# ajparra/iRotAvg

Measured on AMD Instinct MI355X. Metric: IRLS edge-updates/sec (+ iters-to-converge), higher is better.
Workload: dtype f64

## Files before the change

### irotavg_amd/capi.py

```python
import ctypes as C
import os

import numpy as np

_HERE = os.path.dirname(os.path.abspath(__file__))
LIB_PATH = os.path.join(_HERE, "libirotavg_hip.so")

OK = 0
ERR_BAD_ARG, ERR_NOT_SPANNING, ERR_SOLVER, ERR_UNKNOWN_COST = -1, -2, -3, -4
ERR_NOMEM, ERR_HIP, ERR_NO_DEVICE, ERR_NOT_CONVERGED = -5, -6, -7, -8
ERR_UNSUPPORTED = -9

SYMBOLS = [
    "irotavg_default_options", "irotavg_init_mst", "irotavg_make_A", "irotavg_l1ra", "irotavg_irls",
    "irotavg_quat_normalised", "irotavg_graph_create", "irotavg_graph_destroy",
    "irotavg_graph_set_rotations", "irotavg_graph_get_rotations",
    "irotavg_graph_snapshot_rotations", "irotavg_graph_restore_rotations", "irotavg_graph_get_weights",
    "irotavg_graph_set_weights", "irotavg_graph_irls", "irotavg_graph_l1ra",
    "irotavg_graph_quat_normalised", "irotavg_graph_get_stats", "irotavg_graph_reset_stats",
    "irotavg_graph_synchronize", "irotavg_graph_edge_residual", "irotavg_graph_get_residuals",
    "irotavg_graph_ls_solve", "irotavg_graph_update_weights", "irotavg_graph_apply_step",
    "irotavg_graph_l1decode_pd", "irotavg_graph_time_kernel", "irotavg_graph_fingerprint", "irotavg_version",
    "irotavg_device_count", "irotavg_error_string",
    "irotavg_viewgraph_create", "irotavg_viewgraph_destroy", "irotavg_viewgraph_add_view",
# ... 243 lines not shown
    return I


def default_options(**kw):
    o = Options()
    lib().irotavg_default_options(C.byref(o))
    for k, v in kw.items():
        if not hasattr(o, k):
            raise AttributeError(k)
        setattr(o, k, v)
    return o


def check(rc, where):
    if rc != OK:
        raise IrotavgError(rc, where)


class Graph:

    def __init__(self, I, QQ, n_total, f, **opts):
        I = edges(I)
        QQ = fmat(QQ)
        self.m, self.n_total, self.f = len(I), int(n_total), int(f)
        self.nu = self.n_total - self.f
        self._h = C.c_void_p()
        o = default_options(**opts)
        rc = lib().irotavg_graph_create(C.byref(self._h), self.m, self.n_total, self.f, _i(I),
                                        _d(QQ), QQ.shape[0], C.byref(o))
        if rc != OK:
            self._h = C.c_void_p()
            raise IrotavgError(rc, "irotavg_graph_create")

    def close(self):
        if getattr(self, "_h", None) and self._h.value:
            lib().irotavg_graph_destroy(self._h)
            self._h = C.c_void_p()

    def __del__(self):
        try:
            self.close()
        except Exception:
            pass

    def __enter__(self):
        return self

    def __exit__(self, *a):
        self.close()

    def set_rotations(self, Q):
        Q = fmat(Q)
        assert Q.shape == (self.n_total, 4)
        check(lib().irotavg_graph_set_rotations(self._h, _d(Q), Q.shape[0]), "set_rotations")

    def get_rotations(self):
        Q = np.zeros((self.n_total, 4), order="F")
        check(lib().irotavg_graph_get_rotations(self._h, _d(Q), Q.shape[0]), "get_rotations")
        return Q

    def snapshot_rotations(self):
        check(lib().irotavg_graph_snapshot_rotations(self._h), "snapshot_rotations")

    def restore_rotations(self):
        check(lib().irotavg_graph_restore_rotations(self._h), "restore_rotations")

    def get_weights(self):
        w = np.zeros(self.m)
        check(lib().irotavg_graph_get_weights(self._h, _d(w)), "get_weights")
        return w

    def set_weights(self, w):
        w = np.ascontiguousarray(w, dtype=np.float64)
        assert w.shape == (self.m,)
        check(lib().irotavg_graph_set_weights(self._h, _d(w)), "set_weights")

    def irls(self, cost=4, sigma=5 * np.pi / 180, max_iters=50, change_th=1e-3, allow_rc=()):
        iters = C.c_int(0)
        rt = C.c_double(0)
        trace = np.full(max(max_iters, 1), np.nan)
        rc = lib().irotavg_graph_irls(self._h, cost, sigma, max_iters, change_th, C.byref(iters),
                                      C.byref(rt), _d(trace))
        if rc != OK and rc not in allow_rc:
            raise IrotavgError(rc, "irotavg_graph_irls")
        return dict(rc=rc, iters=iters.value, runtime=rt.value, scores=trace[:iters.value].copy())

    def l1ra(self, max_iters=5, change_th=1e-3, allow_rc=()):
        iters = C.c_int(0)
        rt = C.c_double(0)
        trace = np.full(max(max_iters, 1), np.nan)
        rc = lib().irotavg_graph_l1ra(self._h, max_iters, change_th, C.byref(iters), C.byref(rt),
                                      _d(trace))
        if rc != OK and rc not in allow_rc:
            raise IrotavgError(rc, "irotavg_graph_l1ra")
        return dict(rc=rc, iters=iters.value, runtime=rt.value, scores=trace[:iters.value].copy())

    def quat_normalised(self):
        check(lib().irotavg_graph_quat_normalised(self._h), "quat_normalised")

    def stats(self):
        s = Stats()
        check(lib().irotavg_graph_get_stats(self._h, C.byref(s)), "get_stats")
        d = {k: getattr(s, k) for k, _ in Stats._fields_
             if k not in ("level_rows", "level_nnz", "last_relres")}
        d["level_rows"] = list(s.level_rows)[:s.levels]
        d["level_nnz"] = list(s.level_nnz)[:s.levels]
        d["last_relres"] = list(s.last_relres)
        return d

    def reset_stats(self):
        lib().irotavg_graph_reset_stats(self._h)

    def synchronize(self):
        check(lib().irotavg_graph_synchronize(self._h), "synchronize")

    def edge_residual(self):
        check(lib().irotavg_graph_edge_residual(self._h), "edge_residual")

    def get_residuals(self):
        r = np.zeros((self.m, 3), order="F")
        check(lib().irotavg_graph_get_residuals(self._h, _d(r), self.m), "get_residuals")
        return r

    def ls_solve(self, allow_rc=(), return_rc=False):
        X = np.zeros((self.nu, 3), order="F")
        rc = lib().irotavg_graph_ls_solve(self._h, _d(X), self.nu)
        if rc != OK and rc not in allow_rc:
            raise IrotavgError(rc, "irotavg_graph_ls_solve")
        return (rc, X) if return_rc else X

    def update_weights(self, cost, sigma):
        check(lib().irotavg_graph_update_weights(self._h, cost, sigma), "update_weights")

    def apply_step(self):
        s = C.c_double(0)
        check(lib().irotavg_graph_apply_step(self._h, C.byref(s)), "apply_step")
        return s.value

    def l1decode_pd(self, y, pdmaxiter=2):
        y = np.ascontiguousarray(y, dtype=np.float64)
        assert y.shape == (self.m,)
        x = np.zeros(self.nu)
        stuck = C.c_int(0)
        check(lib().irotavg_graph_l1decode_pd(self._h, _d(y), pdmaxiter, _d(x), C.byref(stuck)),
              "l1decode_pd")
        return x, stuck.value

    def direct_info(self):
        out = (C.c_int64 * 64)()
        k = lib().irotavg_graph_direct_info(self._h, out, 64)
        if k < 0:
            raise IrotavgError(k, "direct_info")
        if out[0] == 0:
            return dict(block=0, levels=[], closures=0, fused_assembly=0)
        nl = int(out[1])
        return dict(block=int(out[0]), levels=[dict(blocks=int(out[2 + 3 * l]), chunks=int(out[3 + 3 * l]),
                                                    reduced=int(out[4 + 3 * l])) for l in range(nl)],
                    closures=int(out[2 + 3 * nl]), fused_assembly=int(out[3 + 3 * nl]) if k > 3 + 3 * nl else 0)

    def direct_residual(self):
        out = np.zeros(3)
        check(lib().irotavg_graph_direct_residual(self._h, _d(out)), "direct_residual")
        return out

    def rotation_variance(self, pairs=None, marginals=True, allow_rc=()):
        return _variance_call(lambda *a: lib().irotavg_graph_rotation_variance(self._h, *a), self.n_total, pairs,
                              marginals, allow_rc, "irotavg_graph_rotation_variance")

    def edge_diagnostics(self, edge_var=True, leverage=True, chi2=True, allow_rc=()):
        return _edge_call(lambda *a: lib().irotavg_graph_edge_diagnostics(self._h, *a), self.m, edge_var, leverage,
                          chi2, allow_rc, "irotavg_graph_edge_diagnostics")

    def pose_weights(self, cost, sigma):
        check(lib().irotavg_graph_pose_weights(self._h, int(cost), float(sigma)), "irotavg_graph_pose_weights")

    def fingerprint(self):
        out = (C.c_uint64 * 512)()
        n = lib().irotavg_graph_fingerprint(self._h, out, 512)
        if n < 0:
            raise IrotavgError(n, "fingerprint")
        return [int(out[i]) for i in range(n)]

    FINGERPRINT_TAIL = ("l0_far_entries", "asm_windowed", "asm_l1_fused", "l1_fused", "cg2", "ndense", "ndense_pad",
                        "dense_bw", "mg_dense_max", "mg_kc_x1000", "additive_top")

    def fingerprint_scalars(self):
        fp = self.fingerprint()
        k = len(self.FINGERPRINT_TAIL)
        if not k <= len(fp) < 512:
            raise ValueError("fingerprint truncated: %d words" % len(fp))
        return dict(zip(self.FINGERPRINT_TAIL, fp[-k:]))

    def time_kernel(self, which, reps=20):
        ms = C.c_double(0)
        check(lib().irotavg_graph_time_kernel(self._h, which, reps, C.byref(ms)), "time_kernel")
        return ms.value


def _variance_call(call, n_total, pairs, marginals, allow_rc, where):
    P = np.zeros((0, 2), dtype=np.int32) if pairs is None else np.ascontiguousarray(pairs, dtype=np.int32).reshape(-1, 2)
    var = np.full(n_total, np.nan) if marginals else None
    pv = np.full(max(len(P), 1), np.nan)
    scale = C.c_double(np.nan)
    rc = call(_d(var) if marginals else None, len(P), _i(P) if len(P) else None, _d(pv), C.byref(scale))
    if rc != OK and rc not in allow_rc:
        raise IrotavgError(rc, where)
    return dict(rc=rc, var=var, pair_var=pv[:len(P)], scale=scale.value)


def rotation_variance(I, QQ, Q, weights, f, pairs=None, marginals=True, allow_rc=()):
    I = edges(I)
    Q = fmat(Q)
    QQ = fmat(QQ)
    w = np.ascontiguousarray(weights, dtype=np.float64)
    n_total = Q.shape[0]
    return _variance_call(lambda *a: lib().irotavg_rotation_variance(len(I), n_total, int(f), _i(I), _d(QQ),
                                                                     QQ.shape[0], _d(Q), Q.shape[0], _d(w), *a),
                          n_total, pairs, marginals, allow_rc, "irotavg_rotation_variance")


def _edge_call(call, m, edge_var, leverage, chi2, allow_rc, where):
    out = [np.full(m, np.nan) if want else None for want in (edge_var, leverage, chi2)]
    scale = C.c_double(np.nan)
    rc = call(*[_d(a) if a is not None else None for a in out], C.byref(scale))
    if rc != OK and rc not in allow_rc:
        raise IrotavgError(rc, where)
    return dict(rc=rc, edge_var=out[0], leverage=out[1], chi2=out[2], scale=scale.value)


def edge_diagnostics(I, QQ, Q, weights, f, edge_var=True, leverage=True, chi2=True, allow_rc=()):
    I = edges(I)
    Q = fmat(Q)
    QQ = fmat(QQ)
    w = np.ascontiguousarray(weights, dtype=np.float64)
    n_total = Q.shape[0]
    return _edge_call(lambda *a: lib().irotavg_edge_diagnostics(len(I), n_total, int(f), _i(I), _d(QQ), QQ.shape[0],
                                                                _d(Q), Q.shape[0], _d(w), *a),
                      len(I), edge_var, leverage, chi2, allow_rc, "irotavg_edge_diagnostics")


def oneshot_cache(enable):
    lib().irotavg_oneshot_cache(1 if enable else 0)


def oneshot_cache_clear():
    lib().irotavg_oneshot_cache_clear()


def oneshot_cache_stats():
    h, m = C.c_int64(0), C.c_int64(0)
    lib().irotavg_oneshot_cache_stats(C.byref(h), C.byref(m))
    return int(h.value), int(m.value)


def trim_memory():
    return int(lib().irotavg_trim_memory())


def window_solve(I, QQ, Q, f, cost=4, sigma=5 * np.pi / 180, l1_iters=100, irls_iters=100,
                 change_th=1e-3, kernel=0):
    I = edges(I)
    QQ = fmat(QQ)
    Q = fmat(Q)
    w = np.zeros(len(I))
    a, b = C.c_int(0), C.c_int(0)
    rc = lib().irotavg_window_solve_kernel(len(I), Q.shape[0], f, _i(I), _d(QQ), QQ.shape[0], _d(Q),
                                           Q.shape[0], cost, sigma, l1_iters, irls_iters, change_th,
                                           _d(w), C.byref(a), C.byref(b), kernel)
    check(rc, "irotavg_window_solve")
    return dict(Q=Q, weights=w, l1_iters=a.value, irls_iters=b.value)


def window_uncertainty(I, QQ, Q, f, weights=None, sigma=5 * np.pi / 180, pairs=None, marginals=True, edge_var=True,
                       leverage=True, chi2=True, allow_rc=()):
    I = edges(I)
    QQ = fmat(QQ)
    Q = fmat(Q)
    w = None if weights is None else np.ascontiguousarray(weights, dtype=np.float64)
    if w is not None and w.shape != (len(I),):
        raise ValueError("weights must have %d entries" % len(I))
    P = np.zeros((0, 2), dtype=np.int32) if pairs is None else np.ascontiguousarray(pairs, dtype=np.int32).reshape(-1, 2)
    n_total = Q.shape[0]
    var = np.full(n_total, np.nan) if marginals else None
    pv = np.full(max(len(P), 1), np.nan)
    out = [np.full(len(I), np.nan) if want else None for want in (edge_var, leverage, chi2)]
    scale = C.c_double(np.nan)
    rc = lib().irotavg_window_uncertainty(len(I), n_total, int(f), _i(I), _d(QQ), QQ.shape[0], _d(Q), n_total,
                                          None if w is None else _d(w), float(sigma), None if var is None else _d(var),
                                          len(P), _i(P) if len(P) else None, _d(pv) if len(P) else None,
                                          *[None if a is None else _d(a) for a in out], C.byref(scale))
    if rc != OK and rc not in allow_rc:
        raise IrotavgError(rc, "irotavg_window_uncertainty")
    return dict(rc=rc, var=var, pair_var=pv[:len(P)], edge_var=out[0], leverage=out[1], chi2=out[2], scale=scale.value)


def window_gate(I, QQ, Q, f, cand_I, cand_QQ, weights=None, sigma=5 * np.pi / 180, angle=True, pair_var=True, chi2=True,
                allow_rc=()):
    I = edges(I)
    QQ = fmat(QQ)
    Q = fmat(Q)
    w = None if weights is None else np.ascontiguousarray(weights, dtype=np.float64)
    if w is not None and w.shape != (len(I),):
        raise ValueError("weights must have %d entries" % len(I))
    cI = np.ascontiguousarray(cand_I, dtype=np.int32).reshape(-1, 2)
    cQ = fmat(np.asarray(cand_QQ, dtype=np.float64).reshape(-1, 4))
    if len(cQ) != len(cI):
        raise ValueError("cand_QQ must have %d rows" % len(cI))
    nc, n_total = len(cI), Q.shape[0]
    out = [np.full(nc, np.nan) if want else None for want in (angle, pair_var, chi2)]
    scale = C.c_double(np.nan)
    rc = lib().irotavg_window_gate(len(I), n_total, int(f), _i(I), _d(QQ), QQ.shape[0], _d(Q), n_total,
# ... 231 lines not shown
```

### irotavg_amd/csrc/bcr.hip

```cpp
#include <atomic>

#include "graph.hpp"
#include "kernels.hpp"
#include "asm0w.hpp"

namespace irh {
constexpr double kBcrGateTolMin = 1e-12;

typedef double v4d __attribute__((ext_vector_type(4)));
typedef double v2d __attribute__((ext_vector_type(2)));
typedef int v2i __attribute__((ext_vector_type(2)));

constexpr int kTopMax = 16, kTopRounds = 6;
struct BcrTopSched {
    int n = 0, nr = 0, last = 0;
    signed char ne[kTopRounds];
    signed char i[kTopRounds][4], a[kTopRounds][4], c[kTopRounds][4];
};

#if defined(__HIP_DEVICE_COMPILE__)
#define IRH_GPTR(T) T __attribute__((address_space(1))) *
#else
#define IRH_GPTR(T) T *
#endif
typedef IRH_GPTR(const double) gp_cd;
typedef IRH_GPTR(double) gp_d;
typedef IRH_GPTR(const int) gp_ci;
typedef IRH_GPTR(int) gp_i;
typedef IRH_GPTR(unsigned) gp_u;
typedef IRH_GPTR(const double4) gp_cd4;
constexpr int kUpLevels = 8;
struct BcrUpLevel {
    int nb, nred, nch;
    gp_cd inD, inR, inXD, inXR, inXG;
    gp_d W, sepD, sepR, extD, extR, extG;
};
struct BcrUpArgs {
    int nl;
    BcrUpLevel lev[kUpLevels];
    int n;
    gp_ci sl_off, col;
    gp_cd val, diag;
    gp_cd4 rhs;
    gp_d xtop;
    gp_u cnt;
    int top16;
    BcrTopSched top;
    gp_d xtop_all;
    gp_i fail;
};

struct BcrLevel {
    int nb = 0;
    int nred = 0;
    int nch = 0;
    DevBuf<double> W;
    DevBuf<double> sepD, sepR, extD, extR, extG;
    DevBuf<double> x;
};
struct BcrState {
    int B = 0;
    int NR = 3;
    int nfar = 0;
    std::vector<BcrLevel> lev;
    DevBuf<double> xtop;
    DevBuf<int> far_i, far_j, far_e;
    std::vector<DevBuf<double>> Dinv;
    DevBuf<double> topDinv;
    DevBuf<int> cl_off;
    DevBuf<int4> cl_step;
    DevBuf<int4> cl_init;
    DevBuf<int> cl_owner;
    DevBuf<double> cl_R, cl_W;
    DevBuf<double> cl_S, cl_T, lam;
    DevBuf<int> cl_alive;
    DevBuf<int> dead;
    DevBuf<int> co_off, co_rec;
    DevBuf<int2> co_elim;
    int cl_nslots = 0, cl_nsteps = 0, cl_nelim = 0, cl_npad = 0, cl_maxsteps = 1, cl_ndense = 0;
    DevBuf<int> cl_dense;
    int ext0 = 0;
    int dbg_word = -1;
    DevBuf<long long> stamps;
    DevBuf<unsigned> up_cnt;
    unsigned up_gen = 0;
    DevBuf<BcrUpArgs> up_args;
    bool up_used = false;
    bool top16 = false;
    BcrTopSched tsched;
    DevBuf<BcrTopSched> tsched_dev;
    DevBuf<int> ghost_extcol;
    DevBuf<double> remD, remR;
    DevBuf<double> res_part;
    DevBuf<int> res_zero;
    DevBuf<int> gate_skip;
    bool dead_clean = false;
    DevBuf<int2> cl_fin;
    DevBuf<int> cl_gid;
    DevBuf<uint8_t> cl_own;
    DevBuf<int> fix_row, fix_off, fix_e;
    DevBuf<double> fix_saved;
    int nfix = 0;
};

void BcrDeleter::operator()(BcrState *p) const { delete p; }

template <int CTRL>
__device__ __forceinline__ double bcr_dpp(double v) {
    int lo = __double2loint(v), hi = __double2hiint(v);
    lo = __builtin_amdgcn_mov_dpp(lo, CTRL, 0xf, 0xf, true);
    hi = __builtin_amdgcn_mov_dpp(hi, CTRL, 0xf, 0xf, true);
    return __hiloint2double(hi, lo);
}
__device__ __forceinline__ double bcr_row16_sum(double v) {
    v += bcr_dpp<0xB1>(v);
    v += bcr_dpp<0x4E>(v);
    v += bcr_dpp<0x141>(v);
    v += bcr_dpp<0x140>(v);
    return v;
}

template <int B>
__device__ __forceinline__ void bcr_invert(double *Dm, int lane, int *dead = nullptr, bool reg = false) {
    static_assert(B % 2 == 0 && B <= 32, "block size");
    constexpr int HB = B / 2;
    const int c = lane & 31, h = lane >> 5;
    const bool act = c < B;
    const int cl = act ? c : B - 1;
    const v2d *Dh = reinterpret_cast<const v2d *>(Dm + h * HB);
    double t[HB];
#pragma unroll
    for (int i = 0; i < HB; i++) t[i] = Dm[(h * HB + i) * B + cl];
    const double dg = Dm[cl * B + cl];
    const double dgt = kDeadTol * dg;
    int ndead = 0;
    auto pivot_inverse = [&](double tk, int k, int kh) {
        const double p0 = readlane_d(tk, k + 32 * kh);
        const bool alive = p0 > readlane_d(dgt, k);
        ndead += alive ? 0 : 1;
        double p = p0;
        if (reg && !alive) {
            const double ref = readlane_d(dg, k);
            p = ref > 0.0 ? ref : 1.0;
        }
        double x = __builtin_amdgcn_rcp(p);
        x = fma(fma(-p, x, 1.0), x, x);
        x = fma(fma(-p, x, 1.0), x, x);
        return (alive || reg) ? x : 0.0;
    };
    if (h == 0 && act) Dm[c] = c == 0 ? -1.0 : t[0];
    asm volatile("" ::: "memory");
    double pinv = pivot_inverse(t[0], 0, 0);
    double rowk = Dm[cl], colk[HB];
#pragma unroll
    for (int i = 0; i < HB; i += 2) {
        const v2d v = Dh[i / 2];
        colk[i] = v.x;
        colk[i + 1] = v.y;
    }
#pragma unroll
    for (int k = 0; k < B; k++) {
        const int kh = k / HB, ki = k - kh * HB;
        const int k1 = k + 1, kh1 = k1 / HB, ki1 = k1 - kh1 * HB;
        const bool isk = c == k;
        const double f = rowk * pinv;
        const double g = f;
        const double keep = isk ? 0.0 : 1.0;
        auto upd = [&](int i) {
            const double a = t[i] * keep;
            double u = fma(-colk[i], g, a);
            if (i == ki) u = (h == kh) ? g : u;
            t[i] = u;
        };
        double pinv1 = 0.0, rowk1 = 0.0, colk1[HB];
        if (k1 < B) {
            upd(ki1);
            if (h == kh1 && act) Dm[c] = c == k1 ? -1.0 : t[ki1];
            asm volatile("" ::: "memory");
            pinv1 = pivot_inverse(t[ki1], k1, kh1);
            rowk1 = Dm[cl];
#pragma unroll
            for (int i = 0; i < HB; i += 2) {
                const v2d v = Dh[i / 2];
                colk1[i] = v.x;
                colk1[i + 1] = v.y;
            }
        }
#pragma unroll
        for (int i = 0; i < HB; i++)
            if (!(k1 < B && i == ki1)) upd(i);
#pragma unroll
        for (int i = 0; i < HB; i++) asm volatile("" : "+v"(t[i]));
        if (k1 < B) {
            pinv = pinv1;
            rowk = rowk1;
#pragma unroll
            for (int i = 0; i < HB; i++) colk[i] = colk1[i];
        }
    }
    asm volatile("" ::: "memory");
#pragma unroll
    for (int i = 0; i < HB; i++)
        if (act) Dm[(h * HB + i) * B + c] = -t[i];
    if (dead && ndead && lane == 0) atomicAdd(dead, ndead);
}

__device__ __forceinline__ void bcr_stamp(long long *st, int slot) {
    if (st && threadIdx.x == 0) st[(size_t)blockIdx.x * 16 + slot] = (long long)__builtin_readcyclecounter();
}

template <int B, int NR = 3>
struct BcrDim {
    static constexpr int NC = 2 * B + NR;
// ... 142 lines not shown
        constexpr int NS = (Dm::NT + WPE - 1) / WPE;
        const int lj = lane & 15, lk = lane >> 4;
#pragma unroll
        for (int sl = 0; sl < NS; sl++) {
            const int nt = part + sl * WPE;
            if (nt >= Dm::NT) continue;
            const int j = 16 * nt + lj;
#pragma unroll
            for (int mt = 0; mt < Dm::MT; mt++)
#pragma unroll
                for (int r = 0; r < 4; r++) {
                    const int row = 16 * mt + 4 * r + lk;
                    if (row < B) {
                        const double v = w[mt][sl][r];
                        if (j < B)
                            Di[row * B + j] = v;
                        else if (j < 2 * B) {
                            if (hasQ) Q[row * B + j - B] = v;
                        } else if (j < Dm::NC)
                            Ri[row * NR + j - 2 * B] = v;
                    }
                }
        }
    }

    template <int WPE>
    __device__ __forceinline__ void phase2_mul(int part, const double *P, v4d (&out)[Dm::MT][NTPW], int lane) {
        constexpr int NS = (Dm::NT + WPE - 1) / WPE;
        double aop[Dm::MT][Dm::KS];
        bcr_load_a<B, false>(P, lane, aop);
#pragma unroll
        for (int sl = 0; sl < NS; sl++)
#pragma unroll
            for (int mt = 0; mt < Dm::MT; mt++) out[mt][sl] = v4d{0.0, 0.0, 0.0, 0.0};
#pragma unroll
        for (int s = 0; s < Dm::KS; s++)
#pragma unroll
            for (int sl = 0; sl < NS; sl++) {
                if (part + sl * WPE >= Dm::NT) continue;
#pragma unroll
                for (int mt = 0; mt < Dm::MT; mt++)
                    out[mt][sl] = __builtin_amdgcn_mfma_f64_16x16x4f64(aop[mt][s], w[s >> 2][sl][s & 3], out[mt][sl], 0, 0, 0);
            }
    }
    template <int WPE>
    __device__ __forceinline__ void phase2_put(int part, const v4d (&out)[Dm::MT][NTPW], double *P, double *Da,
                                               bool assign, double *Ra, int lane) {
        constexpr int NS = (Dm::NT + WPE - 1) / WPE;
        const int lj = lane & 15, lk = lane >> 4;
#pragma unroll
        for (int sl = 0; sl < NS; sl++) {
            const int nt = part + sl * WPE;
            if (nt >= Dm::NT) continue;
            const int c = 16 * nt + lj;
#pragma unroll
            for (int mt = 0; mt < Dm::MT; mt++)
#pragma unroll
                for (int r = 0; r < 4; r++) {
                    const int row = 16 * mt + 4 * r + lk;
                    if (row < B) {
                        const double v = out[mt][sl][r];
                        if (c < B)
                            Da[row * B + c] = assign ? -v : Da[row * B + c] - v;
                        else if (c < 2 * B)
                            P[row * B + c - B] = -v;
                        else if (c < Dm::NC)
                            Ra[row * NR + c - 2 * B] -= v;
                    }
                }
        }
    }
};

template <int B, int NR, int NBT = 12>
__device__ __forceinline__ void bcr_gather_row(int row, int lb, int r, const int *__restrict__ sl_off,
                                               const int *__restrict__ col, const double *__restrict__ val,
                                               const double *__restrict__ diag, const double4 *__restrict__ rhs,
                                               double *blocks, int oD, int oGnext, int oGprevT, double *Rblk, int nfar,
                                               const int *__restrict__ far_i, const int *__restrict__ far_j) {
    double *Dblk = blocks + oD;
    const int sl = row >> 6, ln = row & 63;
    const int o0 = sl_off[sl], w = sl_off[sl + 1] - o0;
    const v2i *__restrict__ cp = reinterpret_cast<const v2i *>(col) + (size_t)(o0 / 2) * 64 + ln;
    const v2d *__restrict__ vp = reinterpret_cast<const v2d *>(val) + (size_t)(o0 / 2) * 64 + ln;
    const int c0 = lb * B;
    const double dgv = diag[row];
    const double4 bb = rhs[row];
    for (int q0 = 0; q0 < w / 2; q0 += NBT) {
        v2i cc[NBT];
        v2d vv[NBT];
#pragma unroll
        for (int u = 0; u < NBT; u++) {
            const int q = q0 + u < w / 2 ? q0 + u : w / 2 - 1;
            cc[u] = __builtin_nontemporal_load(&cp[(size_t)q * 64]);
            vv[u] = __builtin_nontemporal_load(&vp[(size_t)q * 64]);
        }
#pragma unroll
        for (int u = 0; u < NBT; u++) {
#pragma unroll
            for (int h = 0; h < 2; h++) {
                const int c = h ? cc[u].y : cc[u].x;
                const double v = h ? vv[u].y : vv[u].x;
                const int gc = c - c0;
                const bool inD = gc >= 0 && gc < B, inN = gc >= B && gc < 2 * B, inP = gc < 0 && gc >= -B;
                int idx = oD + r * B + r;
                idx = inD ? oD + r * B + gc : idx;
                idx = inN ? oGnext + r * B + gc - B : idx;
                idx = inP ? oGprevT + (gc + B) * B + r : idx;
                const bool keep = q0 + u < w / 2 && v != 0.0 && !(inN && oGnext < 0) && !(inP && oGprevT < 0);
                double *dst = blocks + idx;
                if (keep) atomicAdd(dst, v);
            }
        }
    }
    Dblk[r * B + r] += dgv;
    Rblk[r * NR + 0] = bb.x;
    Rblk[r * NR + 1] = bb.y;
    Rblk[r * NR + 2] = bb.z;
    if (NR > 3)
        for (int q = 0; q < nfar; q++) {
            const int fi = far_i[q], fj = far_j[q];
            if (fi == row || fj == row) Rblk[r * NR + 3 + q] = (fi == row ? 1.0 : 0.0) - (fj == row ? 1.0 : 0.0);
        }
}

__constant__ signed char kBcrPlace[9][8] = {{-1, -1, -1, -1, -1, -1, -1, -1}, {7, -1, -1, -1, -1, -1, -1, -1},
                                             {3, 7, -1, -1, -1, -1, -1, -1},   {3, 5, 7, -1, -1, -1, -1, -1},
                                             {1, 3, 5, 7, -1, -1, -1, -1},     {1, 3, 5, 6, 7, -1, -1, -1},
                                             {1, 3, 4, 5, 6, 7, -1, -1},       {1, 2, 3, 4, 5, 6, 7, -1},
                                             {0, 1, 2, 3, 4, 5, 6, 7}};
__device__ __forceinline__ int bcr_pos(bool placed, int k, int t) { return placed ? (int)kBcrPlace[k][t] : t; }
__device__ __forceinline__ int bcr_ridx(bool placed, int k, int i) {
    if (!placed) return i < k ? i : -1;
    for (int t = 0; t < k; t++)
        if (kBcrPlace[k][t] == i) return t;
    return -1;
}

template <bool COH>
__device__ __forceinline__ double bcr_ld(const double *p) {
    if (!COH) return *p;
    const unsigned long long v = __hip_atomic_load(reinterpret_cast<const unsigned long long *>(p), __ATOMIC_RELAXED, __HIP_MEMORY_SCOPE_AGENT);
    return __longlong_as_double((long long)v);
}
template <bool COH>
__device__ __forceinline__ void bcr_st(double *p, double v) {
    if (!COH)
        *p = v;
    else
        __hip_atomic_store(reinterpret_cast<unsigned long long *>(p), (unsigned long long)__double_as_longlong(v), __ATOMIC_RELAXED,
                           __HIP_MEMORY_SCOPE_AGENT);
}

template <int B, int NR, bool L0, bool TOP, int NW, bool COH>
__device__ __forceinline__ void bcr_reduce_body(
    const int chunk, double (*sDG)[B * B], double (*sR)[B * NR], double *sZ,

    int nb, int nred, int n, const int *__restrict__ sl_off, const int *__restrict__ col, const double *__restrict__ val,
    const double *__restrict__ diag, const double4 *__restrict__ rhs, const double *__restrict__ inD,
    const double *__restrict__ inR, const double *__restrict__ inXD, const double *__restrict__ inXR,
    const double *__restrict__ inXG, double *__restrict__ W, double *__restrict__ sepD, double *__restrict__ sepR,
    double *__restrict__ extD, double *__restrict__ extR, double *__restrict__ extG, double *__restrict__ xtop, int dbg,
    int nfar, const int *__restrict__ far_i, const int *__restrict__ far_j, int ext0, const int *__restrict__ bptr,
    const int *__restrict__ bghost, const double *__restrict__ bval, const int *__restrict__ ghost_extcol, int place,
    long long *__restrict__ stamps, double *__restrict__ Dinvg, double *__restrict__ topDinv, int *__restrict__ deadctr,
    int reg) {
    typedef BcrDim<B, NR> Dm;
    constexpr int BB = B * B;
    double(*sD)[BB] = sDG;
    double(*sG)[BB] = sDG + 8;
    const int tid = threadIdx.x, lane = tid & 63;
    const int wave = __builtin_amdgcn_readfirstlane(tid >> 6);
    const bool hasExt = chunk > 0 || ext0;
    constexpr int NT_ = NW * 64;
    const int kreal = nb - chunk * 8 < 8 ? nb - chunk * 8 : 8;
    const bool placed = place && kreal < 8;

    const bool fastload = !L0 && !placed && !(chunk * 8 + 8 > nred && nred < nb);
    if (!fastload) {
        for (int e = tid; e < 8 * BB; e += NT_) {
            (&sD[0][0])[e] = 0.0;
            (&sG[0][0])[e] = 0.0;
        }
        for (int e = tid; e < 9 * B * NR; e += NT_) (&sR[0][0])[e] = 0.0;
        if (tid < 2) sZ[tid] = 0.0;
    }
    bcr_stamp(stamps, 0);
    if (!fastload) __syncthreads();
    bcr_stamp(stamps, 1);
    if (!L0 && fastload) {
        constexpr int NIT = (8 * BB + NT_ - 1) / NT_, U = NIT <= 12 ? NIT : 8;
        constexpr int NIR = (8 * B * NR + NT_ - 1) / NT_;
        const size_t cb = (size_t)chunk * 8 * BB, cr = (size_t)chunk * 8 * B * NR;
        double vr[NIR], vy[NIR];
#pragma unroll
        for (int u = 0; u < NIR; u++) {
            const int e = tid + NT_ * u, i = e / (B * NR);
            const bool ok = e < 8 * B * NR && i < kreal;
            vr[u] = ok ? bcr_ld<COH>(inR + cr + e) : 0.0;
            vy[u] = ok && chunk * 8 + i + 1 < nred ? bcr_ld<COH>(inXR + cr + B * NR + e) : 0.0;
        }
        for (int u0 = 0; u0 < NIT; u0 += U) {
            double vd[U], vx[U], vg[U];
#pragma unroll
            for (int u = 0; u < U; u++) {
                const int e = tid + NT_ * (u0 + u), i = e / BB;
                const bool ok = e < 8 * BB && i < kreal;
                vd[u] = ok ? bcr_ld<COH>(inD + cb + e) : 0.0;
                vx[u] = ok && chunk * 8 + i + 1 < nred ? bcr_ld<COH>(inXD + cb + BB + e) : 0.0;
                vg[u] = ok && (chunk * 8 + i > 0 || ext0) ? bcr_ld<COH>(inXG + cb + e) : 0.0;
            }
#pragma unroll
            for (int u = 0; u < U; u++) {
                const int e = tid + NT_ * (u0 + u), i = e / BB, el = e - i * BB;
                if (e >= 8 * BB) continue;
                (&sD[0][0])[e] = i < kreal ? vd[u] + vx[u] : (el % (B + 1) == 0 ? 1.0 : 0.0);
                (&sG[0][0])[e] = vg[u];
            }
        }
#pragma unroll
        for (int u = 0; u < NIR; u++) {
            const int e = tid + NT_ * u;
            if (e < 8 * B * NR) (&sR[1][0])[e] = vr[u] + vy[u];
        }
        for (int e = tid; e < B * NR; e += NT_) sR[0][e] = 0.0;
        if (tid < 2) sZ[tid] = 0.0;
    } else if (L0) {
        const int row0 = chunk * 8 * B;
        for (int t = tid; t < kreal * B; t += NT_) {
            const int row = row0 + t, blk = t / B, r = t - blk * B;
            const int ps = bcr_pos(placed, kreal, blk);
            if (row < n)
                bcr_gather_row<B, NR>(row, chunk * 8 + blk, r, sl_off, col, val, diag, rhs, &sDG[0][0], ps * BB,
                                      ps < 7 ? (8 + ps + 1) * BB : -1, blk == 0 ? 8 * BB : -1, sR[ps + 1], nfar, far_i,
                                      far_j);
            else
                sD[ps][r * B + r] = 1.0;
        }
        for (int i = placed ? 1 : 0; i < 8; i++)
            if (bcr_ridx(placed, kreal, i) < 0)
                for (int e = tid; e < B; e += NT_) sD[i][e * B + e] = 1.0;
        if (ext0 && chunk == 0) {
            for (int r = tid; r < B && r < n; r += NT_)
                for (int sl = bptr[r]; sl < bptr[r + 1]; sl++) {
                    const int gi = bghost[sl];
                    const int ec = gi >= 0 ? ghost_extcol[gi] : -1;
                    if (ec >= 0) sG[0][ec * B + r] -= bval[sl];
                }
        }
    } else {
        auto where = [&](int i, int &gb, int &slot) {
            const int t = bcr_ridx(placed, kreal, i);
            gb = t >= 0 ? chunk * 8 + t : -1;
            slot = t > 0 ? bcr_pos(placed, kreal, t - 1) + 1 : 0;
            return t;
        };
        constexpr int NIT = (8 * BB + NT_ - 1) / NT_, U = NIT <= 12 ? NIT : 8;
        const bool allraw = !placed && chunk * 8 >= nred;
        if (allraw)
            for (int e = tid; e < (8 - kreal) * B; e += NT_) sD[kreal + e / B][(e % B) * (B + 1)] = 1.0;
        for (int u0 = 0; u0 < NIT && !allraw; u0 += U) {
            double vd[U], vx[U], vg[U];
#pragma unroll
            for (int u = 0; u < U; u++) {
                const int e = tid + NT_ * (u0 + u), i = e / BB, el = e - i * BB;
                int gb, slot;
                const int t = e < 8 * BB ? where(i, gb, slot) : -1;
                const bool ok = t >= 0 && gb < nred;
                vd[u] = ok ? bcr_ld<COH>(inD + (size_t)gb * BB + el) : 0.0;
                vx[u] = ok && gb + 1 < nred ? bcr_ld<COH>(inXD + (size_t)(gb + 1) * BB + el) : 0.0;
                vg[u] = ok && (gb > 0 || ext0) ? bcr_ld<COH>(inXG + (size_t)gb * BB + el) : 0.0;
            }
#pragma unroll
            for (int u = 0; u < U; u++) {
                const int e = tid + NT_ * (u0 + u), i = e / BB, el = e - i * BB;
                if (e >= 8 * BB) continue;
                int gb, slot;
                const int t = where(i, gb, slot);
                if (t >= 0 && gb < nred) {
                    sD[i][el] = vd[u] + vx[u];
                    if (gb > 0 || ext0) sG[slot][el] = vg[u];
                } else if (t < 0 && !(placed && i == 0) && el / B == el % B) {
                    sD[i][el] = 1.0;
                }
            }
        }
        if (!allraw) {
            constexpr int NIR = (8 * B * NR + NT_ - 1) / NT_;
            double vr[NIR], vy[NIR];
#pragma unroll
            for (int u = 0; u < NIR; u++) {
                const int e = tid + NT_ * u, i = e / (B * NR), el = e - i * (B * NR);
                int gb, slot;
                const int t = e < 8 * B * NR ? where(i, gb, slot) : -1;
                const bool ok = t >= 0 && gb < nred;
                vr[u] = ok ? bcr_ld<COH>(inR + (size_t)gb * B * NR + el) : 0.0;
                vy[u] = ok && gb + 1 < nred ? bcr_ld<COH>(inXR + (size_t)(gb + 1) * B * NR + el) : 0.0;
                if (ok) sR[i + 1][el] = vr[u] + vy[u];
            }
        }
        if (chunk * 8 + 8 > nred && nred < nb) {
            for (int t = tid; t < 8 * B; t += NT_) {
                const int i = t / B, r = t - i * B, gb = chunk * 8 + i;
                if (gb >= nred && gb < nb) {
                    const int lb = 8 * nred + (gb - nred), row = lb * B + r;
                    if (row < n)
                        bcr_gather_row<B, NR, (NW == 8 && B <= 24 ? 24 : 12)>(row, lb, r, sl_off, col, val, diag, rhs, &sDG[0][0],
                                                                            i * BB, -1, gb > 0 ? (8 + i) * BB : -1, sR[i + 1],
                                                                            nfar, far_i, far_j);
                    else
                        sD[i][r * B + r] = 1.0;
                }
            }
        }
    }
    __syncthreads();
    bcr_stamp(stamps, 2);

    constexpr int WPE0 = NW / 4 < Dm::NT ? NW / 4 : Dm::NT;
    constexpr int NTPW = (Dm::NT + WPE0 - 1) / WPE0;
    BcrElim<B, NR, NTPW> E;
    v4d out[Dm::MT][NTPW];
#define IRH_BCR_ROUND(RND)                                                                                          \
    {                                                                                                               \
        constexpr int NE = 4 >> RND;                                                                                \
        constexpr int WPE = NW / NE < Dm::NT ? NW / NE : Dm::NT;                                                    \
         \
         \
         \
        const int e = wave / WPE, part0 = wave - e * WPE;                                                           \
        const int part = (WPE == 2 && NE == 4) ? (part0 ^ ((e >> 1) & 1)) : part0;                                  \
        int i = -1, a = -1, c = 7;                                                                                  \
        if (e < NE) {                                                                                               \
            if (RND == 0) {                                                                                         \
                i = 2 * e;                                                                                          \
                a = i - 1;                                                                                          \
                c = i + 1;                                                                                          \
            } else if (RND == 1) {                                                                                  \
                i = 1 + 4 * e;                                                                                      \
                a = e == 0 ? -1 : 3;                                                                                \
                c = e == 0 ? 3 : 7;                                                                                 \
            } else {                                                                                                \
                i = 3;                                                                                              \
            }                                                                                                       \
        }                                                                                                           \
        const bool active = i >= 0 && bcr_ridx(placed, kreal, i) >= 0;                                              \
        const bool hasP = a >= 0 || hasExt;                                                                         \
           \
          \
        const int isw = wave < NE ? (RND == 0 ? 2 * wave : RND == 1 ? 1 + 4 * wave : 3) : -1;                       \
        if (isw >= 0 && bcr_ridx(placed, kreal, isw) >= 0 && !(dbg & 1))                                            \
            bcr_invert<B>(sD[isw], lane, deadctr, reg != 0);                                                        \
        __syncthreads();                                                                                            \
                                        \
        if (Dinvg && active && part == 0)                                                                           \
            for (int o = lane; o < BB; o += 64) Dinvg[((size_t)chunk * 7 + i) * BB + o] = sD[i][o];                 \
        bcr_stamp(stamps, 3 + 4 * RND);                                                                             \
        if (active && !(dbg & 2))                                                                                   \
            E.template phase1<WPE>(part, sD[i], sG[a + 1], hasP, sG[i + 1], sR[i + 1], sD[c], sR[c + 1],            \
                                   W + ((size_t)chunk * 7 + i) * B * Dm::NC, sZ, lane);                             \
        __syncthreads();                                                                                            \
        bcr_stamp(stamps, 4 + 4 * RND);                                                                             \
        if (active && hasP && !(dbg & 4)) E.template phase2_mul<WPE>(part, sG[a + 1], out, lane);                   \
        if (WPE > 1) __syncthreads();                                                                               \
        bcr_stamp(stamps, 5 + 4 * RND);                                                                             \
        if (active && hasP && !(dbg & 4))                                                                           \
            E.template phase2_put<WPE>(part, out, sG[a + 1], a >= 0 ? sD[a] : sD[0], a < 0 && RND == 0, sR[a + 1],  \
                                       lane);                                                                       \
        __syncthreads();                                                                                            \
        bcr_stamp(stamps, 6 + 4 * RND);                                                                             \
    }
    IRH_BCR_ROUND(0)
    IRH_BCR_ROUND(1)
    IRH_BCR_ROUND(2)
#undef IRH_BCR_ROUND

    if (TOP) {
        if (wave == 0) {
            if (bcr_ridx(placed, kreal, 7) >= 0) {
                bcr_invert<B>(sD[7], lane, deadctr, reg != 0);
                if (topDinv)
                    for (int o = lane; o < BB; o += 64) topDinv[o] = sD[7][o];
                for (int o = lane; o < B * NR; o += 64) {
                    const int k = o / NR, q = o - NR * k;
                    double s = 0.0;
                    for (int cidx = 0; cidx < B; cidx++) s += sD[7][k * B + cidx] * sR[8][cidx * NR + q];
                    xtop[o] = s;
                }
            } else {
                for (int o = lane; o < B * NR; o += 64) xtop[o] = 0.0;
            }
        }
    } else {
        for (int e = tid; e < BB; e += NT_) {
            bcr_st<COH>(sepD + (size_t)chunk * BB + e, sD[7][e]);
            if (hasExt) {
                bcr_st<COH>(extD + (size_t)chunk * BB + e, sD[0][e]);
                bcr_st<COH>(extG + (size_t)chunk * BB + e, sG[0][e]);
            }
        }
        for (int e = tid; e < B * NR; e += NT_) {
            bcr_st<COH>(sepR + (size_t)chunk * B * NR + e, sR[8][e]);
            if (hasExt) bcr_st<COH>(extR + (size_t)chunk * B * NR + e, sR[0][e]);
        }
    }
    bcr_stamp(stamps, 15);
}

struct BcrAsmArgs {
    int nch, nsl;
    long long m, mpad;
    const uint32_t *slot_eid;
    const int *tile_e0;
    const uint32_t *beid;
    const uint8_t *bflag;
    const double *wsrc, *er;
    double *excess, *idg, *bval;
};
template <bool ASM>
struct BcrL0Ptr {
    typedef const double *__restrict__ d;
    typedef const double4 *__restrict__ d4;
};
template <>
struct BcrL0Ptr<true> {
    typedef double *d;
    typedef double4 *d4;
};

template <int B, int NR, bool L0, bool TOP, int NW, bool ASM = false>
__global__ __launch_bounds__(NW * 64, (NW == 4 && B <= 24 && NR == 3 ? 2 : 1)) void k_bcr_reduce(

    int nb, int nred, int n, const int *__restrict__ sl_off, const int *__restrict__ col, typename BcrL0Ptr<ASM>::d val,
    typename BcrL0Ptr<ASM>::d diag, typename BcrL0Ptr<ASM>::d4 rhs, const double *__restrict__ inD,
    const double *__restrict__ inR, const double *__restrict__ inXD, const double *__restrict__ inXR,
    const double *__restrict__ inXG, double *__restrict__ W, double *__restrict__ sepD, double *__restrict__ sepR,
    double *__restrict__ extD, double *__restrict__ extR, double *__restrict__ extG, double *__restrict__ xtop, int dbg,
    int nfar, const int *__restrict__ far_i, const int *__restrict__ far_j, int ext0, const int *__restrict__ bptr,
    const int *__restrict__ bghost, const double *__restrict__ bval, const int *__restrict__ ghost_extcol, int place,
    long long *__restrict__ stamps, double *__restrict__ Dinvg, double *__restrict__ topDinv, int *__restrict__ deadctr,
    int reg, BcrAsmArgs A) {
    constexpr int kRed = 16 * B * B + 9 * B * NR + 2, kAsm = ASM ? Asm0wLds<0, false>::doubles : 0;
    __shared__ double lds[kRed > kAsm ? kRed : kAsm];
    double(*sDG)[B * B] = reinterpret_cast<double(*)[B * B]>(lds);
    double(*sR)[B * NR] = reinterpret_cast<double(*)[B * NR]>(lds + 16 * B * B);
    double *sZ = lds + 16 * B * B + 9 * B * NR;
    if constexpr (ASM) {
        static_assert(L0 && NR == 3 && (8 * B) % 64 == 0, "a chunk's rows are whole slices");
        constexpr int SPC = 8 * B / 64;
#define IRH_BCR_ASM_SLICE(sl_)                                                                                           \
    asm0w_slice<0, false, NW * 64>(sl_, lds, n, A.m, A.mpad, sl_off, A.slot_eid, (const uint8_t *)nullptr, A.tile_e0, bptr, \
                                   A.beid, A.bflag, A.wsrc, A.er, val, A.excess, diag, A.idg, rhs, A.bval, 0,            \
                                   (const int *)nullptr, (double *)nullptr, (double *)nullptr, (double *)nullptr,        \
                                   (double *)nullptr)
        if ((int)blockIdx.x >= A.nch) {
            const int sl = A.nch * SPC + ((int)blockIdx.x - A.nch);
            if (sl < A.nsl) IRH_BCR_ASM_SLICE(sl);
            return;
        }
        for (int k = 0; k < SPC; k++) {
            const int sl = (int)blockIdx.x * SPC + k;
            if (sl >= A.nsl) break;
            IRH_BCR_ASM_SLICE(sl);
            __syncthreads();
        }
#undef IRH_BCR_ASM_SLICE
        __builtin_amdgcn_fence(__ATOMIC_RELEASE, "workgroup");
        __syncthreads();
        __builtin_amdgcn_fence(__ATOMIC_ACQUIRE, "workgroup");
    }
    bcr_reduce_body<B, NR, L0, TOP, NW, false>(blockIdx.x, sDG, sR, sZ, nb, nred, n, sl_off, col, val, diag, rhs, inD, inR, inXD, inXR,
                                               inXG, W, sepD, sepR, extD, extR, extG, xtop, dbg, nfar, far_i, far_j, ext0, bptr,
                                               bghost, bval, ghost_extcol, place, stamps, Dinvg, topDinv, deadctr, reg);
}

static BcrTopSched bcr_top_schedule(int n) {
    BcrTopSched T;
    memset(&T, 0, sizeof(T));
    T.n = n;
    std::vector<int> alive(n);
    for (int k = 0; k < n; k++) alive[k] = k;
    while (alive.size() > 1 && T.nr < kTopRounds) {
        const int r = T.nr++;
        std::vector<int> next;
        int ne = 0;
        for (size_t p = 0; p < alive.size(); p++) {
            if (p % 2 == 0 && ne < 4) {
                T.i[r][ne] = (signed char)alive[p];
                T.a[r][ne] = (signed char)(p > 0 ? alive[p - 1] : -1);
                T.c[r][ne] = (signed char)(p + 1 < alive.size() ? alive[p + 1] : -1);
                ne++;
            } else {
                next.push_back(alive[p]);
            }
        }
        T.ne[r] = (signed char)ne;
        alive.swap(next);
    }
    T.last = alive[0];
    return T;
}
static size_t bcr_top_lds(int B, int n) {
    return ((size_t)(2 * n - 1) * B * B + (size_t)2 * n * B * 3 + 2) * sizeof(double) + sizeof(BcrTopSched);
}

template <int B, int NW, bool COH>
__device__ __forceinline__ void bcr_top_body(double *smem, const BcrTopSched *__restrict__ Tg, const double *__restrict__ inD,
                                             const double *__restrict__ inR, const double *__restrict__ inXD,
                                             const double *__restrict__ inXR, const double *__restrict__ inXG,
                                             double *__restrict__ xout, int dbg, long long *__restrict__ stamps) {
    constexpr int NR = 3;
    typedef BcrDim<B, NR> Dm;
    constexpr int BB = B * B, XB = B * NR, NT_ = NW * 64;
    static_assert(NW == 8, "eight waves");
    const int n = Tg->n;
    double(*sD)[BB] = reinterpret_cast<double(*)[BB]>(smem);
    double(*sG)[BB] = sD + n;
    double(*sR)[XB] = reinterpret_cast<double(*)[XB]>(smem + (size_t)(2 * n - 1) * BB);
    double(*sX)[XB] = sR + n;
    double *sZ = &sX[n][0];
    BcrTopSched &T = *reinterpret_cast<BcrTopSched *>(sZ + 2);
    const int tid = threadIdx.x, lane = tid & 63;
    const int wave = __builtin_amdgcn_readfirstlane(tid >> 6);
    static_assert(sizeof(BcrTopSched) % 4 == 0, "copied by words");
    if (tid < (int)(sizeof(BcrTopSched) / 4)) reinterpret_cast<int *>(&T)[tid] = reinterpret_cast<const int *>(Tg)[tid];
    bcr_stamp(stamps, 0);
    {
        constexpr int U = 6;
        const int nD = n * BB, nG = (n - 1) * BB, nR = n * XB;
        for (int e0 = 0; e0 < nD; e0 += U * NT_) {
            double vd[U], vx[U], vg[U];
#pragma unroll
            for (int u = 0; u < U; u++) {
                const int e = e0 + tid + NT_ * u;
                vd[u] = e < nD ? bcr_ld<COH>(inD + e) : 0.0;
                vx[u] = e < nG ? bcr_ld<COH>(inXD + BB + e) : 0.0;
                vg[u] = e < nG ? bcr_ld<COH>(inXG + BB + e) : 0.0;
            }
#pragma unroll
            for (int u = 0; u < U; u++) {
                const int e = e0 + tid + NT_ * u;
                if (e < nD) (&sD[0][0])[e] = vd[u] + vx[u];
                if (e < nG) (&sG[0][0])[e] = vg[u];
            }
        }
        for (int e = tid; e < nR; e += NT_) {
            const double vr = bcr_ld<COH>(inR + e);
            const double vy = e < nR - XB ? bcr_ld<COH>(inXR + XB + e) : 0.0;
            (&sR[0][0])[e] = vr + vy;
        }
        if (tid < 2) sZ[tid] = 0.0;
    }
    __syncthreads();
    bcr_stamp(stamps, 1);
    for (int r = 0; r < T.nr; r++) {
        const int ne = T.ne[r];
        if (wave < ne && !(dbg & 1)) bcr_invert<B>(sD[T.i[r][wave]], lane);
        __syncthreads();
        bcr_stamp(stamps, 2 + 2 * r);
        auto products = [&](auto wpe_tag) {
            constexpr int WPE = decltype(wpe_tag)::value;
            const int e = wave / WPE, part0 = wave - e * WPE;
            const int part = WPE == 2 ? (part0 ^ ((e >> 1) & 1)) : part0;
            const bool active = e < ne;
            const int i = active ? T.i[r][e] : 0, a = active ? T.a[r][e] : -1, c = active ? T.c[r][e] : -1;
            const bool hasP = a >= 0, hasQ = c >= 0;
            BcrElim<B, NR, 2> E;
            v4d out[Dm::MT][2];
            if (active && !(dbg & 2))
                E.template phase1<WPE>(part, sD[i], hasP ? sG[a] : sZ, hasP, hasQ ? sG[i] : sZ, sR[i], hasQ ? sD[c] : sD[i],
                                       hasQ ? sR[c] : sR[i], (double *)nullptr, sZ, lane, hasQ);
            __syncthreads();
            if (active && hasP && !(dbg & 4)) E.template phase2_mul<WPE>(part, sG[a], out, lane);
            if (active && !(dbg & 2)) E.template keep_w<WPE>(part, sD[i], hasQ ? sG[i] : sZ, hasQ, sR[i], lane);
            __syncthreads();
            if (active && hasP && !(dbg & 4)) E.template phase2_put<WPE>(part, out, sG[a], sD[a], false, sR[a], lane);
            __syncthreads();
        };
        if (ne > 2) products(std::integral_constant<int, 2>());
        else products(std::integral_constant<int, 4>());
        bcr_stamp(stamps, 3 + 2 * r);
    }
    const int last = T.last;
    if (wave == 0) {
        bcr_invert<B>(sD[last], lane);
        for (int o = lane; o < XB; o += 64) {
            const int k = o / NR, q = o - NR * k;
            double acc = 0.0;
            for (int cidx = 0; cidx < B; cidx++) acc += sD[last][k * B + cidx] * sR[last][cidx * NR + q];
            sX[last][o] = acc;
        }
    }
    __syncthreads();
    bcr_stamp(stamps, 14);
    {
        constexpr int UPB = B / 4, NCT = (2 * B + 15) / 16;
        const int lk = lane >> 4, lp = lane & 15;
        for (int r = T.nr - 1; r >= 0; r--) {
            const int ne = T.ne[r];
            for (int u = wave; u < ne * UPB; u += NW) {
                const int e = u / UPB, it = u - e * UPB;
                const int i = T.i[r][e], a = T.a[r][e], c = T.c[r][e];
                const double *xa = sX[a >= 0 ? a : 0], *xc = sX[c >= 0 ? c : 0];
                const int k = 4 * it + lk;
                double s0 = 0.0, s1 = 0.0, s2 = 0.0;
#pragma unroll
                for (int t = 0; t < NCT; t++) {
                    const int cidx = lp + 16 * t;
                    if (cidx < B) {
                        if (a >= 0) {
                            const double wv = sD[i][k * B + cidx];
                            s0 += wv * xa[cidx * 3 + 0];
                            s1 += wv * xa[cidx * 3 + 1];
                            s2 += wv * xa[cidx * 3 + 2];
                        }
                    } else if (cidx < 2 * B) {
                        if (c >= 0) {
                            const double wv = sG[i][k * B + cidx - B];
                            s0 += wv * xc[(cidx - B) * 3 + 0];
                            s1 += wv * xc[(cidx - B) * 3 + 1];
                            s2 += wv * xc[(cidx - B) * 3 + 2];
                        }
                    }
                }
                s0 = bcr_row16_sum(s0);
                s1 = bcr_row16_sum(s1);
                s2 = bcr_row16_sum(s2);
                if (lp == 0) {
                    sX[i][k * 3 + 0] = sR[i][k * 3 + 0] - s0;
                    sX[i][k * 3 + 1] = sR[i][k * 3 + 1] - s1;
                    sX[i][k * 3 + 2] = sR[i][k * 3 + 2] - s2;
                }
            }
            __syncthreads();
        }
    }
    for (int e = tid; e < n * XB; e += NT_) xout[e] = (&sX[0][0])[e];
    bcr_stamp(stamps, 15);
}

template <int B>
__global__ __launch_bounds__(512, 1) void k_bcr_top(const BcrTopSched *__restrict__ T, const double *__restrict__ inD, const double *__restrict__ inR,
                                                    const double *__restrict__ inXD, const double *__restrict__ inXR,
                                                    const double *__restrict__ inXG, double *__restrict__ xout, int dbg,
                                                    long long *__restrict__ stamps) {
    extern __shared__ __attribute__((aligned(16))) double top_smem[];
    bcr_top_body<B, 8, false>(top_smem, T, inD, inR, inXD, inXR, inXG, xout, dbg, stamps);
}

extern __shared__ __attribute__((aligned(16))) double up_smem[];
typedef IRH_GPTR(const BcrUpArgs) gp_args;
template <int B, bool TOP>
__device__ __noinline__ void bcr_up_chunk(gp_args A, int i, int dbg, long long *stl) {
    constexpr int NR = 3;
    IRH_GPTR(const BcrUpLevel) L = &A->lev[i];
    double(*sDG)[B * B] = reinterpret_cast<double(*)[B * B]>(up_smem);
    double(*sR)[B * NR] = reinterpret_cast<double(*)[B * NR]>(up_smem + 16 * B * B);
    double *sZ = up_smem + 16 * B * B + 9 * B * NR;
    bcr_reduce_body<B, NR, false, TOP, 8, true>(
        blockIdx.x, sDG, sR, sZ, L->nb, L->nred, A->n, (const int *)A->sl_off, (const int *)A->col, (const double *)A->val,
        (const double *)A->diag, (const double4 *)A->rhs, (const double *)L->inD, (const double *)L->inR, (const double *)L->inXD,
        (const double *)L->inXR, (const double *)L->inXG, (double *)L->W, (double *)L->sepD, (double *)L->sepR, (double *)L->extD,
        (double *)L->extR, (double *)L->extG, (double *)A->xtop, dbg, 0, (const int *)nullptr, (const int *)nullptr, 0, (const int *)nullptr, (const int *)nullptr,
        (const double *)nullptr, (const int *)nullptr, 0, stl ? stl - (size_t)blockIdx.x * 16 : nullptr, (double *)nullptr,
        (double *)nullptr, (int *)nullptr, 0);
}
template <int B>
__device__ __noinline__ void bcr_up_top(gp_args A, int i, int dbg, long long *stl) {
    IRH_GPTR(const BcrUpLevel) L = &A->lev[i];
    bcr_top_body<B, 8, true>(up_smem, (const BcrTopSched *)&A->top, (const double *)L->inD, (const double *)L->inR,
                             (const double *)L->inXD, (const double *)L->inXR, (const double *)L->inXG, (double *)A->xtop_all, dbg,
                             stl ? stl - (size_t)blockIdx.x * 16 : nullptr);
}
template <int B>
__global__ __launch_bounds__(512, 1) void k_bcr_reduce_up(const BcrUpArgs *__restrict__ Ap, unsigned gen, int dbg,
                                                          long long *__restrict__ stamps) {
    constexpr int NR = 3;
    __shared__ int s_ok;
    const gp_args Ag = (gp_args)Ap;
    const BcrUpArgs &A = *Ap;
    const int wg = blockIdx.x;
    const int nl = A.nl;
    bool fine = true;
    for (int i = 0; i < nl; i++) {
        if (wg >= A.lev[i].nch) break;
        long long *stl = stamps && wg == (dbg >> 8) ? stamps + 32 * i : nullptr;
        if (stl && threadIdx.x == 0) stl[16] = (long long)__builtin_readcyclecounter();
        if (stl && (threadIdx.x & 63) == 0) stl[20 + (threadIdx.x >> 6)] = 0x10000 + (long long)__builtin_amdgcn_s_getreg((4 << 0) | (0 << 6) | (31 << 11));
        if (i > 0) {
            if (threadIdx.x == 0) {
                const unsigned target = gen * (unsigned)A.lev[i - 1].nch;
                int good = 0;
                for (int spin = 0; spin < (1 << 21); spin++) {
                    if ((int)(__hip_atomic_load((const unsigned *)A.cnt + (i - 1), __ATOMIC_RELAXED, __HIP_MEMORY_SCOPE_AGENT) - target) >= 0) {
                        good = 1;
                        break;
                    }
                    __builtin_amdgcn_s_sleep(2);
                }
                if (!good) __hip_atomic_store((int *)A.fail, 1, __ATOMIC_RELAXED, __HIP_MEMORY_SCOPE_AGENT);
                s_ok = good;
            }
            __syncthreads();
            fine = fine && s_ok != 0;
        }
        if (stl && threadIdx.x == 0) stl[17] = (long long)__builtin_readcyclecounter();
        if (i == nl - 1) {
            const bool bad = !fine || __hip_atomic_load((const int *)A.fail, __ATOMIC_RELAXED, __HIP_MEMORY_SCOPE_AGENT) != 0;
            if (A.top16) {
                if (!bad) bcr_up_top<B>(Ag, i, dbg, stl);
                else
                    for (int e = threadIdx.x; e < A.top.n * B * NR; e += 512) A.xtop_all[e] = __builtin_nan("");
            } else {
                if (!bad) bcr_up_chunk<B, true>(Ag, i, dbg, stl);
                else
                    for (int e = threadIdx.x; e < B * NR; e += 512) A.xtop[e] = __builtin_nan("");
            }
        } else {
            if (fine) bcr_up_chunk<B, false>(Ag, i, dbg, stl);
            if (stl && threadIdx.x == 0) stl[18] = (long long)__builtin_readcyclecounter();
            __builtin_amdgcn_s_waitcnt(0);
            __syncthreads();
            if (threadIdx.x == 0) __hip_atomic_fetch_add((unsigned *)A.cnt + i, 1u, __ATOMIC_RELAXED, __HIP_MEMORY_SCOPE_AGENT);
            if (stl && threadIdx.x == 0) stl[19] = (long long)__builtin_readcyclecounter();
        }
    }
}

template <int B>
static size_t bcr_up_lds(int ntop) {
    const size_t chunk = ((size_t)16 * B * B + 9 * B * 3 + 2) * sizeof(double);
    return ntop > 0 ? std::max(chunk, bcr_top_lds(B, ntop)) : chunk;
}
namespace {
std::atomic<int> g_up_used[16];
template <int B>
int bcr_up_capacity(int dev) {
    static std::atomic<int> cap[16];
    const int d = dev & 15;
    int c = cap[d].load(std::memory_order_relaxed);
    if (c == 0) {
        int per_cu = 0, cus = 0;
        if (hipOccupancyMaxActiveBlocksPerMultiprocessor(&per_cu, k_bcr_reduce_up<B>, 512, bcr_up_lds<B>(0)) != hipSuccess) per_cu = 0;
        if (hipDeviceGetAttribute(&cus, hipDeviceAttributeMultiprocessorCount, dev) != hipSuccess) cus = 0;
        (void)hipGetLastError();
        c = per_cu > 0 && cus > 0 ? per_cu * cus : -1;
        cap[d].store(c, std::memory_order_relaxed);
    }
    return c;
}
template <int B>
bool bcr_up_reserve(Graph &g, int nwg) {
    const int capwg = bcr_up_capacity<B>(g.device);
    if (capwg <= 0) return false;
    const int total = g.sw.bcr_up_cap;
    const int cost = (int)(((long long)nwg * 1024 + capwg - 1) / capwg);
    const int need = cost - g.bcr_up_held;
    if (need <= 0) return true;
    std::atomic<int> &used = g_up_used[g.device & 15];
    const int before = used.fetch_add(need, std::memory_order_acq_rel);
    if (before + need > total) {
        used.fetch_sub(need, std::memory_order_acq_rel);
        return false;
    }
    g.bcr_up_held += need;
    return true;
}
}
void bcr_up_release(Graph &g) noexcept {
    if (g.bcr_up_held > 0) {
        g_up_used[g.device & 15].fetch_sub(g.bcr_up_held, std::memory_order_acq_rel);
        g.bcr_up_held = 0;
    }
}

__device__ __forceinline__ int bcr_back_mask(int m) {
    if (m & 0x05) m |= 0x02;
    if (m & 0x50) m |= 0x20;
    if (m & 0x36) m |= 0x08;
    return m;
}
template <int B, int NR, int NWB = 4>
__device__ __forceinline__ void bcr_back_rounds(const double *sW, double (*sX)[B * NR], bool placed, int kreal, int wave,
                                                int lane, int mask = 0x7f) {
    typedef BcrDim<B, NR> Dm;
    constexpr int WB = B * Dm::NC;
    const int lk = lane >> 4, lp = lane & 15;
#pragma unroll
    for (int rnd = 2; rnd >= 0; rnd--) {
        if (NR == 3) {
            constexpr int UPB = B / 4;
            const int nbk = 4 >> rnd;
            for (int u = wave; u < nbk * UPB; u += NWB) {
                const int e = u / UPB, it = u - e * UPB;
                int i, a, c;
                if (rnd == 0) {
                    i = 2 * e;
                    a = i - 1;
                    c = i + 1;
                } else if (rnd == 1) {
                    i = 1 + 4 * e;
                    a = e == 0 ? -1 : 3;
                    c = e == 0 ? 3 : 7;
                } else {
                    i = 3;
                    a = -1;
                    c = 7;
                }
                if (!((mask >> i) & 1) || bcr_ridx(placed, kreal, i) < 0) continue;
                const double *Wi = sW + i * WB;
                const double *xa = sX[a + 1], *xcn = sX[c + 1];
                const int k = 4 * it + lk;
                double s0 = 0.0, s1 = 0.0, s2 = 0.0;
#pragma unroll
                for (int t = 0; t < Dm::NT; t++) {
                    const int cidx = lp + 16 * t;
                    if (cidx < Dm::NC) {
                        const double wv = Wi[k * Dm::NC + cidx];
                        if (cidx < B) {
                            s0 -= wv * xa[cidx * 3 + 0];
                            s1 -= wv * xa[cidx * 3 + 1];
                            s2 -= wv * xa[cidx * 3 + 2];
                        } else if (cidx < 2 * B) {
                            s0 -= wv * xcn[(cidx - B) * 3 + 0];
                            s1 -= wv * xcn[(cidx - B) * 3 + 1];
                            s2 -= wv * xcn[(cidx - B) * 3 + 2];
                        } else {
                            const int q = cidx - 2 * B;
                            s0 += q == 0 ? wv : 0.0;
                            s1 += q == 1 ? wv : 0.0;
                            s2 += q == 2 ? wv : 0.0;
                        }
                    }
                }
                s0 = bcr_row16_sum(s0);
                s1 = bcr_row16_sum(s1);
                s2 = bcr_row16_sum(s2);
                if (lp == 0) {
                    sX[i + 1][k * 3 + 0] = s0;
                    sX[i + 1][k * 3 + 1] = s1;
                    sX[i + 1][k * 3 + 2] = s2;
                }
            }
        } else {
            static_assert(NR == 3 || NWB == 4, "the closures' right-hand sides ride on four-wave workgroups");
            int i = -1, a = -1, c = 7;
            if (rnd == 0) {
                i = 2 * wave;
                a = i - 1;
                c = i + 1;
            } else if (rnd == 1) {
                if (wave < 2) {
                    i = 1 + 4 * wave;
                    a = wave == 0 ? -1 : 3;
                    c = wave == 0 ? 3 : 7;
                }
            } else if (wave == 0) {
                i = 3;
            }
            if (i >= 0 && bcr_ridx(placed, kreal, i) >= 0) {
                const double *Wi = sW + i * WB;
                const double *xa = sX[a + 1], *xcn = sX[c + 1];
                for (int o = lane; o < B * NR; o += 64) {
                    const int k = o / NR, q = o - NR * k;
                    const double *wr = Wi + k * Dm::NC;
                    double sacc = wr[2 * B + q];
#pragma unroll 4
                    for (int cidx = 0; cidx < B; cidx++)
                        sacc -= wr[cidx] * xa[cidx * NR + q] + wr[B + cidx] * xcn[cidx * NR + q];
                    sX[i + 1][o] = sacc;
                }
            }
        }
        __syncthreads();
    }
}

__device__ __forceinline__ void bcr_apply_sum(double acc, double *__restrict__ part, int slot) {
    __shared__ double sm[16];
    acc = wave_sum(acc);
    if ((threadIdx.x & 63) == 0) sm[threadIdx.x >> 6] = acc;
    __syncthreads();
    if (threadIdx.x == 0) {
        double t = 0.0;
        for (int w = 0; w < (int)(blockDim.x >> 6); w++) t += sm[w];
        part[slot] = t;
    }
// ... 893 lines not shown
    for (size_t k = 0; k < steps.size(); k++) steps[k].w *= 2;
    if (r >= 8) {
        int d = 0;
        for (auto &kv : by_key)
            if ((long long)kv.second.size() * 4 >= r) {
                dense.resize((size_t)(d + 1) * r, -1);
                for (int k : kv.second) {
                    dense[(size_t)d * r + owner[(size_t)k]] = k;
                    steps[(size_t)k].w |= 1;
                }
                d++;
            }
        S.cl_ndense = d;
    }
    if (dense.empty()) dense.push_back(-1);
    S.cl_dense.upload(dense, g.stream);
    S.cl_nslots = nslots;
    S.cl_nsteps = (int)steps.size();
    S.cl_nelim = (int)elim.size();
    S.cl_npad = r <= kSolveLdsMax ? r : (r + 63) / 64 * 64;
    S.far_i.upload(g.bcr_far_i, g.stream);
    S.far_j.upload(g.bcr_far_j, g.stream);
    S.far_e.upload(g.bcr_far_e, g.stream);
    S.cl_off.upload(off, g.stream);
    S.cl_step.upload(steps, g.stream);
    S.cl_init.upload(init, g.stream);
    if (shard) {
        std::vector<int> gowner(owner.size());
        for (size_t k = 0; k < owner.size(); k++) gowner[k] = g.bcr_far_gid[(size_t)owner[k]];
        if (gowner.empty()) gowner.push_back(0);
        S.cl_owner.upload(gowner, g.stream);
        S.cl_fin.upload(fin, g.stream);
        S.cl_gid.upload(g.bcr_far_gid, g.stream);
        S.cl_own.upload(g.bcr_far_own, g.stream);
    } else {
        S.cl_owner.upload(owner, g.stream);
    }
    S.co_off.upload(eoff, g.stream);
    S.co_rec.upload(erec, g.stream);
    S.co_elim.upload(elim, g.stream);
    S.cl_R.alloc(steps.size() * (size_t)B);
    S.cl_W.alloc(steps.size() * (size_t)B);
    if (!shard) S.cl_S.alloc((size_t)S.cl_npad * S.cl_npad);
    S.cl_T.alloc((size_t)S.cl_npad * 3);
    S.lam.alloc((size_t)S.cl_npad * 3);
    S.cl_alive.alloc((size_t)S.cl_npad);
    S.Dinv.resize((size_t)nl);
    for (int l = 0; l < nl; l++) S.Dinv[(size_t)l].alloc((size_t)S.lev[l].nch * 7 * B * B);
    S.topDinv.alloc((size_t)B * B);
    S.dead.alloc(1);
    IRH_CHECK(hipMemsetAsync(S.topDinv.p, 0, sizeof(double) * (size_t)B * B, g.stream));
    IRH_CHECK(hipStreamSynchronize(g.stream));
}

static void bcr_alloc(Graph &g) {
    if (g.bcr) return;
    g.bcr.reset(new BcrState());
    BcrState &S = *g.bcr;
    S.B = g.bcr_B;
    S.nfar = (int)g.bcr_far_e.size();
    S.NR = 3;
    const int B = S.B, NR = S.NR, NC = 2 * B + NR;
    const int nb0 = (g.levels[0].n + B - 1) / B;
    int nch0 = (nb0 + 7) / 8;
    int nraw = 0;
    {
        int ncu = 256;
        (void)hipDeviceGetAttribute(&ncu, hipDeviceAttributeMultiprocessorCount, g.device);
        if (ncu <= 0) ncu = 256;
        const int cap = ncu * (B <= 24 && NR == 3 ? 2 : 1);
        const int full = nch0 / cap * cap, rem = nch0 - full;
        if (full > 0 && rem > 0 && rem <= cap / 4 && !g.bcr_shard && !g.sw.bcr_no_mixed) {
            nraw = nb0 - 8 * full;
            nch0 = full;
        }
    }
    S.top16 = B <= 24 && S.nfar == 0 && !g.bcr_shard && !g.sw.bcr_no_top16;
    const int topmax = S.top16 ? kTopMax : 8;
    int nb = nb0, nch = nch0;
    for (int l = 0;; l++) {
        S.lev.emplace_back();
        BcrLevel &L = S.lev.back();
        L.nb = nb;
        L.nch = nch;
        L.nred = (l == 1 && nraw > 0) ? nb - nraw : nb;
        const bool last = nb <= topmax && !g.bcr_shard && l > 0;
        if (last && S.top16) {
            L.x.alloc((size_t)L.nch * 8 * B * NR);
            S.tsched = bcr_top_schedule(nb);
            S.tsched_dev.alloc(1);
            IRH_CHECK(hipMemcpyAsync(S.tsched_dev.p, &S.tsched, sizeof(BcrTopSched), hipMemcpyHostToDevice, g.stream));
            IRH_CHECK(hipStreamSynchronize(g.stream));
            break;
        }
        if (l == 0 && nb <= 8) S.top16 = false;
        L.W.alloc((size_t)L.nch * 7 * B * NC);
        if (l > 0) L.x.alloc((size_t)L.nch * 8 * B * NR);
        if (nb <= 8 && !g.bcr_shard) {
            S.top16 = false;
            break;
        }
        L.sepD.alloc((size_t)L.nch * B * B);
        L.extD.alloc((size_t)L.nch * B * B);
        L.extG.alloc((size_t)L.nch * B * B);
        L.sepR.alloc((size_t)L.nch * B * NR);
        L.extR.alloc((size_t)L.nch * B * NR);
        if (nb <= 8) break;
        nb = L.nch + (l == 0 ? nraw : 0);
        nch = (nb + 7) / 8;
    }
    if (g.bcr_shard) {
        S.ext0 = g.bcr_ext0;
        S.ghost_extcol.upload(g.bcr_ghost_extcol, g.stream);
        S.remD.alloc((size_t)B * B);
        S.remR.alloc((size_t)B * NR);
        IRH_CHECK(hipStreamSynchronize(g.stream));
    }
    S.xtop.alloc((size_t)B * NR);
    if (S.nfar > 0) bcr_closure_plan(g);
    if (g.bcr_shard && !g.bcr_fix_row.empty()) {
        S.nfix = (int)g.bcr_fix_row.size();
        S.fix_row.upload(g.bcr_fix_row, g.stream);
        S.fix_off.upload(g.bcr_fix_off, g.stream);
        S.fix_e.upload(g.bcr_fix_e, g.stream);
        S.fix_saved.alloc((size_t)S.nfix);
        IRH_CHECK(hipStreamSynchronize(g.stream));
    }
}

template <int B, int NR>
static void bcr_run(Graph &g, int only, int pass, bool open_top = false, int phase = 0, const double *xc_top = nullptr,
                    const double *xext = nullptr) {
    BcrState &S = *g.bcr;
    Level &L0 = g.levels[0];
    hipStream_t st = g.stream;
    const int nl = (int)S.lev.size();
    const int dbg = S.dbg_word >= 0 ? S.dbg_word : g.sw.bcr_dbg;
    long long *stamps = nullptr;
    if (dbg & 64) {
        if (!S.stamps.p) S.stamps.alloc((size_t)S.lev[0].nch * 16);
        stamps = S.stamps.p;
    }
    const int nfar = 0;
    const int *fi = nullptr, *fj = nullptr;
    (void)pass;
    bool fused_up = false;
    if constexpr (NR == 3 && B <= 24) {
        fused_up = nl >= 3 && nl - 1 <= kUpLevels && only < 0 && phase == 0 && !open_top && !g.bcr_shard && S.nfar == 0 &&
                   S.lev[1].nch <= 256 && !(dbg & 64) && !g.bcr_no_fused_up;
        if ((dbg & 128) && !S.stamps.p) S.stamps.alloc((size_t)std::max(S.lev[0].nch * 16, 32 * kUpLevels));
        if (fused_up) fused_up = bcr_up_reserve<B>(g, S.lev[1].nch);
    }
    if (only < 0 && phase != 2) S.up_used = false;
    for (int l = 0; l < nl && phase != 2; l++) {
        if (only >= 0 && only != l) continue;
        if constexpr (NR == 3 && B <= 24) {
            if (S.top16 && l == nl - 1 && !fused_up) {
                const BcrLevel &F = S.lev[l - 1];
                const size_t lds = bcr_top_lds(B, S.lev[l].nb);
                static std::atomic<size_t> lds_set[16];
                if (lds_set[g.device & 15].load() < lds) {
                    IRH_CHECK(hipFuncSetAttribute(reinterpret_cast<const void *>(&k_bcr_top<B>),
                                                  hipFuncAttributeMaxDynamicSharedMemorySize, (int)lds));
                    lds_set[g.device & 15].store(lds);
                }
                hipLaunchKernelGGL((k_bcr_top<B>), dim3(1), dim3(512), lds, st, S.tsched_dev.p, F.sepD.p, F.sepR.p, F.extD.p,
                                   F.extR.p, F.extG.p, S.lev[l].x.p, dbg, stamps);
                continue;
            }
            if (fused_up && l >= 1) {
                if (l > 1) continue;
                if (S.up_cnt.n < (size_t)kUpLevels + 1) {
                    S.up_cnt.alloc(kUpLevels + 1);
                    S.up_cnt.zero(st);
                    S.up_gen = 0;
                }
                if (!S.up_args.p) {
                    BcrUpArgs A;
                    memset(&A, 0, sizeof(A));
                    A.nl = nl - 1;
                    for (int i = 0; i < A.nl; i++) {
                        BcrLevel &Li = S.lev[1 + i], &Fi = S.lev[i];
                        A.lev[i] = BcrUpLevel{Li.nb,          Li.nred,        Li.nch,         (gp_cd)Fi.sepD.p, (gp_cd)Fi.sepR.p,
                                              (gp_cd)Fi.extD.p, (gp_cd)Fi.extR.p, (gp_cd)Fi.extG.p, (gp_d)Li.W.p,   (gp_d)Li.sepD.p,
                                              (gp_d)Li.sepR.p, (gp_d)Li.extD.p, (gp_d)Li.extR.p, (gp_d)Li.extG.p};
                    }
                    A.n = L0.n;
                    A.sl_off = (gp_ci)L0.sl_off.p;
                    A.col = (gp_ci)L0.col.p;
                    A.val = (gp_cd)L0.val.p;
                    A.diag = (gp_cd)L0.diag.p;
                    A.rhs = (gp_cd4)L0.b.p;
                    A.xtop = (gp_d)S.xtop.p;
                    A.cnt = (gp_u)S.up_cnt.p;
                    A.top16 = S.top16;
                    A.top = S.tsched;
                    A.xtop_all = (gp_d)S.lev[nl - 1].x.p;
                    A.fail = (gp_i) reinterpret_cast<int *>(S.up_cnt.p + kUpLevels);
                    S.up_args.alloc(1);
                    IRH_CHECK(hipMemcpyAsync(S.up_args.p, &A, sizeof(A), hipMemcpyHostToDevice, st));
                    IRH_CHECK(hipStreamSynchronize(st));
                }
                if (g.sw.bcr_fake_up_fail && g.stats.direct_up_fallbacks == 0)
                    IRH_CHECK(hipMemsetAsync(S.up_cnt.p + kUpLevels, 1, sizeof(int), st));
                const size_t lds = bcr_up_lds<B>(S.top16 ? S.lev[nl - 1].nb : 0);
                static std::atomic<size_t> lds_set[16];
                if (lds_set[g.device & 15].load() < lds) {
                    IRH_CHECK(hipFuncSetAttribute(reinterpret_cast<const void *>(&k_bcr_reduce_up<B>),
                                                  hipFuncAttributeMaxDynamicSharedMemorySize, (int)lds));
                    lds_set[g.device & 15].store(lds);
                }
                hipLaunchKernelGGL((k_bcr_reduce_up<B>), dim3(S.lev[1].nch), dim3(512), lds, st, S.up_args.p, ++S.up_gen, dbg,
                                   (dbg & 128) ? S.stamps.p : (long long *)nullptr);
                S.up_used = true;
                continue;
            }
        }
        BcrLevel &L = S.lev[l];
        const BcrLevel *F = l > 0 ? &S.lev[l - 1] : nullptr;
        const bool top = l == nl - 1 && !open_top;
#define IRH_BCR_ARGS                                                                                             \
    L.nb, L.nred, L0.n, L0.sl_off.p, L0.col.p, L0.val.p, L0.diag.p, L0.b.p, F ? F->sepD.p : nullptr,             \
        F ? F->sepR.p : nullptr, F ? F->extD.p : nullptr, F ? F->extR.p : nullptr, F ? F->extG.p : nullptr, L.W.p, \
        L.sepD.p, L.sepR.p, L.extD.p, L.extR.p, L.extG.p, S.xtop.p, dbg, nfar, fi, fj, S.ext0, g.bptr.p, g.bghost.p,  \
        g.bval.p, S.ghost_extcol.p, (int)g.bcr_shard, stamps, S.nfar > 0 ? S.Dinv[(size_t)l].p : (double *)nullptr,         \
        S.nfar > 0 ? S.topDinv.p : (double *)nullptr, S.nfar > 0 ? S.dead.p : (int *)nullptr, (int)g.bcr_guard, asmA
        const bool wide = L.nch <= 256;
        BcrAsmArgs asmA{};
        bool asm0 = false;
        if constexpr (NR == 3 && (8 * B) % 64 == 0) {
            asm0 = l == 0 && g.bcr_asm_fused && only < 0 && phase == 0 && !open_top && S.nfar == 0 && !g.bcr_shard;
            if (asm0) {
                asmA = BcrAsmArgs{L.nch,   L0.nsl,    (long long)g.m, (long long)g.mpad, g.slot_eid.p, g.tile_e0.p, g.beid.p,
                                  g.bflag.p, g.bcr_wsrc, g.er.p,         L0.excess.p,       L0.idg.p,     g.bval.p};
                const int extra = std::max(0, L0.nsl - L.nch * (8 * B / 64));
#define IRH_BCR_LAUNCH_ASM(TOP_)                                                                                          \
    if (B <= 24 && wide)                                                                                                  \
        hipLaunchKernelGGL((k_bcr_reduce<B, NR, true, TOP_, (B <= 24 ? 8 : 4), true>), dim3(L.nch + extra),               \
                           dim3(B <= 24 ? 512 : 256), 0, st, IRH_BCR_ARGS);                                               \
    else                                                                                                                  \
        hipLaunchKernelGGL((k_bcr_reduce<B, NR, true, TOP_, 4, true>), dim3(L.nch + extra), dim3(256), 0, st, IRH_BCR_ARGS);
                if (top) {
                    IRH_BCR_LAUNCH_ASM(true)
                } else {
                    IRH_BCR_LAUNCH_ASM(false)
                }
#undef IRH_BCR_LAUNCH_ASM
            }
        }
        if (asm0) continue;
#define IRH_BCR_LAUNCH(L0_, TOP_)                                                                                   \
    if constexpr (B <= 24) {                                                                                        \
        if (wide)                                                                                                   \
            hipLaunchKernelGGL((k_bcr_reduce<B, NR, L0_, TOP_, 8>), dim3(L.nch), dim3(512), 0, st, IRH_BCR_ARGS);   \
        else                                                                                                        \
            hipLaunchKernelGGL((k_bcr_reduce<B, NR, L0_, TOP_, 4>), dim3(L.nch), dim3(256), 0, st, IRH_BCR_ARGS);   \
    } else {                                                                                                        \
        hipLaunchKernelGGL((k_bcr_reduce<B, NR, L0_, TOP_, 4>), dim3(L.nch), dim3(256), 0, st, IRH_BCR_ARGS);       \
    }
        if (l == 0 && top) {
            IRH_BCR_LAUNCH(true, true)
        } else if (l == 0) {
            IRH_BCR_LAUNCH(true, false)
        } else if (top) {
            IRH_BCR_LAUNCH(false, true)
        } else {
            IRH_BCR_LAUNCH(false, false)
        }
#undef IRH_BCR_LAUNCH
#undef IRH_BCR_ARGS
    }
    double4 *Xout = g.bcr_out ? g.bcr_out : g.X.p + g.ng;
    bool fused_back = false;
    const int ltop = S.top16 ? nl - 2 : nl - 1;
    if constexpr (NR == 3) fused_back = ltop >= 1 && !g.bcr_shard && !open_top;
    const bool apply = NR == 3 && g.bcr_apply && only < 0 && phase == 0 && (fused_back || (S.top16 && nl == 2)) && !g.bcr_out &&
                       g.ng == 0;
    g.bcr_applied = apply;
    for (int l = ltop; l >= 0 && phase != 1; l--) {
        if (only >= 0 && only != 100 + l) continue;
        BcrLevel &L = S.lev[l];
        if constexpr (NR == 3) {
            if (fused_back && l >= 1) {
                if (l > 1) continue;
                BcrBackPlan P;
                for (int k = 0; k < nl; k++) {
                    P.W[k] = S.lev[k].W.p;
                    P.nb[k] = S.lev[k].nb;
                }
                P.top = ltop;
                P.base = 1;
                hipLaunchKernelGGL((k_bcr_back_top<B>), dim3(L.nch), dim3(kBackTopThreads), 0, st, P,
                                   S.top16 ? S.lev[nl - 1].x.p : S.xtop.p, L.x.p, Xout, L0.n, L.nred,
                                   apply ? g.Q.p : (double4 *)nullptr, g.f, g.part_score.p, S.lev[0].nch, (int)S.top16);
                continue;
            }
        }
        const double *xc = l == nl - 1 ? (open_top ? xc_top : S.xtop.p) : S.lev[l + 1].x.p;
        if (l == 0)
            hipLaunchKernelGGL((k_bcr_back<B, NR, true>), dim3(L.nch), dim3(256), 0, st, L.nb, L.nred, L0.n, L.W.p, xc,
                               (double *)nullptr, Xout, (double *)nullptr, 0, 0, nfar, xext, (int)g.bcr_shard,
                               apply ? g.Q.p : (double4 *)nullptr, g.f, g.part_score.p, 0);
        else
            hipLaunchKernelGGL((k_bcr_back<B, NR, false>), dim3(L.nch), dim3(256), 0, st, L.nb, L.nred, L0.n, L.W.p, xc,
                               L.x.p, Xout, (double *)nullptr, 0, 0, nfar, xext, (int)g.bcr_shard);
    }
}

template <int B>
static void bcr_launch_forward(hipStream_t st, const BcrClPlan &P, int r, int nslots, const int *off, const int4 *steps,
                               const int4 *init, double *recR, double *recW, double *T, const double *slot_init,
                               const int2 *fin, const int *gid, double *dep, int world, int rank);

template <int B>
static void bcr_run_all(Graph &g, int only) {
    BcrState &S = *g.bcr;
    if (S.nfar == 0 || only >= 0) {
        bcr_run<B, 3>(g, only, 0);
        return;
    }
    hipStream_t st = g.stream;
    const int r = S.nfar, npad = S.cl_npad, nl = (int)S.lev.size();
    if (!S.dead_clean) IRH_CHECK(hipMemsetAsync(S.dead.p, 0, sizeof(int), st));
    S.dead_clean = false;
    bcr_run<B, 3>(g, -1, 0, false, 1);
    BcrClPlan P;
    for (int l = 0; l < nl; l++) {
        P.W[l] = S.lev[l].W.p;
        P.Wrw[l] = S.lev[l].W.p;
        P.Dinv[l] = S.Dinv[(size_t)l].p;
    }
    P.topDinv = S.topDinv.p;
    P.xtop = S.xtop.p;
    bcr_launch_forward<B>(st, P, r, S.cl_nslots, S.cl_off.p, S.cl_step.p, S.cl_init.p, S.cl_R.p, S.cl_W.p, S.cl_T.p, nullptr,
                          nullptr, nullptr, nullptr, 0, 0);
    const int nt = (npad + 15) / 16;
    const size_t lds_pairs = (size_t)4 * (S.cl_maxsteps + 64) * sizeof(int);
    if (r <= kClosurePairsMax && S.cl_maxsteps < 32768 && lds_pairs <= 60 * 1024 && !g.sw.bcr_s_tiles)
        hipLaunchKernelGGL((k_bcr_closure_S_pairs<B>), dim3((npad + 3) / 4, npad), dim3(256), lds_pairs, st, r, npad,
                           S.cl_maxsteps, S.cl_off.p, S.cl_step.p, S.cl_R.p, S.cl_W.p, S.far_e.p, g.bcr_wsrc, g.bcr_wsquare,
                           S.cl_S.p, S.cl_T.p, S.cl_alive.p);
    else
    hipLaunchKernelGGL((k_bcr_closure_S<B>), dim3(nt, nt), dim3(256), (size_t)32 * S.cl_maxsteps * sizeof(int), st, r, npad,
                       S.cl_maxsteps, S.cl_ndense, S.cl_dense.p, S.cl_off.p, S.cl_step.p, S.cl_R.p,
                       S.cl_W.p, S.far_e.p, g.bcr_wsrc, g.bcr_wsquare, S.cl_S.p, S.cl_T.p, S.cl_alive.p);
    if (r <= kSolveLdsMax) {
        bcr_launch_solve_lds(st, r, npad, S.cl_S.p, S.cl_T.p, S.lam.p);
    } else {
        dense_invert_spd(g, S.cl_S.p, npad);
        hipLaunchKernelGGL(k_bcr_closure_lambda, dim3((r + 3) / 4), dim3(256), 0, st, r, npad, S.cl_S.p, S.cl_T.p,
                           S.lam.p);
    }
    hipLaunchKernelGGL((k_bcr_closure_correct<B>), dim3(S.cl_nelim), dim3(1024), 0, st, P, S.co_off.p, S.co_rec.p,
                       S.co_elim.p, S.cl_owner.p, S.cl_W.p, S.lam.p);
    bcr_run<B, 3>(g, -1, 0, false, 2);
}

struct BcrPtrs {
    const double *d[kMaxLevels], *r[kMaxLevels];
    int n;
};
template <int B>
__global__ __launch_bounds__(256) void k_bcr_pack_top(BcrPtrs P, int ext0, const double *__restrict__ sepD,
                                                      const double *__restrict__ sepR, const double *__restrict__ extG,
                                                      double *__restrict__ buf, int world, int rank) {
    constexpr int BB = B * B, BR = B * 3;
    double *oD = buf + (size_t)rank * BB, *oXD = buf + (size_t)world * BB + (size_t)rank * BB,
           *oXG = buf + (size_t)2 * world * BB + (size_t)rank * BB,
           *oR = buf + (size_t)3 * world * BB + (size_t)rank * BR,
           *oXR = buf + (size_t)3 * world * BB + (size_t)world * BR + (size_t)rank * BR;
    for (int e = threadIdx.x; e < BB; e += 256) {
        oD[e] = sepD[e];
        double sacc = 0.0;
        if (ext0)
            for (int l = 0; l < P.n; l++) sacc += P.d[l][e];
        oXD[e] = sacc;
        oXG[e] = ext0 ? extG[e] : 0.0;
    }
    for (int e = threadIdx.x; e < BR; e += 256) {
        oR[e] = sepR[e];
        double sacc = 0.0;
        if (ext0)
            for (int l = 0; l < P.n; l++) sacc += P.r[l][e];
        oXR[e] = sacc;
    }
}

__global__ __launch_bounds__(256) void k_bcr_top_records(int B, int world, int mine, double *__restrict__ buf, double *__restrict__ rec) {
    const int BB = B * B, BR = B * 3, RS = 3 * BB + 2 * BR;
    const int r0 = mine >= 0 ? mine : 0, r1 = mine >= 0 ? mine + 1 : world;
    for (int idx = blockIdx.x * 256 + threadIdx.x; idx < (r1 - r0) * RS; idx += gridDim.x * 256) {
        const int rank = r0 + idx / RS, e = idx % RS;
        size_t b;
        if (e < 3 * BB) b = (size_t)(e / BB) * world * BB + (size_t)rank * BB + e % BB;
        else {
            const int q = e - 3 * BB;
            b = (size_t)3 * world * BB + (size_t)(q / BR) * world * BR + (size_t)rank * BR + q % BR;
        }
        if (mine >= 0) rec[(size_t)rank * RS + e] = buf[b];
        else buf[b] = rec[(size_t)rank * RS + e];
    }
}
void bcr_top_to_record(BcrTop &T, int rank, hipStream_t st) {
    hipLaunchKernelGGL(k_bcr_top_records, dim3(8), dim3(256), 0, st, T.B, T.world, rank, T.buf.p, T.rec.p);
}
void bcr_top_from_records(BcrTop &T, hipStream_t st) {
    hipLaunchKernelGGL(k_bcr_top_records, dim3(8 * T.world), dim3(256), 0, st, T.B, T.world, -1, T.buf.p, T.rec.p);
}

void bcr_top_alloc(BcrTop &T, int B, int world) {
    T.B = B;
    T.world = world;
    T.buf.alloc(T.n_doubles());
    T.rec.alloc(T.n_doubles());
    T.W.alloc((size_t)7 * B * (2 * B + 3));
    T.x.alloc((size_t)8 * B * 3);
    T.xtop.alloc((size_t)B * 3);
}


__global__ __launch_bounds__(256) void k_bcr_fix_diag(int nfix, const int *__restrict__ row, const int *__restrict__ off,
                                                       const int *__restrict__ e, const double *__restrict__ wsrc, int wsquare,
                                                       double *__restrict__ diag, double *__restrict__ saved, int restore) {
    const int k = blockIdx.x * 256 + threadIdx.x;
    if (k >= nfix) return;
    const int rw = row[k];
    if (restore) {
        diag[rw] = saved[k];
        return;
    }
    const double d = diag[rw];
    saved[k] = d;
    double s = 0.0;
    for (int t = off[k]; t < off[k + 1]; t++) {
        const double w = wsrc[e[t]];
        s += wsquare ? w * w : w;
    }
    diag[rw] = d - s;
}

__global__ void k_bcr_add_dead(const int *__restrict__ dead, double *__restrict__ sum) {
    if (threadIdx.x == 0 && blockIdx.x == 0) *sum += (double)*dead;
}

template <int B>
__global__ __launch_bounds__(256) void k_bcr_top_closure_S(int r, int npad, int nst, const double *__restrict__ recR,
                                                            const double *__restrict__ recW, const double *__restrict__ Ttop,
                                                            double *__restrict__ S, double *__restrict__ T,
                                                            const double *__restrict__ deadx) {
    __shared__ double sx[16][65], sy[16][65];
    if (blockIdx.x < blockIdx.y) return;
    const int tp = threadIdx.x >> 4, tq = threadIdx.x & 15;
    const int p = blockIdx.y * 16 + tp, q = blockIdx.x * 16 + tq;
// ... 215 lines not shown
    std::vector<int4> steps((size_t)r * nst);
    for (int q = 0; q <= r; q++) off[(size_t)q] = q * nst;
    for (int q = 0; q < r; q++)
        for (int d = 0; d < nst; d++) {
            steps[(size_t)q * nst + d] = prog[(size_t)d];
            owner[(size_t)q * nst + d] = q;
        }
    for (int d = 0; d <= nst; d++) eoff[(size_t)d] = d * r;
    for (int d = 0; d < nst; d++)
        for (int q = 0; q < r; q++) erec[(size_t)d * r + q] = q * nst + d;
    hipStream_t st = g0.stream;
    T.cl_off.upload(off, st);
    T.cl_step.upload(steps, st);
    T.cl_owner.upload(owner, st);
    T.co_off.upload(eoff, st);
    T.co_rec.upload(erec, st);
    T.co_elim.upload(elim, st);
    T.xbuf.alloc(T.x_doubles());
    T.Dinv.alloc((size_t)7 * B * B);
    T.topDinv.alloc((size_t)B * B);
    T.recR.alloc((size_t)r * nst * B);
    T.recW.alloc((size_t)r * nst * B);
    T.Ttop.alloc((size_t)r * 3);
    T.lam.alloc((size_t)T.npad * 3);
    T.dead.alloc(1);
    IRH_CHECK(hipMemsetAsync(T.topDinv.p, 0, sizeof(double) * (size_t)B * B, st));
    IRH_CHECK(hipMemsetAsync(T.xbuf.p, 0, sizeof(double) * T.x_doubles(), st));
    IRH_CHECK(hipStreamSynchronize(st));
}
#define IRH_BCR_DISPATCH(fn, ...)              \
    switch (g.bcr_B) {                         \
    case 8: fn<8>(__VA_ARGS__); break;         \
    case 16: fn<16>(__VA_ARGS__); break;       \
    case 24: fn<24>(__VA_ARGS__); break;       \
    default: fn<32>(__VA_ARGS__); break;       \
    }
void bcr_shard_reduce(Graph &g, BcrTop &T, int rank) {
    bcr_alloc(g);
    IRH_BCR_DISPATCH(bcr_shard_reduce_t, g, T, rank)
}
void bcr_top_solve(Graph &g, BcrTop &T) { IRH_BCR_DISPATCH(bcr_top_solve_t, g, T) }
void bcr_shard_back(Graph &g, BcrTop &T, int rank) {
    IRH_BCR_DISPATCH(bcr_shard_back_t, g, T, rank)
    g.stats.direct_solves += 1;
}
void bcr_shard_closures_forward(Graph &g, BcrTop &T, int rank) { IRH_BCR_DISPATCH(bcr_shard_closures_forward_t, g, T, rank) }
void bcr_top_solve_closures(Graph &g, BcrTop &T) { IRH_BCR_DISPATCH(bcr_top_solve_closures_t, g, T) }
void bcr_shard_closures_correct(Graph &g, BcrTop &T) { IRH_BCR_DISPATCH(bcr_shard_closures_correct_t, g, T) }

int bcr_solve(Graph &g, int only) {
    if (!g.bcr_B) return IROTAVG_ERR_BAD_ARG;
    bcr_alloc(g);
    switch (g.bcr_B) {
    case 8: bcr_run_all<8>(g, only); break;
    case 12: bcr_run_all<12>(g, only); break;
    case 16: bcr_run_all<16>(g, only); break;
    case 20: bcr_run_all<20>(g, only); break;
    case 24: bcr_run_all<24>(g, only); break;
    case 28: bcr_run_all<28>(g, only); break;
    case 32: bcr_run_all<32>(g, only); break;
    default: return IROTAVG_ERR_BAD_ARG;
    }
    if (only < 0) g.stats.direct_solves += 1;
    return IROTAVG_OK;
}

__global__ __launch_bounds__(256) void k_bcr_residual(int n, const int *__restrict__ sl_off, const int *__restrict__ col,
                                                       const double *__restrict__ val, const double *__restrict__ diag,
                                                       const double4 *__restrict__ rhs, const double4 *__restrict__ X,
                                                       double *__restrict__ part) {
    const int row = blockIdx.x * 256 + threadIdx.x;
    double r0 = 0.0, r1 = 0.0, r2 = 0.0, b0 = 0.0, b1 = 0.0, b2 = 0.0;
    if (row < n) {
        const int sl = row >> 6, ln = row & 63;
        const int o0 = sl_off[sl], w = sl_off[sl + 1] - o0;
        const v2i *__restrict__ cp = reinterpret_cast<const v2i *>(col) + (size_t)(o0 / 2) * 64 + ln;
        const v2d *__restrict__ vp = reinterpret_cast<const v2d *>(val) + (size_t)(o0 / 2) * 64 + ln;
        const double4 x = X[row], bb = rhs[row];
        const double d = diag[row];
        double s0 = d * x.x, s1 = d * x.y, s2 = d * x.z;
        for (int q = 0; q < w / 2; q++) {
            const v2i cc = cp[(size_t)q * 64];
            const v2d vv = vp[(size_t)q * 64];
#pragma unroll
            for (int h = 0; h < 2; h++) {
                const double v = h ? vv.y : vv.x;
                const int c = h ? cc.y : cc.x;
                if (v != 0.0) {
                    const double4 xc = X[c];
                    s0 += v * xc.x;
                    s1 += v * xc.y;
                    s2 += v * xc.z;
                }
            }
        }
        r0 = (bb.x - s0) * (bb.x - s0);
        r1 = (bb.y - s1) * (bb.y - s1);
        r2 = (bb.z - s2) * (bb.z - s2);
        b0 = bb.x * bb.x;
        b1 = bb.y * bb.y;
        b2 = bb.z * bb.z;
    }
    block_sum3_store(r0, r1, r2, part + 8 * blockIdx.x);
    __syncthreads();
    block_sum3_store(b0, b1, b2, part + 8 * blockIdx.x + 4);
}

int bcr_residual(Graph &g, double *relres) {
    if (!g.bcr_B || g.stats.direct_solves == 0 || g.levels.empty()) return IROTAVG_ERR_BAD_ARG;
    if (g.ng > 0 || g.bcr_shard) return IROTAVG_ERR_BAD_ARG;
    if (g.bcr_last_guarded) {
        for (int c = 0; c < 3; c++) relres[c] = g.stats.last_relres[c];
        return IROTAVG_OK;
    }
    Level &L0 = g.levels[0];
    const int grid = (L0.n + 255) / 256;
    DevBuf<double> part;
    part.alloc((size_t)grid * 8);
    hipLaunchKernelGGL(k_bcr_residual, dim3(grid), dim3(256), 0, g.stream, L0.n, L0.sl_off.p, L0.col.p, L0.val.p, L0.diag.p,
                       L0.b.p, g.X.p, part.p);
    IRH_CHECK(hipGetLastError());
    std::vector<double> h((size_t)grid * 8);
    IRH_CHECK(hipMemcpyAsync(h.data(), part.p, sizeof(double) * h.size(), hipMemcpyDeviceToHost, g.stream));
    IRH_CHECK(hipStreamSynchronize(g.stream));
    double rr[3] = {0, 0, 0}, bb[3] = {0, 0, 0};
    for (int b = 0; b < grid; b++)
        for (int c = 0; c < 3; c++) {
            rr[c] += h[(size_t)b * 8 + c];
            bb[c] += h[(size_t)b * 8 + 4 + c];
        }
    for (int c = 0; c < 3; c++) {
        relres[c] = bb[c] > 0.0 ? std::sqrt(rr[c] / bb[c]) : (rr[c] > 0.0 ? HUGE_VAL : 0.0);
        g.stats.last_relres[c] = relres[c];
    }
    return IROTAVG_OK;
}

int bcr_info(Graph &g, int64_t *out, int cap) {
    int k = 0;
    auto put = [&](int64_t v) {
        if (k < cap) out[k++] = v;
    };
    put(g.bcr_B);
    if (!g.bcr_B) return k;
    bcr_alloc(g);
    put((int64_t)g.bcr->lev.size());
    for (const BcrLevel &L : g.bcr->lev) {
        put(L.nb);
        put(L.nch);
        put(L.nred);
    }
    put(g.bcr->nfar);
    put(g.bcr_asm_fused_last ? 1 : 0);
    return k;
}

int bcr_stamps_up(Graph &g, double *out) {
    if (!g.bcr_B) return IROTAVG_ERR_BAD_ARG;
    bcr_alloc(g);
    BcrState &S = *g.bcr;
    struct DbgScope {
        BcrState &S;
        ~DbgScope() { S.dbg_word = -1; }
    } dbg_scope{S};
    S.dbg_word = 128 + 256 * g.sw.bcr_stamp_chunk;
    const size_t cnt = (size_t)std::max(S.lev[0].nch * 16, 32 * kUpLevels);
    if (!S.stamps.p) S.stamps.alloc(cnt);
    IRH_CHECK(hipMemsetAsync(S.stamps.p, 0, sizeof(long long) * cnt, g.stream));
    const int rc = bcr_solve(g, -1);
    S.dbg_word = -1;
    if (rc != IROTAVG_OK) return rc;
    long long h[32 * kUpLevels];
    IRH_CHECK(hipMemcpyAsync(h, S.stamps.p, sizeof(h), hipMemcpyDeviceToHost, g.stream));
    IRH_CHECK(hipStreamSynchronize(g.stream));
    bcr_up_release(g);
    for (int k = 0; k < 32 * kUpLevels; k++) out[k] = !h[k] ? -1.0 : (k & 31) >= 20 ? (double)h[k] : (double)(h[k] - h[16]);
    return S.up_used ? IROTAVG_OK : IROTAVG_ERR_BAD_ARG;
}

int bcr_stamps(Graph &g, int level, int chunk, double *out) {
    if (!g.bcr_B) return IROTAVG_ERR_BAD_ARG;
    bcr_alloc(g);
    BcrState &S = *g.bcr;
    if (level < 0 || level >= (int)S.lev.size() || chunk < 0 || chunk >= S.lev[level].nch) return IROTAVG_ERR_BAD_ARG;
    struct DbgScope {
        BcrState &S;
        ~DbgScope() { S.dbg_word = -1; }
    } dbg_scope{S};
    S.dbg_word = 64;
    if (!S.stamps.p) S.stamps.alloc((size_t)S.lev[0].nch * 16);
    IRH_CHECK(hipMemsetAsync(S.stamps.p, 0, sizeof(long long) * (size_t)S.lev[0].nch * 16, g.stream));
    const int rc = bcr_solve(g, level);
    S.dbg_word = -1;
    if (rc != IROTAVG_OK) return rc;
    long long h[16];
    IRH_CHECK(hipMemcpyAsync(h, S.stamps.p + (size_t)chunk * 16, sizeof(h), hipMemcpyDeviceToHost, g.stream));
    IRH_CHECK(hipStreamSynchronize(g.stream));
    for (int k = 0; k < 16; k++) out[k] = h[k] ? (double)(h[k] - h[0]) : -1.0;
    return IROTAVG_OK;
}

__global__ __launch_bounds__(256) void k_bcr_resid_norms(int n, const double4 *__restrict__ b, const double4 *__restrict__ Ax,
                                                          double *__restrict__ part) {
    const int row = blockIdx.x * 256 + threadIdx.x;
    double r0 = 0.0, r1 = 0.0, r2 = 0.0, b0 = 0.0, b1 = 0.0, b2 = 0.0;
    if (row < n) {
        const double4 bb = b[row], a = Ax[row];
        r0 = (bb.x - a.x) * (bb.x - a.x);
        r1 = (bb.y - a.y) * (bb.y - a.y);
        r2 = (bb.z - a.z) * (bb.z - a.z);
        b0 = bb.x * bb.x;
        b1 = bb.y * bb.y;
        b2 = bb.z * bb.z;
    }
    block_sum3_store(r0, r1, r2, part + 8 * blockIdx.x);
    __syncthreads();
    block_sum3_store(b0, b1, b2, part + 8 * blockIdx.x + 4);
}

__global__ __launch_bounds__(256) void k_bcr_gate(int *__restrict__ dead, int *__restrict__ flags,
                                                  const double *__restrict__ part, int nparts, double tol2,
                                                  int *__restrict__ skip_out, int *__restrict__ flags_copy) {
    __shared__ double sh[4][6];
    const int t = threadIdx.x;
    double a[6] = {0, 0, 0, 0, 0, 0};
    if (part)
        for (int b = t; b < nparts; b += 256) {
            for (int c = 0; c < 3; c++) {
                a[c] += part[(size_t)b * 8 + c];
                a[3 + c] += part[(size_t)b * 8 + 4 + c];
            }
        }
    for (int c = 0; c < 6; c++) {
        double v = a[c];
        for (int o = 32; o > 0; o >>= 1) v += __shfl_xor(v, o);
        if ((t & 63) == 0) sh[t >> 6][c] = v;
    }
    __syncthreads();
    if (t != 0) return;
    bool ok = true;
    if (part) {
        for (int c = 0; c < 6; c++) a[c] = sh[0][c] + sh[1][c] + sh[2][c] + sh[3][c];
        for (int c = 0; c < 3; c++) ok = ok && (a[c] <= tol2 * a[3 + c]);
    }
    const int d = dead ? dead[0] : 0;
    flags[FL_DONE] = d == 0 && ok ? 1 : 0;
    flags[FL_ITERS] = d == 0 && !ok ? 1 : 0;
    flags[3] = d;
    if (dead) dead[0] = 0;
    if (skip_out) skip_out[0] = d == 0 && ok ? 0 : 1;
    if (flags_copy) {
        flags_copy[FL_DONE] = d == 0 && ok ? 1 : 0;
        flags_copy[FL_ITERS] = d == 0 && !ok ? 1 : 0;
        flags_copy[FL_STALE] = 0;
        flags_copy[3] = d;
    }
}
const int *bcr_gate_skip_word(Graph &g) {
    BcrState *S = g.bcr.get();
    if (!S) return nullptr;
    if (!S->gate_skip.p) {
        S->gate_skip.alloc(1);
        S->gate_skip.zero(g.stream);
    }
    return S->gate_skip.p;
}
void bcr_gate(Graph &g, double *flags_copy) {
    BcrState *S = g.bcr.get();
    int *dead = S && S->nfar > 0 ? S->dead.p : nullptr;
    if (dead) S->dead_clean = true;
    const double *part = nullptr;
    int grid = 0;
    if (S && S->nfar > 0 && g.ng == 0 && !g.bcr_shard) {
        Level &L0 = g.levels[0];
        grid = (L0.n + 255) / 256;
        if (S->res_part.n < (size_t)grid * 8) {
            S->res_part.alloc((size_t)grid * 8);
            S->res_zero.alloc(FL_COUNT);
            S->res_zero.zero(g.stream);
        }
        launch_spmv(g, g.X.p, nullptr, S->res_zero.p);
        hipLaunchKernelGGL(k_bcr_resid_norms, dim3(grid), dim3(256), 0, g.stream, L0.n, L0.b.p, g.AP.p, S->res_part.p);
        part = S->res_part.p;
    }
    const double gate = std::max(g.opt.pcg_rtol, kBcrGateTolMin);
    const double tol = g.sw.bcr_fake_give_up ? -1.0 : gate * gate;
    int *skip_out = (S && flags_copy) ? const_cast<int *>(bcr_gate_skip_word(g)) : nullptr;
    hipLaunchKernelGGL(k_bcr_gate, dim3(1), dim3(256), 0, g.stream, dead, g.flags.p, part, grid, tol, skip_out,
                       reinterpret_cast<int *>(flags_copy));
}

int bcr_closures(Graph &g) { return g.bcr_B ? (int)g.bcr_far_e.size() : 0; }

int bcr_apply_slots(Graph &g) {
    if (!g.bcr_B || !g.bcr_far_e.empty() || g.bcr_shard || g.ng != 0) return 0;
    bcr_alloc(g);
    const BcrState &S = *g.bcr;
    if (S.lev.size() < 2 || S.nfar != 0) return 0;
    const int slots = S.lev[0].nch + (S.top16 && S.lev.size() == 2 ? 0 : S.lev[1].nch);
    return slots <= 4 * kMaxParts ? slots : 0;
}

const int *bcr_fail_word(Graph &g) {
    if (!g.bcr || !g.bcr->up_used || g.bcr->up_cnt.n < (size_t)kUpLevels + 1) return nullptr;
    return reinterpret_cast<const int *>(g.bcr->up_cnt.p + kUpLevels);
}
bool bcr_up_failed(Graph &g) {
    const int *w = bcr_fail_word(g);
    if (!w) return false;
    int h = 0;
    if (hipMemcpyAsync(&h, w, sizeof(int), hipMemcpyDeviceToHost, g.stream) != hipSuccess) return false;
    if (hipStreamSynchronize(g.stream) != hipSuccess) return false;
    if (!h) return false;
    (void)hipMemsetAsync(const_cast<int *>(w), 0, sizeof(int), g.stream);
    g.bcr_no_fused_up = true;
    g.stats.direct_up_fallbacks += 1;
    bcr_up_release(g);
    return true;
}

int bcr_levels(Graph &g) {
    if (!g.bcr_B) return 0;
    bcr_alloc(g);
    return (int)g.bcr->lev.size();
}

constexpr int kBcrMaxFar = 2048;

bool bcr_band_part_anchored(int64_t m, int f, int64_t nu, int B, const int32_t *I) {
    std::vector<int> parent((size_t)nu);
    for (int64_t r = 0; r < nu; r++) parent[(size_t)r] = (int)r;
    std::vector<uint8_t> anch((size_t)nu, 0);
    auto find = [&](int x) {
        while (parent[(size_t)x] != x) {
            parent[(size_t)x] = parent[(size_t)parent[(size_t)x]];
            x = parent[(size_t)x];
        }
        return x;
    };
    for (int64_t k = 0; k < m; k++) {
        const int i = I[2 * k], j = I[2 * k + 1];
        if (i >= f && j >= f) {
            if (i == j) continue;
            if (std::abs(i - j) > 32 && std::abs((i - f) / B - (j - f) / B) >= 2) continue;
            const int a = find(i - f), b = find(j - f);
            if (a != b) parent[(size_t)std::max(a, b)] = std::min(a, b);
        } else if (i < f && j >= f) {
            anch[(size_t)(j - f)] = 1;
        }
    }
    for (int64_t r = 0; r < nu; r++)
        if (anch[(size_t)r]) anch[(size_t)find((int)r)] = 1;
    for (int64_t r = 0; r < nu; r++)
        if (!anch[(size_t)find((int)r)]) return false;
    return true;
}

static bool bcr_plan_begin(Graph &g, int *mode) {
    g.bcr_B = 0;
    g.band0 = -1;
    g.bcr_far_i.clear();
    g.bcr_far_j.clear();
    g.bcr_far_e.clear();
    *mode = g.sw.has_band_direct ? g.sw.band_direct : g.opt.band_direct;
    return *mode >= 0 && g.ng == 0 && g.no >= 1;
}
static int bcr_plan_block(Graph &g, int mode, int band, int bandall, long long nfar) {
    g.band0 = bandall;
    if (nfar > (g.no < 8192 ? kBcrMaxFar / 2 : kBcrMaxFar)) return 0;
    if (mode == 0 && g.no <= 2048) return 0;
    return band <= 8 ? 8 : (band + 3) / 4 * 4;
}

void bcr_plan(Graph &g, const int32_t *I) {
    int mode = 0;
    if (!bcr_plan_begin(g, &mode)) return;
    const int f = g.f;
    std::atomic<int> band(0), bandall(0);
    std::atomic<long long> nfar(0);
    std::atomic<bool> bad(false);
    const int64_t nt = g.n_total;
    parallel_for(g.m, 65536, [&](int64_t k0, int64_t k1, int) {
        int bmax = 0, ball = 0;
        long long far = 0;
        for (int64_t k = k0; k < k1; k++) {
            const int i = I[2 * k], j = I[2 * k + 1];
            if (i < 0 || j < 0 || i >= nt || j >= nt) {
                bad = true;
                return;
            }
            if (i >= f && j >= f) {
                const int d = std::abs(i - j);
                ball = std::max(ball, d);
                if (d <= 32) bmax = std::max(bmax, d);
                else far++;
            }
        }
        int cur = band.load();
        while (bmax > cur && !band.compare_exchange_weak(cur, bmax)) {
        }
        cur = bandall.load();
        while (ball > cur && !bandall.compare_exchange_weak(cur, ball)) {
        }
        nfar += far;
    });
    if (bad.load()) return;
    const int B = bcr_plan_block(g, mode, band.load(), bandall.load(), nfar.load());
    if (!B) return;
    if (nfar.load() > 0) {
        for (int64_t k = 0; k < g.m; k++) {
            const int i = I[2 * k], j = I[2 * k + 1];
            if (i >= f && j >= f && std::abs(i - j) > 32 && std::abs((i - f) / B - (j - f) / B) >= 2) {
                g.bcr_far_i.push_back(i - f);
                g.bcr_far_j.push_back(j - f);
                g.bcr_far_e.push_back((int)k);
            }
        }
        bool refuse = !g.bcr_far_e.empty() && g.sw.bcr_no_closures;
        if (!g.bcr_far_e.empty() && !refuse) {
            std::vector<uint8_t> ok((size_t)g.no, 0);
            parallel_for(g.m, 65536, [&](int64_t k0, int64_t k1, int) {
                for (int64_t k = k0; k < k1; k++) {
                    const int i = I[2 * k], j = I[2 * k + 1];
                    if (i >= f && j >= f) {
                        if (i != j && std::abs(i - j) <= 32) ok[(size_t)(std::max(i, j) - f)] = 1;
                    } else if (i < f && j >= f) {
                        ok[(size_t)(j - f)] = 1;
                    }
                }
            });
            for (int r = 0; r < g.no && !refuse; r++) refuse = !ok[(size_t)r];
            if (refuse) refuse = !bcr_band_part_anchored(g.m, f, g.no, B, I);
        }
        if (refuse) {
            g.bcr_far_i.clear();
            g.bcr_far_j.clear();
            g.bcr_far_e.clear();
            return;
        }
    }
    g.bcr_B = B;
}

namespace {
__global__ __launch_bounds__(256) void k_plan_stats(long long m, int f, int nt, const int2 *__restrict__ I,
                                                    const int *__restrict__ relabel, int *__restrict__ out,
                                                    unsigned long long *__restrict__ nfar) {
    __shared__ int sb[3][4];
    __shared__ unsigned long long sf[4];
    int band = 0, ball = 0, bad = 0;
    unsigned long long far = 0;
    for (long long k = (long long)blockIdx.x * 256 + threadIdx.x; k < m; k += (long long)gridDim.x * 256) {
        const int2 e = I[k];
        int i = e.x, j = e.y;
        if (i < 0 || j < 0 || i >= nt || j >= nt) {
            bad = 1;
            continue;
        }
        if (relabel) {
            i = relabel[i];
            j = relabel[j];
        }
        if (i >= f && j >= f) {
            const int d = abs(i - j);
            ball = max(ball, d);
            if (d <= 32) band = max(band, d);
            else far++;
        }
    }
    for (int o = 32; o >= 1; o >>= 1) {
        band = max(band, __shfl_xor(band, o));
        ball = max(ball, __shfl_xor(ball, o));
// ... 104 lines not shown
```

### irotavg_amd/csrc/capi.cpp

```cpp
#include <atomic>
#include <cmath>
#include <mutex>
#include <new>
#include <vector>

#include "graph.hpp"
#include "marginals.hpp"
#include "winbatch.hpp"

using namespace irh;

struct irotavg_graph {
    Graph g;
};

#define API_TRY try {
#define API_CATCH                          \
    }                                      \
    catch (const HipError &) {             \
        return IROTAVG_ERR_HIP;            \
    }                                      \
    catch (const std::bad_alloc &) {       \
        return IROTAVG_ERR_NOMEM;          \
    }                                      \
// ... 64 lines not shown
        bool grew = false;
        for (int64_t k = 0; k < m; k++) {
            const int64_t a = I[2 * k], b = I[2 * k + 1];
            if (a < 0 || b < 0 || a >= n || b >= n) return IROTAVG_ERR_BAD_ARG;
            if (seen[a] && !seen[b]) {
                if (b >= f) {
                    const double qq[4] = {QQ[k], QQ[ldqq + k], QQ[2 * ldqq + k], QQ[3 * ldqq + k]};
                    const double qa[4] = {Q[a], Q[ldq + a], Q[2 * ldq + a], Q[3 * ldq + a]};
                    double r[4];
                    h_qmul(qq, qa, r);
                    for (int c = 0; c < 4; c++) Q[c * ldq + b] = r[c];
                }
                seen[b] = 1;
                count++;
                grew = true;
            } else if (!seen[a] && seen[b]) {
                if (a >= f) {
                    const double qq[4] = {QQ[k], QQ[ldqq + k], QQ[2 * ldqq + k], -QQ[3 * ldqq + k]};
                    const double qb[4] = {Q[b], Q[ldq + b], Q[2 * ldq + b], Q[3 * ldq + b]};
                    double r[4];
                    h_qmul(qq, qb, r);
                    for (int c = 0; c < 4; c++) Q[c * ldq + a] = r[c];
                }
                seen[a] = 1;
                count++;
                grew = true;
            }
        }
        if (!grew && count < n) return IROTAVG_ERR_NOT_SPANNING;
    }
    return IROTAVG_OK;
}

int64_t irotavg_make_A(int n, int f, int64_t m, const int32_t *I, int64_t *colptr,
                       int64_t *rowidx, double *vals) {
    if (n < 0 || f < 0 || n - f <= 1 || !I || !colptr || !rowidx || !vals)
        return IROTAVG_ERR_BAD_ARG;
    const int64_t nu = (int64_t)n - f;
    std::vector<int64_t> cnt((size_t)nu + 1, 0);
    auto row = [&](int64_t k, int64_t c[2], double v[2]) -> int {
        const int64_t j = (int64_t)I[2 * k + 1] - f, i = (int64_t)I[2 * k] - f;
        if (j < 0) return 0;
        if (i < 0) {
            c[0] = j;
            v[0] = 1.0;
            return 1;
        }
        if (i == j) {
            c[0] = i;
            v[0] = -1.0;
            return 1;
        }
        c[0] = j;
        v[0] = 1.0;
        c[1] = i;
        v[1] = -1.0;
        return 2;
    };
    int64_t c[2];
    double v[2];
    for (int64_t k = 0; k < m; k++) {
        const int ne = row(k, c, v);
        for (int e = 0; e < ne; e++) {
            if (c[e] >= nu) return IROTAVG_ERR_BAD_ARG;
            cnt[c[e]]++;
        }
    }
    colptr[0] = 0;
    for (int64_t q = 0; q < nu; q++) colptr[q + 1] = colptr[q] + cnt[q];
    for (int64_t q = 0; q < nu; q++) cnt[q] = colptr[q];
    for (int64_t k = 0; k < m; k++) {
        const int ne = row(k, c, v);
        for (int e = 0; e < ne; e++) {
            const int64_t p = cnt[c[e]]++;
            rowidx[p] = k;
            vals[p] = v[e];
        }
    }
    return colptr[nu];
}

}

int irh::graph_create(irotavg_graph **out, int64_t m, int64_t n_total, int f, const int32_t *I, const double *QQ,
                      int64_t ldqq, const irotavg_options *opt, const DevEdgeSrc *src, const Switches &sw) {
    if (!out || (src ? !src->I || !src->qq : !I || !QQ || ldqq < m) || m <= 0 || n_total <= 0 || f < 0 || n_total - f < 1 ||
        n_total > 0x7fffffffLL)
        return IROTAVG_ERR_BAD_ARG;
    *out = nullptr;
    if (irotavg_device_count() <= 0) return IROTAVG_ERR_NO_DEVICE;
    irotavg_graph *h = nullptr;
    API_TRY
    h = new irotavg_graph();
    Graph &g = h->g;
    g.sw = sw;
    if (opt)
        g.opt = *opt;
    else
        irotavg_default_options(&g.opt);
    if (g.opt.pcg_rtol <= 0) g.opt.pcg_rtol = 1e-10;
    if (g.opt.mg_omega <= 0) g.opt.mg_omega = 0.7;
    if (g.opt.mg_levels_max <= 0) g.opt.mg_levels_max = 16;
    if (g.opt.pcg_max_iters <= 0) g.opt.pcg_max_iters = 2000;
    if (g.opt.pcg_check_every <= 0) g.opt.pcg_check_every = 8;
    if (g.opt.device >= 0) IRH_CHECK(hipSetDevice(g.opt.device));
    IRH_CHECK(hipGetDevice(&g.device));
    g.stream = StreamPool::get().take();
    g.m = m;
    g.n_total = n_total;
    g.f = f;
    g.nu = (int)(n_total - f);
    g.ng = 0;
    g.no = g.nu;
    if (src && src->ordered) order_streams(g, src->caller, g.stream, true);
    if (src)
        bcr_plan_dev(g, *src);
    else
        bcr_plan(g, I);
    if (g.bcr_B) g.opt.mg_levels_max = 1;
    const int rc = src ? build_graph_device(g, nullptr, nullptr, 0, src) : build_graph(g, I, QQ, ldqq);
    if (rc != IROTAVG_OK) {
        irotavg_graph_destroy(h);
        return rc;
    }
    *out = h;
    return IROTAVG_OK;
    }
    catch (const HipError &) {
        if (h) irotavg_graph_destroy(h);
        return IROTAVG_ERR_HIP;
    }
    catch (const std::bad_alloc &) {
        if (h) irotavg_graph_destroy(h);
        return IROTAVG_ERR_NOMEM;
    }
    catch (...) {
        if (h) irotavg_graph_destroy(h);
        return IROTAVG_ERR_HIP;
    }
}

Graph &irh::graph_of(irotavg_graph *h) { return h->g; }

extern "C" {

int irotavg_graph_create(irotavg_graph **out, int64_t m, int64_t n_total, int f, const int32_t *I,
                         const double *QQ, int64_t ldqq, const irotavg_options *opt) {
    return graph_create(out, m, n_total, f, I, QQ, ldqq, opt, nullptr, read_switches());
}

int64_t irotavg_trim_memory(void) {
    try {
        StreamPool::get().trim();
        return (int64_t)DevPool::get().trim();
    } catch (...) {
        return 0;
    }
}

void irotavg_graph_destroy(irotavg_graph *h) {
    if (!h) return;
    const bool timing = h->g.sw.build_timing;
    double t0 = now_seconds();
    auto lap = [&](const char *what) {
        if (!timing) return;
        const double t = now_seconds();
        std::fprintf(stderr, "[irotavg_hip destroy] %-24s %8.3f ms\n", what, 1e3 * (t - t0));
        t0 = t;
    };
    hipStream_t s = h->g.stream;
    const int dev = h->g.device;
    if (s) (void)hipStreamSynchronize(s);
    lap("sync");
    release_l1_clones(h->g);
    lap("clones");
    h->g.stream = nullptr;
    delete h;
    lap("delete");
    if (s) StreamPool::get().give(s, dev);
    lap("stream destroy");
}

int irotavg_graph_set_rotations(irotavg_graph *h, const double *Q, int64_t ldq) {
    if (!h || !Q || ldq < h->g.n_total) return IROTAVG_ERR_BAD_ARG;
    API_TRY
    Graph &g = h->g;
    std::vector<double4> aos((size_t)g.n_total);
    parallel_for(g.n_total, 8192, [&](int64_t a, int64_t b, int) {
        for (int64_t i = a; i < b; i++) aos[i] = make_double4(Q[i], Q[ldq + i], Q[2 * ldq + i], Q[3 * ldq + i]);
    });
    g.Q.upload(aos.data(), aos.size(), g.stream);
    IRH_CHECK(hipStreamSynchronize(g.stream));
    return IROTAVG_OK;
    API_CATCH
}

int irotavg_graph_get_rotations(irotavg_graph *h, double *Q, int64_t ldq) {
    if (!h || !Q || ldq < h->g.n_total) return IROTAVG_ERR_BAD_ARG;
    API_TRY
    Graph &g = h->g;
    std::vector<double4> aos((size_t)g.n_total);
    IRH_CHECK(hipMemcpyAsync(aos.data(), g.Q.p, sizeof(double4) * aos.size(), hipMemcpyDeviceToHost,
                             g.stream));
    IRH_CHECK(hipStreamSynchronize(g.stream));
    parallel_for(g.n_total, 8192, [&](int64_t a, int64_t b, int) {
        for (int64_t i = a; i < b; i++) {
            Q[i] = aos[i].x;
            Q[ldq + i] = aos[i].y;
            Q[2 * ldq + i] = aos[i].z;
            Q[3 * ldq + i] = aos[i].w;
        }
    });
    return IROTAVG_OK;
    API_CATCH
}

int irotavg_graph_snapshot_rotations(irotavg_graph *h) {
    if (!h) return IROTAVG_ERR_BAD_ARG;
    API_TRY
    Graph &g = h->g;
    if (g.Qsnap.n < (size_t)g.n_total) g.Qsnap.alloc((size_t)g.n_total);
    IRH_CHECK(hipMemcpyAsync(g.Qsnap.p, g.Q.p, sizeof(double4) * (size_t)g.n_total,
                             hipMemcpyDeviceToDevice, g.stream));
    IRH_CHECK(hipStreamSynchronize(g.stream));
    return IROTAVG_OK;
    API_CATCH
}

int irotavg_graph_restore_rotations(irotavg_graph *h) {
    if (!h || h->g.Qsnap.n < (size_t)h->g.n_total) return IROTAVG_ERR_BAD_ARG;
    API_TRY
    Graph &g = h->g;
    IRH_CHECK(hipMemcpyAsync(g.Q.p, g.Qsnap.p, sizeof(double4) * (size_t)g.n_total,
                             hipMemcpyDeviceToDevice, g.stream));
    return IROTAVG_OK;
    API_CATCH
}

int irotavg_graph_get_weights(irotavg_graph *h, double *w) {
    if (!h || !w) return IROTAVG_ERR_BAD_ARG;
    API_TRY
    Graph &g = h->g;
    IRH_CHECK(hipMemcpyAsync(w, g.dw.p, sizeof(double) * (size_t)g.m, hipMemcpyDeviceToHost, g.stream));
    IRH_CHECK(hipStreamSynchronize(g.stream));
    return IROTAVG_OK;
    API_CATCH
}

int irotavg_graph_set_weights(irotavg_graph *h, const double *w) {
    if (!h || !w) return IROTAVG_ERR_BAD_ARG;
    API_TRY
    Graph &g = h->g;
    IRH_CHECK(hipMemcpyAsync(g.dw.p, w, sizeof(double) * (size_t)g.m, hipMemcpyHostToDevice, g.stream));
    IRH_CHECK(hipStreamSynchronize(g.stream));
    return IROTAVG_OK;
    API_CATCH
}

int irotavg_graph_irls(irotavg_graph *h, int cost, double sigma, int max_iters, double change_th,
                       int *iters, double *runtime, double *trace) {
    if (!h || !iters || !runtime) return IROTAVG_ERR_BAD_ARG;
    API_TRY
    return run_irls(h->g, cost, sigma, max_iters, change_th, iters, runtime, trace);
    API_CATCH
}

int irotavg_graph_l1ra(irotavg_graph *h, int max_iters, double change_th, int *iter, double *runtime,
                       double *trace) {
    if (!h || !iter || !runtime) return IROTAVG_ERR_BAD_ARG;
    API_TRY
    return run_l1ra(h->g, max_iters, change_th, iter, runtime, trace);
    API_CATCH
}

int irotavg_graph_quat_normalised(irotavg_graph *h) {
    if (!h) return IROTAVG_ERR_BAD_ARG;
    API_TRY
    normalise_rotations(h->g);
    IRH_CHECK(hipStreamSynchronize(h->g.stream));
    return IROTAVG_OK;
    API_CATCH
}

int irotavg_graph_get_stats(irotavg_graph *h, irotavg_stats *out) {
    if (!h || !out) return IROTAVG_ERR_BAD_ARG;
    *out = h->g.stats;
    out->band = h->g.band0;
    out->band_block = h->g.bcr_B;
    return IROTAVG_OK;
}

int irotavg_graph_direct_info(irotavg_graph *h, int64_t *info, int cap) {
    if (!h || !info || cap < 1) return IROTAVG_ERR_BAD_ARG;
    API_TRY
    return bcr_info(h->g, info, cap);
    API_CATCH
}

static bool variance_args_ok(int64_t n_total, int64_t npairs, const int32_t *pairs, const double *pair_var) {
    if (npairs < 0 || (npairs > 0 && (!pairs || !pair_var))) return false;
    for (int64_t t = 0; t < 2 * npairs; t++)
        if (pairs[t] < 0 || pairs[t] >= n_total) return false;
    return true;
}

int irotavg_graph_rotation_variance(irotavg_graph *h, double *var, int64_t npairs, const int32_t *pairs,
// ... 586 lines not shown
```

### irotavg_amd/csrc/graph.hpp

```cpp
#pragma once
#include <functional>
#include <memory>

#include "common.hpp"
#include "hostwait.hpp"

namespace irh {

struct Graph;
void bcr_up_release(Graph &g) noexcept;
struct BcrState;
struct BcrDeleter {
    void operator()(BcrState *p) const;
};

struct Graph {
    int64_t m = 0, n_total = 0, mpad = 0;
    int f = 0, nu = 0, ng = 0, no = 0;
    irotavg_options opt{};
    Switches sw;
    hipStream_t stream = nullptr;
    int device = 0;

    DevBuf<int> ei, ej;
    DevBuf<uint8_t> eflag;
    DevBuf<double> qq;
    DevBuf<double> er;
    DevBuf<double> dw;
    DevBuf<double4> T;
    DevBuf<double4> Q;
    DevBuf<double4> Qsnap;

    DevBuf<uint8_t> slot_cs;
    DevBuf<int> tile_e0;
    int asm_windowed = 1;
    int asm_l1_fused = 0;
    DevBuf<uint32_t> slot_eid;
    DevBuf<int> bptr;
    DevBuf<uint32_t> beid;
    DevBuf<uint8_t> bflag;
    DevBuf<int> bghost;
    DevBuf<double> bval;
    DevBuf<double4> PG;

    std::vector<Level> levels;
    DevBuf<double> dense_inv;
    DevBuf<double> dense_wr, dense_wc;
    DevBuf<double> dense_chol;
    DevBuf<double> dense_wb;
    int dense_repairs_in_a_row = 0;
    DevBuf<double> dense_la;
    int ndense = 0, ndense_pad = 0;
    int dense_bw = 0;
    bool dense_valid = false, dense_fresh = false;
    int64_t its_fresh = 0;
    bool asm_check_stale = false, asm_check_done = false;
    DevBuf<unsigned long long> dense_mm;
    int stale_streak = 0;
    unsigned stale_skips = 0;
    bool dense_stale_pending = false;
    double dense_scale = 1.0, stale_spread = 1.1;
    DevBuf<double> dense_ref_diag, dense_ref_val;
    struct DenseSlot {
        DevBuf<double> inv, ref_diag, ref_val;
        double scale = 1.0;
        bool valid = false;
    };
    std::vector<DenseSlot> dense_parked;
    int dense_slot = 0;
    DevBuf<double> dense_maxdiag;
    int additive_top = 1;

    DevBuf<double4> X, P, AP;
    bool kc_auto = false;
    int l1_fused = 0;
    int cg2 = 0;
    long long l0_far_entries = 0;
    DevBuf<double> b2p;
    DevBuf<double4> R2;
    DevBuf<double4> P2;
    DevBuf<double> part_pq, part_rr, part_rz, part_rz2, part_score;
    DevBuf<double> scal;
    DevBuf<int> flags;

    DevBuf<double> pd;
    DevBuf<double> pdn;
    DevBuf<double> pd_part;
    bool pd_ready = false;
    const double *pd_rhs_src = nullptr;
    bool pd_rhs_done = false;
    std::vector<std::unique_ptr<Graph>> l1_clones;
    bool is_clone = false;

    double *hpin = nullptr;
    double *h_part() { return hpin; }
    double *h_scal() { return hpin + 4 * kMaxParts; }
    int *h_flags() { return reinterpret_cast<int *>(hpin + 4 * kMaxParts + SC_COUNT); }
    int *h_seq() { return reinterpret_cast<int *>(hpin + 8192); }
    int pub_seq = 0;
    hipEvent_t ev_in = nullptr, ev_out = nullptr;
    ~Graph() {
        bcr_up_release(*this);
        if (ev_in) (void)hipEventDestroy(ev_in);
        if (ev_out) (void)hipEventDestroy(ev_out);
        if (hpin) PinPool::get().give(hpin);
    }
    Graph() = default;
    Graph(const Graph &) = delete;
    Graph &operator=(const Graph &) = delete;

    int bcr_B = 0, band0 = -1;
    bool bcr_apply = false, bcr_applied = false;
    int bcr_up_held = 0;
    bool pool_headroom = false;
    bool bcr_no_fused_up = false;
    bool bcr_asm_fused = false, bcr_asm_fused_last = false;
    std::unique_ptr<BcrState, BcrDeleter> bcr;
    std::vector<int> bcr_far_i, bcr_far_j, bcr_far_e;
    const double *bcr_wsrc = nullptr;
    int bcr_wsquare = 0;
    bool bcr_guard = false;
    bool bcr_last_guarded = false;
    double4 *bcr_out = nullptr;
    bool bcr_shard = false;
    int bcr_ext0 = 0;
    std::vector<int> bcr_ghost_extcol;
    std::vector<int> bcr_far_gid;
    std::vector<uint8_t> bcr_far_own;
    std::vector<int> bcr_fix_row, bcr_fix_off, bcr_fix_e;

    double last_score_sum = 0.0;
    double irls_settle = -1.0;
    int force_np = 0;
    irotavg_stats stats{};
};

struct PrecInfo {
    int np_rz = 0, np_rz2 = 0;
};

struct BuildTail {
    int nlev = 1;
    int agg[kMaxLevels] = {0};
    int dense_bw = 0;
    bool l1_window_ok = false;
    bool l1_band8 = false;
};
struct HierPlan {
    std::vector<int> n, agg;
};
HierPlan plan_hierarchy(Graph &g, int n0, int64_t nnz0, bool far0);
struct DevEdgeSrc {
    const int2 *I = nullptr;
    const double *qq = nullptr;
    long long qq_rs = 4, qq_cs = 1;
    const int *relabel = nullptr;
    bool ordered = false;
    hipStream_t caller = nullptr;
};
int build_graph(Graph &g, const int32_t *I, const double *QQ, int64_t ldqq);
int build_graph_host(Graph &g, const int32_t *I, const double *QQ, int64_t ldqq);
int build_graph_device(Graph &g, const int32_t *I, const double *QQ, int64_t ldqq, const DevEdgeSrc *src = nullptr);
int finish_build(Graph &g, const BuildTail &T);
void ingest_qq(Graph &g, const double *src, long long rs, long long cs);
void order_streams(Graph &g, hipStream_t from, hipStream_t to, bool in);

void launch_edge_residual(Graph &g, bool weights_to_one = false);
int ls_solve(Graph &g, const std::function<void()> *tail = nullptr, bool *tail_ran = nullptr);
void launch_update_weights(Graph &g, int cost, double sigma, bool gated = false);
void launch_apply_step(Graph &g, bool gated);
double finish_apply_step(Graph &g);
double apply_step(Graph &g, bool gated = false, const std::function<void()> *behind = nullptr);
struct PubPart {
    const double *src;
    double *dst;
    int n;
};
void publish_parts(Graph &g, const PubPart *parts, int nparts);
void wait_published(Graph &g);
int run_irls(Graph &g, int cost, double sigma, int max_iters, double change_th, int *iters,
             double *runtime, double *trace);
int run_l1ra(Graph &g, int max_iters, double change_th, int *iters, double *runtime,
             double *trace);
int l1decode_pd_dev(Graph &g, int coord_plane_from_er, const double *y_host, int pdmaxiter,
                    double *x_host, int *stuck, int out_component);
int time_kernel(Graph &g, int which, int reps, double *ms);
void release_l1_clones(Graph &g);
std::unique_ptr<Graph> make_solver_clone(Graph &g, hipStream_t stream);
void normalise_rotations(Graph &g);
void fill(Graph &g, double *p, long long n, double v);
void read_back_state(Graph &g);
void alloc_state(Graph &g);
void assemble(Graph &g, int mode, const double *wsrc, bool refresh_dense = true);
void assemble_values(Graph &g, int mode, const double *wsrc);
int pcg_solve(Graph &g, const std::function<void()> *tail = nullptr, bool *tail_ran = nullptr);
int pcg_solve_classic(Graph &g, const std::function<void()> *tail = nullptr, bool *tail_ran = nullptr);
void launch_spmv(Graph &g, const double4 *p = nullptr, const double4 *pg = nullptr, const int *flags = nullptr);
void launch_update(Graph &g, bool init, int par, int np_pq, const double4 *p = nullptr,
                   const double4 *rin = nullptr, double4 *rout = nullptr);
void launch_pupdate(Graph &g, int par, int first, const PrecInfo &pi, bool check = false, int np_rr = 1,
                    double rtol2 = 0.0);
PrecInfo precondition(Graph &g, int first, double rtol2, bool check = true);
void launch_form_u(Graph &g, double *part_g);
void launch_cgd_update(Graph &g, bool init, int par, int first, double rtol2, const double *part_g,
                       const double *part_d, const double *rr_in, double *rr_out);
int round_grid(long long gsz);
int grid_for_rows(const Level &L);
int grid_for_elems(long long n);
int normalise_host_rows(int64_t n, double *Q, int64_t ldq, int f);
struct PdMember {
    Graph *g;
    const uint8_t *eown;
    const double *y;
};
struct PdGroup {
    std::vector<PdMember> mem;
    long long m_global = 0;
    std::function<void(double *, int, int)> combine;
    std::function<void()> halo_x;
    std::function<int()> solve;
};
int l1decode_group(PdGroup &G, int pdmaxiter, int xplane, int *stuck);
void pd_prepare_graph(Graph &g);
void pd_pack_solution(Graph &g);
constexpr int kPdXPlane0 = 3;
constexpr int IROTAVG_RETRY_STALE = 100;
int pcg_solve_cg2(Graph &g, const std::function<void()> *tail = nullptr, bool *tail_ran = nullptr,
                  bool device_scale = false);
void cg2_time_once(Graph &g, int which);
int cg2_phase_stamps(Graph &g, double *out, int n);
void cycle_levels(Graph &g, int from);
struct WindowSolver;
WindowSolver *window_solver_new(const Switches &sw);
void window_solver_delete(WindowSolver *w);
bool window_fits(int nv, int f, int ne);
int window_solve(WindowSolver &ws, int nv, int f, int ne, const int32_t *I, const double *QQ_aos,
                 double *Q_aos, double *weights, int l1_max, int irls_max, int cost, double sigma,
                 double change_th, int *l1_iters, int *irls_iters, int kernel = 0);
bool window_fits_wave(int nv, int f, int ne);
struct WinBatchItem {
    int nv, f, ne;
    const int32_t *I;
    const double *QQ_aos;
    double *Q_aos;
    int l1_iters, irls_iters, status;
};
int window_solve_batch(WindowSolver &ws, int nb, WinBatchItem *items, int l1_max, int irls_max, int cost, double sigma,
                       double change_th);
struct WinBatchPlan;
struct WinBatchArrays {
    const int32_t *I;
    const double *QQ;
    long long qq_rs, qq_cs;
    double *Q;
    long long q_rs, q_cs;
    double *weights;
};
int window_solve_batch_dev(const WinBatchPlan &plan, int device, const WinBatchArrays &A, int cost, double sigma,
                           int l1_max, int irls_max, double change_th, int32_t *results, hipStream_t stream);
int window_init_mst_batch_dev(const WinBatchPlan &plan, int device, const WinBatchArrays &A, int32_t *results ,
                              hipStream_t stream);
struct CycleArrays {
    const int32_t *I;
    const double *QQ;
    long long qq_rs, qq_cs;
    int32_t *tri_count, *tri_ok;
    double *tri_min;
};
int cycle_check_dev(int64_t m, int64_t n_total, const CycleArrays &A, double threshold, int64_t *summary ,
                    hipStream_t stream);
int cycle_check_host(int64_t m, int64_t n_total, const CycleArrays &A, double threshold, int64_t *summary);
int cycle_check_group(int lanes);
struct WinCov;
WinCov *wincov_new();
void wincov_delete(WinCov *w);
struct WinCovQuery {
    int nv, f, ne;
    const int32_t *I;
    const double *qq_aos, *Q_aos;
    double sigma;
    const double *weights;
    double *var;
    double *edge_var, *leverage, *chi2;
    int np;
    const int32_t *prow;
    double *pair_var;
    int nc;
    const int32_t *crow;
    const double *cq;
    double *angle, *cand_var, *cand_chi2;
    double s2;
};
int wincov_query(WinCov &wc, WinCovQuery &q);
struct WinCovPlan;
struct WinCovArrays {
    const int32_t *I;
    const double *QQ;
    long long qq_rs, qq_cs;
    const double *Q;
    long long q_rs, q_cs;
    const double *weights;
    double *var;
    const int32_t *pairs;
    double *pair_var;
    double *edge_var, *leverage, *chi2;
    bool gate = false;
    const int32_t *cand = nullptr;
    const double *cand_QQ = nullptr;
    long long cq_rs = 0, cq_cs = 0;
    double *angle = nullptr, *cand_var = nullptr, *cand_chi2 = nullptr;
};
int wincov_batch_dev(const WinCovPlan &plan, int device, const WinCovArrays &A, double sigma, double *scale ,
                     int32_t *results , hipStream_t stream);
void launch_pose_weights(Graph &g, int cost, double sigma);
void candidate_angles(Graph &g, int64_t n, const double *q12, double *angle);
void bcr_plan(Graph &g, const int32_t *I);
void bcr_plan_dev(Graph &g, const DevEdgeSrc &src);
int bcr_solve(Graph &g, int only = -1);
int bcr_levels(Graph &g);
int bcr_info(Graph &g, int64_t *out, int cap);
int bcr_residual(Graph &g, double *relres);
int bcr_closures(Graph &g);
constexpr double kClosureRepairAccept = 1e-8;
bool bcr_band_part_anchored(int64_t m, int f, int64_t nu, int B, const int32_t *I);
int bcr_apply_slots(Graph &g);
void bcr_gate(Graph &g, double *flags_copy = nullptr);
const int *bcr_gate_skip_word(Graph &g);
void dense_invert_spd(Graph &g, double *A, int npad);
int bcr_stamps(Graph &g, int level, int chunk, double *out);
int bcr_stamps_up(Graph &g, double *out);
bool bcr_up_failed(Graph &g);
const int *bcr_fail_word(Graph &g);
struct BcrTop {
    int B = 0, world = 0;
    DevBuf<double> buf;
    DevBuf<double> rec;
    size_t record_doubles() const { return 3 * (size_t)B * B + 2 * (size_t)B * 3; }
    DevBuf<double> W, x, xtop;
    size_t n_doubles() const { return (size_t)world * (3 * (size_t)B * B + 2 * (size_t)B * 3); }
    int r = 0, npad = 0, nst = 0;
    DevBuf<double> xbuf, Dinv, topDinv, recR, recW, Ttop, lam;
    DevBuf<int> dead, cl_off, cl_owner, co_off, co_rec;
    DevBuf<int4> cl_step;
    DevBuf<int2> co_elim;
    size_t x_dep() const { return 0; }
    size_t x_S() const { return (size_t)r * world * B; }
    size_t x_T() const { return x_S() + (size_t)npad * npad; }
    size_t x_dead() const { return x_T() + (size_t)npad * 3; }
    size_t x_pivots() const { return x_dead() + (size_t)npad; }
    size_t x_doubles() const { return x_pivots() + 1; }
};
void bcr_top_alloc(BcrTop &T, int B, int world);
void bcr_top_to_record(BcrTop &T, int rank, hipStream_t st);
void bcr_top_from_records(BcrTop &T, hipStream_t st);
void bcr_shard_reduce(Graph &g, BcrTop &T, int rank);
void bcr_top_solve(Graph &g, BcrTop &T);
void bcr_shard_back(Graph &g, BcrTop &T, int rank);
void bcr_top_closures_alloc(Graph &g0, BcrTop &T, int r);
void bcr_shard_closures_forward(Graph &g, BcrTop &T, int rank);
void bcr_top_solve_closures(Graph &g, BcrTop &T);
void bcr_shard_closures_correct(Graph &g, BcrTop &T);
int rotation_variance(Graph &g, double *var, int64_t npairs, const int32_t *pairs, double *pair_var, double *scale,
                      double *var_dev = nullptr);
void dense_refresh(Graph &g);
void dense_select_slot(Graph &g, int slot);
bool dense_is_stale(Graph &g, bool allow_repair = false);
bool dense_rescale_only(Graph &g);
bool dense_direct_solve(Graph &g);
void dense_check_async(Graph &g);
int dense_apply_grid(const Graph &g);
void dense_apply(Graph &g, const double4 *b, double4 *y, bool check, bool dot, double *part_dot,
                 int np_rr, int first, double rtol2);

}
struct irotavg_graph;
namespace irh {
int graph_create(irotavg_graph **out, int64_t m, int64_t n_total, int f, const int32_t *I, const double *QQ, int64_t ldqq,
                 const irotavg_options *opt, const DevEdgeSrc *src, const Switches &sw);
Graph &graph_of(irotavg_graph *h);

struct Resident;
struct ResidentStage {
    double *R;
    uint8_t *fixed;
    int32_t *I;
    double *qq;
    double *Q;
};
Resident *resident_new();
void resident_delete(Resident *r);
void resident_invalidate(Resident &r);
long resident_views(const Resident &r);
long resident_edges(const Resident &r);
ResidentStage resident_stage(Resident &r, long n_views, long view_lo, long n_edges, long edge_lo);
int resident_rot_avg(Resident &r, long n_views, long view_lo, long n_edges, long edge_lo, int f,
                     const irotavg_options &opt, const Switches &sw, irotavg_rotavg_info &loc, bool timing, bool dry = false,
                     int dry_a = -1, int dry_b = -1);

int resident_build_handle(Resident &r, long n_views, long view_lo, long n_edges, long edge_lo, int f,
                          const irotavg_options &opt, const Switches &sw, irotavg_graph **out);

}
```

### irotavg_amd/csrc/solver.hip

```cpp
#include <cstring>

#include "graph.hpp"
#include "kernels.hpp"
#include "asm0w.hpp"

namespace irh {


__global__ __launch_bounds__(256) void k_edge_residual(long long mpad, const int *__restrict__ ei,
                                                       const int *__restrict__ ej,
                                                       const double *__restrict__ qq,
                                                       const double4 *__restrict__ Q,
                                                       double *__restrict__ er, double *__restrict__ ones) {
    const long long k = 2ll * ((long long)blockIdx.x * blockDim.x + threadIdx.x);
    if (k >= mpad) return;
    if (ones) *reinterpret_cast<double2 *>(ones + k) = make_double2(1.0, 1.0);
    const int2 ii = *reinterpret_cast<const int2 *>(ei + k);
    const int2 jj = *reinterpret_cast<const int2 *>(ej + k);
    const double2 qx = *reinterpret_cast<const double2 *>(qq + k);
    const double2 qy = *reinterpret_cast<const double2 *>(qq + mpad + k);
    const double2 qz = *reinterpret_cast<const double2 *>(qq + 2 * mpad + k);
    const double2 qw = *reinterpret_cast<const double2 *>(qq + 3 * mpad + k);
    const double4 qi0 = Q[ii.x], qj0 = Q[jj.x], qi1 = Q[ii.y], qj1 = Q[jj.y];
    double2 rx, ry, rz;
// ... 1789 lines not shown
        }
        if (cur < 0.5 * best) {
            best = cur;
            best_it = it;
        } else if (it - best_it >= kStallIters && cur <= accept) {
            stagnated = true;
            break;
        }
        if (it >= maxit) break;
        iteration_tail(pi);
    }
    g.stats.pcg_solves += 1;
    g.stats.pcg_iters += (stagnated || attained) ? it : h_flags[FL_ITERS];
    g.stats.pcg_iters_last = (stagnated || attained) ? it : h_flags[FL_ITERS];
    for (int c = 0; c < 3; c++) g.stats.last_relres[c] = h_scal[SC_RELRES + c];
    if (h_flags[FL_DONE] == 2) return IROTAVG_ERR_SOLVER;
    if (attained) return IROTAVG_OK;
    if (stagnated) {
        g.stats.pcg_stagnated += 1;
        return IROTAVG_OK;
    }
    if (h_flags[FL_DONE] == 0) return IROTAVG_ERR_NOT_CONVERGED;
    return IROTAVG_OK;
}

int ls_solve(Graph &g, const std::function<void()> *tail, bool *tail_ran) {
    if (tail_ran) *tail_ran = false;
    const bool fused_asm = g.bcr_B && (8 * g.bcr_B) % 64 == 0 && g.asm_windowed && g.bcr_far_e.empty() && !g.bcr_shard &&
                           g.ng == 0 && !g.bcr_no_fused_up && !g.sw.bcr_no_fused_asm;
    if (fused_asm) {
        g.bcr_wsrc = g.dw.p;
        g.bcr_wsquare = 1;
    } else {
        assemble(g, 0, g.dw.p, g.opt.dense_always_refresh == 1);
    }
    if (g.bcr_B) {
        g.bcr_last_guarded = false;
        g.bcr_asm_fused = fused_asm;
        struct Done {
            Graph &g;
            ~Done() {
                g.bcr_asm_fused_last = g.bcr_asm_fused;
                g.bcr_asm_fused = false;
            }
        } done{g};
        return bcr_solve(g);
    }
    int rc = pcg_solve(g, tail, tail_ran);
    auto failed = [&]() { return rc == IROTAVG_ERR_NOT_CONVERGED || rc == IROTAVG_ERR_SOLVER; };
    if (failed() && g.ndense > 0 && !g.dense_fresh) {
        assemble(g, 0, g.dw.p, true);
        rc = pcg_solve(g);
    }
    if (failed()) {
        assemble_values(g, 0, g.dw.p);
        if (dense_direct_solve(g)) {
            g.stats.pcg_stagnated += 1;
            rc = IROTAVG_OK;
        }
    }
    return rc;
}

__global__ __launch_bounds__(256) void k_publish(const double *__restrict__ s0, double *__restrict__ d0, int n0,
                                                 const double *__restrict__ s1, double *__restrict__ d1, int n1,
                                                 const double *__restrict__ s2, double *__restrict__ d2, int n2,
                                                 int *__restrict__ seqp, int seq) {
    for (int i = threadIdx.x; i < n0; i += 256) d0[i] = s0[i];
    for (int i = threadIdx.x; i < n1; i += 256) d1[i] = s1[i];
    for (int i = threadIdx.x; i < n2; i += 256) d2[i] = s2[i];
    __threadfence_system();
    __syncthreads();
    if (threadIdx.x == 0) __hip_atomic_store(seqp, seq, __ATOMIC_RELEASE, __HIP_MEMORY_SCOPE_SYSTEM);
}

void publish_begin(Graph &g) {
    next_seq(g.pub_seq);
    __atomic_store_n(g.h_seq(), 0, __ATOMIC_RELEASE);
}
void publish_parts(Graph &g, const PubPart *parts, int nparts) {
    PubPart p[3] = {{nullptr, nullptr, 0}, {nullptr, nullptr, 0}, {nullptr, nullptr, 0}};
    for (int i = 0; i < nparts && i < 3; i++) p[i] = parts[i];
    publish_begin(g);
    hipLaunchKernelGGL(k_publish, dim3(1), dim3(256), 0, g.stream, p[0].src, p[0].dst, p[0].n, p[1].src, p[1].dst,
                       p[1].n, p[2].src, p[2].dst, p[2].n, g.h_seq(), g.pub_seq);
    IRH_CHECK(hipGetLastError());
}

void wait_published(Graph &g) {
    static const bool no_poll = env_no_poll();
    if (no_poll || !wait_seq(g.h_seq(), 0, 1, g.pub_seq, 2e-3, 100e-6)) IRH_CHECK(hipStreamSynchronize(g.stream));
}

void launch_apply_step(Graph &g, bool gated) {
    const int n = g.nu;
    const int grid = grid_for_elems(n);
    hipLaunchKernelGGL(k_apply_step, dim3(grid), dim3(kRowBlock), 0, g.stream, n, g.f, g.ng, g.X.p,
                       g.Q.p, g.part_score.p, 1, gated ? (const int *)g.flags.p : (const int *)nullptr);
    IRH_CHECK(hipMemcpyAsync(g.h_part(), g.part_score.p, sizeof(double) * 4 * (size_t)grid,
                             hipMemcpyDeviceToHost, g.stream));
}
double finish_apply_step(Graph &g) {
    const int grid = grid_for_elems(g.nu);
    double s = 0.0;
    for (int b = 0; b < grid; b++) s += g.h_part()[4 * (size_t)b];
    g.last_score_sum = s;
    return s / (double)g.no;
}
double apply_step(Graph &g, bool gated, const std::function<void()> *behind) {
    const int n = g.nu;
    const int grid = grid_for_elems(n);
    hipLaunchKernelGGL(k_apply_step, dim3(grid), dim3(kRowBlock), 0, g.stream, n, g.f, g.ng, g.X.p, g.Q.p,
                       g.part_score.p, 1, gated ? (const int *)g.flags.p : (const int *)nullptr);
    PubPart part[2] = {{g.part_score.p, g.h_part(), 4 * grid},
                       {reinterpret_cast<const double *>(g.flags.p), reinterpret_cast<double *>(g.h_flags()), FL_COUNT / 2}};
    publish_parts(g, part, gated ? 2 : 1);
    if (behind) (*behind)();
    wait_published(g);
    return finish_apply_step(g);
}

int run_irls(Graph &g, int cost, double sigma, int max_iters, double change_th, int *iters,
             double *runtime, double *trace) {
    if (cost < IROTAVG_L2 || cost > IROTAVG_WELSCH) return IROTAVG_ERR_UNKNOWN_COST;
    const double tic = now_seconds();
    double score = HUGE_VAL;
    int it = 0, rc = IROTAVG_OK;
    if (!(score > change_th && 0 < max_iters)) fill(g, g.dw.p, (long long)g.mpad, 1.0);
    const bool fuse_wr = g.bcr_B && g.ng == 0 && !g.bcr_shard;
    bool er_fresh = false;
    bool with_res = true;
    const std::function<void()> wr_tail = [&]() { launch_weights_then_residual(g, cost, sigma, nullptr, with_res); };
    const int ap_slots = fuse_wr ? bcr_apply_slots(g) : 0;
    while (score > change_th && it < max_iters) {
        if (!er_fresh) launch_edge_residual(g, it == 0);
        er_fresh = false;
        const double rtol_keep = g.opt.pcg_rtol;
        if (!g.bcr_B && (it == 0 || score > 50.0 * change_th) && it + 1 < max_iters) {
            const bool on = g.sw.inexact >= 0 ? g.sw.inexact != 0 : g.opt.inexact_outer == 1;
            if (on) {
                const double last = it == 0 ? 1.0 : score;
                g.opt.pcg_rtol = std::max(rtol_keep, std::min(1e-4, 0.01 * change_th / last));
            }
        }
        struct Restore {
            double &r, v;
            ~Restore() { r = v; }
        } restore_rtol{g.opt.pcg_rtol, rtol_keep};
        if (g.bcr_B) {
            const double score_before = score;
            g.bcr_apply = ap_slots > 0;
            g.bcr_applied = false;
            with_res = !(it + 1 >= max_iters || (it > 0 && score <= 50.0 * change_th));
            rc = ls_solve(g);
            g.bcr_apply = false;
            if (rc != IROTAVG_OK) break;
            if (bcr_closures(g) > 0) {
                const int sgrid = grid_for_elems(g.nu);
                const bool fuse_cl = fuse_wr && 4 * sgrid + 2 <= 4 * kMaxParts && !g.sw.no_fused_cl;
                if (fuse_cl) {
                    bcr_gate(g, g.part_score.p + 4 * (size_t)sgrid);
                    hipLaunchKernelGGL(k_apply_step, dim3(sgrid), dim3(kRowBlock), 0, g.stream, g.nu, g.f, g.ng, g.X.p, g.Q.p,
                                       g.part_score.p, 1, (const int *)g.flags.p);
                    const PubPart part = {g.part_score.p, g.h_part(), 4 * sgrid + 2};
                    publish_begin(g);
                    launch_weights_then_residual(g, cost, sigma, &part, with_res, bcr_gate_skip_word(g));
                    wait_published(g);
                    std::memcpy(g.h_flags(), g.h_part() + 4 * (size_t)sgrid, sizeof(int) * FL_COUNT);
                    score = finish_apply_step(g);
                    er_fresh = with_res && g.h_flags()[FL_DONE] == 1;
                } else {
                    bcr_gate(g);
                    launch_update_weights(g, cost, sigma, true);
                    score = apply_step(g, true);
                }
                if (g.h_flags()[FL_DONE] != 1) {
                    const bool inexact_only = g.h_flags()[FL_ITERS] == 1 && g.h_flags()[3] == 0;
                    g.stats.direct_guarded += 1;
                    g.stats.direct_dead_pivots = g.h_flags()[3];
                    {
                        struct GuardScope {
                            Graph &g;
                            const int64_t ds_keep;
                            const int maxit_keep;
                            ~GuardScope() {
                                g.opt.pcg_max_iters = maxit_keep;
                                g.bcr_guard = false;
                                g.stats.direct_solves = ds_keep;
                            }
                        } guard_scope{g, g.stats.direct_solves, g.opt.pcg_max_iters};
                        g.bcr_guard = true;
                        if (inexact_only) g.opt.pcg_max_iters = 12;
                        rc = pcg_solve_classic(g);
                    }
                    g.bcr_last_guarded = true;
                    if (inexact_only && rc == IROTAVG_ERR_NOT_CONVERGED) {
                        g.stats.pcg_stagnated += 1;
                        rc = IROTAVG_OK;
                    }
                    if (rc == IROTAVG_OK && inexact_only) {
                        const double worst = std::max(g.stats.last_relres[0], std::max(g.stats.last_relres[1], g.stats.last_relres[2]));
                        if (!(worst <= kClosureRepairAccept)) rc = IROTAVG_ERR_SOLVER;
                    }
                    if (g.sw.bcr_fake_give_up) rc = IROTAVG_ERR_SOLVER;
                    if (rc != IROTAVG_OK) break;
                    launch_update_weights(g, cost, sigma);
                    score = apply_step(g);
                }
            } else if (fuse_wr && g.bcr_applied) {
                const PubPart part = {g.part_score.p, g.h_part(), ap_slots};
                publish_begin(g);
                launch_weights_then_residual(g, cost, sigma, &part, with_res);
                wait_published(g);
                double ssum = 0.0;
                for (int b = 0; b < ap_slots; b++) ssum += g.h_part()[b];
                g.last_score_sum = ssum;
                score = ssum / (double)g.no;
                er_fresh = with_res;
            } else if (fuse_wr) {
                score = apply_step(g, false, &wr_tail);
                er_fresh = with_res;
            } else {
                launch_update_weights(g, cost, sigma);
                score = apply_step(g);
            }
            if (!std::isfinite(score)) {
                if (bcr_up_failed(g)) {
                    er_fresh = true;
                    score = score_before;
                    continue;
                }
                rc = IROTAVG_ERR_SOLVER;
                break;
            }
        } else if (g.cg2) {
            g.asm_check_stale = g.ndense > 0 && g.dense_valid && !g.dense_stale_pending && g.opt.dense_always_refresh != 1;
            g.asm_check_done = false;
            assemble_values(g, 0, g.dw.p);
            g.asm_check_stale = false;
            bool spec = false;
            if (g.ndense > 0) {
                if (!g.dense_valid || g.dense_stale_pending || g.opt.dense_always_refresh == 1) {
                    dense_refresh(g);
                    g.dense_valid = true;
                    g.dense_fresh = true;
                    g.dense_stale_pending = false;
                } else {
                    if (!g.asm_check_done) dense_check_async(g);
                    g.dense_fresh = false;
                    spec = true;
                }
            }
            bool tail_ran = false;
            const std::function<void()> tail = [&]() {
                launch_update_weights(g, cost, sigma, true);
                launch_apply_step(g, true);
            };
            rc = pcg_solve_cg2(g, &tail, &tail_ran, spec);
            if (spec) {
                if (g.h_flags()[FL_STALE]) {
                    const int64_t slack = (g.dense_bw >= 1 && g.dense_bw <= kBandMax) ? 4 : 8;
                    g.dense_stale_pending = rc != IROTAVG_OK || g.its_fresh <= 0 ||
                                            g.stats.pcg_iters_last > g.its_fresh + slack;
                } else {
                    g.dense_scale = g.h_scal()[SC_DSCALE];
                }
            } else if (rc == IROTAVG_OK && g.ndense > 0) {
                g.its_fresh = g.stats.pcg_iters_last;
            }
            if (rc == IROTAVG_RETRY_STALE) {
                dense_refresh(g);
                g.dense_valid = true;
                g.dense_fresh = true;
                g.dense_stale_pending = false;
                IRH_CHECK(hipMemcpyAsync(g.levels[0].b.p, g.levels[0].x.p, sizeof(double4) * (size_t)g.levels[0].n,
                                         hipMemcpyDeviceToDevice, g.stream));
                rc = pcg_solve_cg2(g, &tail, &tail_ran, false);
                if (rc == IROTAVG_OK) g.its_fresh = g.stats.pcg_iters_last;
            }
            if ((rc == IROTAVG_ERR_NOT_CONVERGED || rc == IROTAVG_ERR_SOLVER) && g.ndense > 0 && !g.dense_fresh) {
                dense_refresh(g);
                g.dense_valid = true;
                g.dense_fresh = true;
                g.dense_stale_pending = false;
                IRH_CHECK(hipMemcpyAsync(g.levels[0].b.p, g.levels[0].x.p, sizeof(double4) * (size_t)g.levels[0].n,
                                         hipMemcpyDeviceToDevice, g.stream));
                tail_ran = false;
                rc = pcg_solve_classic(g);
                if (rc == IROTAVG_OK) g.its_fresh = 0;
            }
            if (rc != IROTAVG_OK) break;
            if (tail_ran) {
                score = finish_apply_step(g);
            } else {
                launch_update_weights(g, cost, sigma);
                score = apply_step(g);
            }
        } else {
            g.irls_settle = (!g.sw.no_settle && it > 0 && score <= 20.0 * change_th) ? score : -1.0;
            bool tail_ran = false;
            const std::function<void()> tail = [&]() {
                launch_update_weights(g, cost, sigma, true);
                launch_apply_step(g, true);
            };
            rc = ls_solve(g, &tail, &tail_ran);
            if (rc != IROTAVG_OK) break;
            if (tail_ran) {
                score = finish_apply_step(g);
            } else {
                launch_update_weights(g, cost, sigma);
                score = apply_step(g);
            }
        }
        if (trace) trace[it] = score;
        it++;
    }
    g.irls_settle = -1.0;
    IRH_CHECK(hipStreamSynchronize(g.stream));
    bcr_up_release(g);
    const double toc = now_seconds();
    *iters = it;
    *runtime = toc - tic;
    g.stats.outer_iters += it;
    g.stats.edge_updates += (int64_t)it * g.m;
    g.stats.seconds_irls += toc - tic;
    return rc;
}

int time_kernel(Graph &g, int which, int reps, double *ms) {
    if (which >= 100 && which < 116) {
        if (!g.cg2) return IROTAVG_ERR_BAD_ARG;
        double st[16];
        const int rc = cg2_phase_stamps(g, st, 16);
        *ms = st[which - 100];
        return rc;
    }
    if (which >= 600 && which < 600 + 32 * 8) {
        double st[32 * 8];
        const int rc = bcr_stamps_up(g, st);
        *ms = st[which - 600];
        return rc;
    }
    if (which >= 200 && which < 200 + 16 * 16) {
        double st[16];
        const int rc = bcr_stamps(g, (which - 200) / 16, g.sw.bcr_stamp_chunk, st);
        *ms = st[(which - 200) % 16];
        return rc;
    }
    hipEvent_t e0, e1;
    IRH_CHECK(hipEventCreate(&e0));
    IRH_CHECK(hipEventCreate(&e1));
    auto once = [&]() {
        switch (which) {
        case 1: launch_edge_residual(g); break;
        case 2: launch_update_weights(g, IROTAVG_GEMAN_MCCLURE, 5 * IRH_PI / 180.0); break;
        case 3: assemble_values(g, 0, g.dw.p); break;
        case 7: dense_refresh(g); break;
        case 4:
            launch_spmv(g);
            break;
        case 5: (void)precondition(g, 0, -1.0); break;
        case 8: {
            Level &L0 = g.levels[0];
            hipLaunchKernelGGL((k_pspmv_dot<false, false>), dim3(grid_for_rows(L0)), dim3(kRowBlock), 0, g.stream,
                               view_of(L0), __builtin_ctz((unsigned)L0.agg), g.scal.p, 0, g.part_rz.p, 1,
                               g.part_rz2.p, 1, L0.b.p, g.levels[1].y.p, g.opt.mg_omega, g.opt.mg_kc, g.P.p,
                               g.P2.p, g.AP.p, g.part_pq.p, g.flags.p);
            break;
        }
        case 9: cg2_time_once(g, 0); break;
        case 10: cg2_time_once(g, 1); break;
        case 11: launch_weights_then_residual(g, IROTAVG_GEMAN_MCCLURE, 5 * IRH_PI / 180.0, nullptr, true); break;
        case 12: launch_pose_weights(g, IROTAVG_GEMAN_MCCLURE, 5 * IRH_PI / 180.0); break;
        case 6:
            hipLaunchKernelGGL(k_apply_step, dim3(grid_for_elems(g.nu)), dim3(kRowBlock), 0, g.stream,
                               g.nu, g.f, g.ng, g.X.p, g.Q.p, g.part_score.p, 0, (const int *)nullptr);
            break;
        default:
            if (which == 19) (void)bcr_solve(g);
            else if (which >= 20 && which < 40) (void)bcr_solve(g, which - 20);
            else if (which >= 40 && which < 60) (void)bcr_solve(g, 100 + which - 40);
            break;
        }
    };
    if (which >= 19 && which < 60) {
        if (!g.bcr_B) return IROTAVG_ERR_BAD_ARG;
        const int nl = bcr_levels(g);
        if ((which >= 20 && which < 40 && which - 20 >= nl) || (which >= 40 && which - 40 >= nl)) return IROTAVG_ERR_BAD_ARG;
    } else if (which < 1 || which > 12) return IROTAVG_ERR_BAD_ARG;
    if ((which == 9 || which == 10) && !g.cg2) return IROTAVG_ERR_BAD_ARG;
    if (which == 8 && !(g.additive_top && g.levels.size() > 1 && g.ng == 0 && g.l0_far_entries == 0 &&
                        g.opt.no_fused_pspmv != 1))
        return IROTAVG_ERR_BAD_ARG;
    IRH_CHECK(hipMemsetAsync(g.flags.p, 0, sizeof(int) * FL_COUNT, g.stream));
    DevBuf<double> keep_dw, keep_er;
    if (which == 11 || which == 12) {
        keep_dw.alloc((size_t)g.mpad);
        keep_er.alloc((size_t)3 * g.mpad);
        IRH_CHECK(hipMemcpyAsync(keep_dw.p, g.dw.p, sizeof(double) * (size_t)g.mpad, hipMemcpyDeviceToDevice, g.stream));
        IRH_CHECK(hipMemcpyAsync(keep_er.p, g.er.p, sizeof(double) * 3 * (size_t)g.mpad, hipMemcpyDeviceToDevice, g.stream));
    }
    once();
    IRH_CHECK(hipEventRecord(e0, g.stream));
    for (int r = 0; r < reps; r++) once();
    IRH_CHECK(hipEventRecord(e1, g.stream));
    if (which == 11 || which == 12) {
        IRH_CHECK(hipMemcpyAsync(g.dw.p, keep_dw.p, sizeof(double) * (size_t)g.mpad, hipMemcpyDeviceToDevice, g.stream));
        IRH_CHECK(hipMemcpyAsync(g.er.p, keep_er.p, sizeof(double) * 3 * (size_t)g.mpad, hipMemcpyDeviceToDevice, g.stream));
        IRH_CHECK(hipStreamSynchronize(g.stream));
    }
    IRH_CHECK(hipEventSynchronize(e1));
    bcr_up_release(g);
    float t = 0.f;
    IRH_CHECK(hipEventElapsedTime(&t, e0, e1));
    *ms = (double)t / std::max(reps, 1);
    (void)hipEventDestroy(e0);
    (void)hipEventDestroy(e1);
    return IROTAVG_OK;
}

}
```

### irotavg_amd/csrc/switches.hpp

```cpp
#pragma once
#include <algorithm>
#include <cstdlib>
#include <tuple>

namespace irh {

struct Switches {
    bool has_band_direct = false;
    int band_direct = 0;
    int host_build = -1;
    int upload_threads = 4;
    bool asm_classic = false, no_small_tuning = false;
    bool no_dense_refine = false, no_band_inverse = false, pcg_trace = false;
    int cg2_giveup = 0;
    bool no_settle = false, no_fused_cl = false;
    int inexact = -1;
    bool bcr_no_mixed = false, bcr_no_top16 = false, bcr_fake_up_fail = false, bcr_fake_give_up = false;
    bool bcr_no_closures = false, bcr_s_tiles = false, bcr_no_fused_asm = false;
    int bcr_up_cap = 1024;
    int bcr_dbg = 0, bcr_stamp_chunk = 0;
    bool dist_no_closures = false, dist_halo_p2p = false;
    bool no_resident = false, window_stamps = false;
    long resident_min_edges = 20000;
    bool build_timing = false, rotavg_timing = false;
};

inline Switches read_switches() {
    Switches s;
    auto set = [](const char *name) { return std::getenv(name) != nullptr; };
    auto num = [](const char *name, int unset) {
        const char *e = std::getenv(name);
        return e ? std::atoi(e) : unset;
    };
    s.has_band_direct = set("IROTAVG_BAND_DIRECT");
    s.band_direct = num("IROTAVG_BAND_DIRECT", 0);
    s.host_build = set("IROTAVG_HOST_BUILD") ? (num("IROTAVG_HOST_BUILD", 0) != 0 ? 1 : 0) : -1;
    s.upload_threads = std::min(4, std::max(0, num("IROTAVG_UPLOAD_THREADS", 4)));
    s.asm_classic = set("IROTAVG_ASM_CLASSIC");
    s.no_small_tuning = set("IROTAVG_NO_SMALL_TUNING");
    s.no_dense_refine = set("IROTAVG_NO_DENSE_REFINE");
    s.no_band_inverse = set("IROTAVG_NO_BAND_INVERSE");
    s.pcg_trace = set("IROTAVG_PCG_TRACE");
    s.cg2_giveup = set("IROTAVG_CG2_GIVEUP") ? std::max(1, num("IROTAVG_CG2_GIVEUP", 0)) : 0;
    s.no_settle = set("IROTAVG_NO_SETTLE");
    s.no_fused_cl = set("IROTAVG_NO_FUSED_CL");
    s.inexact = set("IROTAVG_INEXACT") ? (num("IROTAVG_INEXACT", 0) != 0 ? 1 : 0) : -1;
    s.bcr_no_mixed = set("IROTAVG_BCR_NO_MIXED");
    s.bcr_no_top16 = set("IROTAVG_BCR_NO_TOP16");
    s.bcr_fake_up_fail = set("IROTAVG_BCR_FAKE_UP_FAIL");
    s.bcr_fake_give_up = set("IROTAVG_BCR_FAKE_GIVE_UP");
    s.bcr_no_closures = set("IROTAVG_BCR_NO_CLOSURES");
    s.bcr_s_tiles = set("IROTAVG_BCR_S_TILES");
    s.bcr_no_fused_asm = set("IROTAVG_BCR_NO_FUSED_ASM");
    s.bcr_up_cap = num("IROTAVG_BCR_UP_CAP", 1024);
    s.bcr_dbg = num("IROTAVG_BCR_DBG", 0);
    s.bcr_stamp_chunk = num("IROTAVG_BCR_STAMP_CHUNK", 0);
    s.dist_no_closures = set("IROTAVG_DIST_NO_CLOSURES");
    s.dist_halo_p2p = set("IROTAVG_DIST_HALO_P2P");
    s.no_resident = set("IROTAVG_NO_RESIDENT");
    s.window_stamps = set("IROTAVG_WINDOW_STAMPS");
    if (const char *e = std::getenv("IROTAVG_RESIDENT_MIN_EDGES")) s.resident_min_edges = std::atol(e);
    s.build_timing = set("IROTAVG_BUILD_TIMING");
    s.rotavg_timing = set("IROTAVG_ROTAVG_TIMING");
    return s;
}

inline bool operator==(const Switches &a, const Switches &b) {
    auto t = [](const Switches &s) {
        return std::make_tuple(
            s.has_band_direct, s.band_direct, s.host_build, s.upload_threads, s.asm_classic, s.no_small_tuning,
            s.no_dense_refine, s.no_band_inverse, s.pcg_trace, s.cg2_giveup, s.no_settle, s.no_fused_cl, s.inexact,
            s.bcr_no_mixed, s.bcr_no_top16, s.bcr_fake_up_fail, s.bcr_fake_give_up, s.bcr_no_closures, s.bcr_s_tiles,
            s.bcr_no_fused_asm,             s.bcr_up_cap, s.bcr_dbg, s.bcr_stamp_chunk, s.dist_no_closures, s.dist_halo_p2p, s.no_resident, s.window_stamps,
            s.resident_min_edges, s.build_timing, s.rotavg_timing);
    };
    return t(a) == t(b);
}

inline const char *env_pool_limit_mb() { return std::getenv("IROTAVG_POOL_LIMIT_MB"); }
inline bool env_pin_default() { return std::getenv("IROTAVG_PIN_DEFAULT") != nullptr; }
inline bool env_no_poll() { return std::getenv("IROTAVG_NO_POLL") != nullptr || env_pin_default(); }
inline bool env_oneshot_cache() {
    const char *e = std::getenv("IROTAVG_ONESHOT_CACHE");
    return !(e && std::atoi(e) == 0);
}
inline int env_build_threads() {
    const char *e = std::getenv("IROTAVG_BUILD_THREADS");
    return e ? std::min(16, std::max(1, std::atoi(e))) : 0;
}

}
```

Baseline: 7.626 billion.

## Cache unit-weight BCR factorization and reuse it for right-hand-side-only solves

During the first IRLS iteration, when the weights are all one, the block cyclic reduction stores its per-level pivot inverses, coupling blocks and top-level operators in new device buffers. A later solve with unit weights can then run a right-hand-side-only reduction and back-substitution from the stored factor instead of refactoring. The stored factor is tied to an epoch counter so a memory trim invalidates it, and it is dropped if the solve result is not finite. In exchange it uses extra device memory and adds global stores to the factoring pass.

```diff
diff --git a/irotavg_amd/capi.py b/irotavg_amd/capi.py
--- a/irotavg_amd/capi.py
+++ b/irotavg_amd/capi.py
@@ -419,11 +419,15 @@
         if k < 0:
             raise IrotavgError(k, "direct_info")
         if out[0] == 0:
-            return dict(block=0, levels=[], closures=0, fused_assembly=0)
+            return dict(block=0, levels=[], closures=0, fused_assembly=0, unit_factor=0, unit_factor_solves=0,
+                        unit_factor_bytes=0)
         nl = int(out[1])
         return dict(block=int(out[0]), levels=[dict(blocks=int(out[2 + 3 * l]), chunks=int(out[3 + 3 * l]),
                                                     reduced=int(out[4 + 3 * l])) for l in range(nl)],
-                    closures=int(out[2 + 3 * nl]), fused_assembly=int(out[3 + 3 * nl]) if k > 3 + 3 * nl else 0)
+                    closures=int(out[2 + 3 * nl]), fused_assembly=int(out[3 + 3 * nl]) if k > 3 + 3 * nl else 0,
+                    unit_factor=int(out[4 + 3 * nl]) if k > 4 + 3 * nl else 0,
+                    unit_factor_solves=int(out[5 + 3 * nl]) if k > 5 + 3 * nl else 0,
+                    unit_factor_bytes=int(out[6 + 3 * nl]) if k > 6 + 3 * nl else 0)
 
     def direct_residual(self):
         out = np.zeros(3)
diff --git a/irotavg_amd/csrc/bcr.hip b/irotavg_amd/csrc/bcr.hip
--- a/irotavg_amd/csrc/bcr.hip
+++ b/irotavg_amd/csrc/bcr.hip
@@ -34,6 +34,7 @@
     int nb, nred, nch;
     gp_cd inD, inR, inXD, inXR, inXG;
     gp_d W, sepD, sepR, extD, extR, extG;
+    gp_d stD, stP, stQ;
 };
 struct BcrUpArgs {
     int nl;
@@ -48,6 +49,7 @@
     BcrTopSched top;
     gp_d xtop_all;
     gp_i fail;
+    gp_d tst;
 };
 
 struct BcrLevel {
@@ -58,7 +60,29 @@
     DevBuf<double> sepD, sepR, extD, extR, extG;
     DevBuf<double> x;
 };
+constexpr int kTopUnitLast = 5 * 4 * kTopRounds;
+struct BcrUnitLevel {
+    DevBuf<double> Wu, Di, P, Q;
+};
+struct BcrUnit {
+    std::vector<BcrUnitLevel> lev;
+    DevBuf<double> top;
+    DevBuf<BcrUpArgs> up_args;
+    bool valid = false;
+    int last = 0;
+    unsigned epoch = 0;
+    int64_t solves = 0, bytes = 0;
+    void release() {
+        lev.clear();
+        top.release();
+        up_args.release();
+        valid = false;
+        last = 0;
+        bytes = 0;
+    }
+};
 struct BcrState {
+    BcrUnit unit;
     int B = 0;
     int NR = 3;
     int nfar = 0;
@@ -507,7 +531,7 @@
                            __HIP_MEMORY_SCOPE_AGENT);
 }
 
-template <int B, int NR, bool L0, bool TOP, int NW, bool COH>
+template <int B, int NR, bool L0, bool TOP, int NW, bool COH, int UF = 0>
 __device__ __forceinline__ void bcr_reduce_body(
     const int chunk, double (*sDG)[B * B], double (*sR)[B * NR], double *sZ,
 
@@ -519,7 +543,7 @@
     int nfar, const int *__restrict__ far_i, const int *__restrict__ far_j, int ext0, const int *__restrict__ bptr,
     const int *__restrict__ bghost, const double *__restrict__ bval, const int *__restrict__ ghost_extcol, int place,
     long long *__restrict__ stamps, double *__restrict__ Dinvg, double *__restrict__ topDinv, int *__restrict__ deadctr,
-    int reg) {
+    int reg, double *__restrict__ stP = nullptr, double *__restrict__ stQ = nullptr) {
     typedef BcrDim<B, NR> Dm;
     constexpr int BB = B * B;
     double(*sD)[BB] = sDG;
@@ -530,6 +554,98 @@
     constexpr int NT_ = NW * 64;
     const int kreal = nb - chunk * 8 < 8 ? nb - chunk * 8 : 8;
     const bool placed = place && kreal < 8;
+
+    if constexpr (UF == 2) {
+        static_assert(NR == 3 && !TOP && 16 * (Dm::NT - 1) == 2 * B, "the last column tile holds the right-hand sides alone");
+        constexpr int XB = B * NR;
+        for (int e = tid; e < 9 * XB; e += NT_) (&sR[0][0])[e] = 0.0;
+        if (tid < 2) sZ[tid] = 0.0;
+        __syncthreads();
+        if (L0) {
+            const int row0 = chunk * 8 * B;
+            for (int t = tid; t < kreal * B; t += NT_) {
+                const int row = row0 + t;
+                if (row < n) {
+                    const double4 bb = rhs[row];
+                    double *Rb = &sR[1][0] + t * NR;
+                    Rb[0] = bb.x;
+                    Rb[1] = bb.y;
+                    Rb[2] = bb.z;
+                }
+            }
+        } else {
+            constexpr int NIR = (8 * XB + NT_ - 1) / NT_;
+            double vr[NIR], vy[NIR];
+#pragma unroll
+            for (int u = 0; u < NIR; u++) {
+                const int e = tid + NT_ * u, i = e / XB, el = e - i * XB, gb = chunk * 8 + i;
+                const bool ok = e < 8 * XB && i < kreal && gb < nred;
+                vr[u] = ok ? bcr_ld<COH>(inR + (size_t)gb * XB + el) : 0.0;
+                vy[u] = ok && gb + 1 < nred ? bcr_ld<COH>(inXR + (size_t)(gb + 1) * XB + el) : 0.0;
+            }
+#pragma unroll
+            for (int u = 0; u < NIR; u++) {
+                const int e = tid + NT_ * u, i = e / XB, gb = chunk * 8 + i;
+                if (e < 8 * XB && i < kreal && gb < nred) (&sR[1][0])[e] = vr[u] + vy[u];
+            }
+            if (chunk * 8 + 8 > nred && nred < nb)
+                for (int t = tid; t < 8 * B; t += NT_) {
+                    const int i = t / B, gb = chunk * 8 + i;
+                    if (gb >= nred && gb < nb) {
+                        const int row = (8 * nred + (gb - nred)) * B + (t - i * B);
+                        if (row < n) {
+                            const double4 bb = rhs[row];
+                            double *Rb = &sR[1][0] + t * NR;
+                            Rb[0] = bb.x;
+                            Rb[1] = bb.y;
+                            Rb[2] = bb.z;
+                        }
+                    }
+                }
+        }
+        __syncthreads();
+        BcrElim<B, NR, 1> E;
+        v4d out[Dm::MT][1];
+#define IRH_BCR_ROUND_RHS(RND)                                                                                      \
+    {                                                                                                               \
+        constexpr int NE = 4 >> RND;                                                                                \
+        int i = -1, a = -1, c = 7;                                                                                  \
+        if (wave < NE) {                                                                                            \
+            if (RND == 0) {                                                                                         \
+                i = 2 * wave;                                                                                       \
+                a = i - 1;                                                                                          \
+                c = i + 1;                                                                                          \
+            } else if (RND == 1) {                                                                                  \
+                i = 1 + 4 * wave;                                                                                   \
+                a = wave == 0 ? -1 : 3;                                                                             \
+                c = wave == 0 ? 3 : 7;                                                                              \
+            } else {                                                                                                \
+                i = 3;                                                                                              \
+            }                                                                                                       \
+        }                                                                                                           \
+        const bool active = i >= 0 && bcr_ridx(placed, kreal, i) >= 0;                                              \
+        const bool hasP = a >= 0 || hasExt;                                                                         \
+        const size_t el = (size_t)chunk * 7 + (i >= 0 ? i : 0);                                                     \
+        if (active)                                                                                                 \
+            E.template phase1<Dm::NT>(Dm::NT - 1, Dinvg + el * BB, stP + el * BB, hasP, stQ + el * BB, sR[i + 1], sZ, \
+                                      sR[c + 1], W + el * B * Dm::NC, sZ, lane);                                    \
+        __syncthreads();                                                                                            \
+        if (active && hasP) {                                                                                       \
+            E.template phase2_mul<Dm::NT>(Dm::NT - 1, stP + el * BB, out, lane);                                    \
+            E.template phase2_put<Dm::NT>(Dm::NT - 1, out, sZ, sZ, false, sR[a + 1], lane);                         \
+        }                                                                                                           \
+        __syncthreads();                                                                                            \
+    }
+        IRH_BCR_ROUND_RHS(0)
+        IRH_BCR_ROUND_RHS(1)
+        IRH_BCR_ROUND_RHS(2)
+#undef IRH_BCR_ROUND_RHS
+        for (int e = tid; e < XB; e += NT_) {
+            bcr_st<COH>(sepR + (size_t)chunk * XB + e, sR[8][e]);
+            if (hasExt) bcr_st<COH>(extR + (size_t)chunk * XB + e, sR[0][e]);
+        }
+        return;
+    }
 
     const bool fastload = !L0 && !placed && !(chunk * 8 + 8 > nred && nred < nb);
     if (!fastload) {
@@ -710,6 +826,12 @@
                                         \
         if (Dinvg && active && part == 0)                                                                           \
             for (int o = lane; o < BB; o += 64) Dinvg[((size_t)chunk * 7 + i) * BB + o] = sD[i][o];                 \
+        if constexpr (UF == 1)                                                                                      \
+            if (active && part == 0)                                                                                \
+                for (int o = lane; o < BB; o += 64) {                                                               \
+                    stP[((size_t)chunk * 7 + i) * BB + o] = sG[a + 1][o];                                           \
+                    stQ[((size_t)chunk * 7 + i) * BB + o] = sG[i + 1][o];                                           \
+                }                                                                                                   \
         bcr_stamp(stamps, 3 + 4 * RND);                                                                             \
         if (active && !(dbg & 2))                                                                                   \
             E.template phase1<WPE>(part, sD[i], sG[a + 1], hasP, sG[i + 1], sR[i + 1], sD[c], sR[c + 1],            \
@@ -771,6 +893,7 @@
     const uint8_t *bflag;
     const double *wsrc, *er;
     double *excess, *idg, *bval;
+    double *stP, *stQ;
 };
 template <bool ASM>
 struct BcrL0Ptr {
@@ -783,7 +906,7 @@
     typedef double4 *d4;
 };
 
-template <int B, int NR, bool L0, bool TOP, int NW, bool ASM = false>
+template <int B, int NR, bool L0, bool TOP, int NW, bool ASM = false, int UF = 0>
 __global__ __launch_bounds__(NW * 64, (NW == 4 && B <= 24 && NR == 3 ? 2 : 1)) void k_bcr_reduce(
 
     int nb, int nred, int n, const int *__restrict__ sl_off, const int *__restrict__ col, typename BcrL0Ptr<ASM>::d val,
@@ -824,9 +947,11 @@
         __syncthreads();
         __builtin_amdgcn_fence(__ATOMIC_ACQUIRE, "workgroup");
     }
-    bcr_reduce_body<B, NR, L0, TOP, NW, false>(blockIdx.x, sDG, sR, sZ, nb, nred, n, sl_off, col, val, diag, rhs, inD, inR, inXD, inXR,
-                                               inXG, W, sepD, sepR, extD, extR, extG, xtop, dbg, nfar, far_i, far_j, ext0, bptr,
-                                               bghost, bval, ghost_extcol, place, stamps, Dinvg, topDinv, deadctr, reg);
+    static_assert(UF == 0 || ASM, "the unit-weight factor rides on the assembling launch");
+    bcr_reduce_body<B, NR, L0, TOP, NW, false, UF>(blockIdx.x, sDG, sR, sZ, nb, nred, n, sl_off, col, val, diag, rhs, inD, inR, inXD, inXR,
+                                                   inXG, W, sepD, sepR, extD, extR, extG, xtop, dbg, nfar, far_i, far_j, ext0, bptr,
+                                                   bghost, bval, ghost_extcol, place, stamps, Dinvg, topDinv, deadctr, reg, A.stP,
+                                                   A.stQ);
 }
 
 static BcrTopSched bcr_top_schedule(int n) {
@@ -859,11 +984,12 @@
     return ((size_t)(2 * n - 1) * B * B + (size_t)2 * n * B * 3 + 2) * sizeof(double) + sizeof(BcrTopSched);
 }
 
-template <int B, int NW, bool COH>
+template <int B, int NW, bool COH, int UF = 0>
 __device__ __forceinline__ void bcr_top_body(double *smem, const BcrTopSched *__restrict__ Tg, const double *__restrict__ inD,
                                              const double *__restrict__ inR, const double *__restrict__ inXD,
                                              const double *__restrict__ inXR, const double *__restrict__ inXG,
-                                             double *__restrict__ xout, int dbg, long long *__restrict__ stamps) {
+                                             double *__restrict__ xout, int dbg, long long *__restrict__ stamps,
+                                             double *__restrict__ tst = nullptr) {
     constexpr int NR = 3;
     typedef BcrDim<B, NR> Dm;
     constexpr int BB = B * B, XB = B * NR, NT_ = NW * 64;
@@ -883,7 +1009,7 @@
     {
         constexpr int U = 6;
         const int nD = n * BB, nG = (n - 1) * BB, nR = n * XB;
-        for (int e0 = 0; e0 < nD; e0 += U * NT_) {
+        for (int e0 = 0; e0 < nD && UF != 2; e0 += U * NT_) {
             double vd[U], vx[U], vg[U];
 #pragma unroll
             for (int u = 0; u < U; u++) {
@@ -910,6 +1036,24 @@
     bcr_stamp(stamps, 1);
     for (int r = 0; r < T.nr; r++) {
         const int ne = T.ne[r];
+        if constexpr (UF == 2) {
+            const bool active = wave < ne;
+            const int i = active ? T.i[r][wave] : 0, a = active ? T.a[r][wave] : -1, c = active ? T.c[r][wave] : -1;
+            const bool hasP = a >= 0, hasQ = c >= 0;
+            const double *op = tst + (size_t)5 * (4 * r + (active ? wave : 0)) * BB;
+            BcrElim<B, NR, 1> E;
+            v4d out[Dm::MT][1];
+            if (active)
+                E.template phase1<Dm::NT>(Dm::NT - 1, op, op + BB, hasP, op + 2 * BB, sR[i], sZ, hasQ ? sR[c] : sR[i],
+                                          (double *)nullptr, sZ, lane, hasQ);
+            __syncthreads();
+            if (active && hasP) E.template phase2_mul<Dm::NT>(Dm::NT - 1, op + BB, out, lane);
+            if (active) E.template keep_w<Dm::NT>(Dm::NT - 1, sZ, sZ, hasQ, sR[i], lane);
+            __syncthreads();
+            if (active && hasP) E.template phase2_put<Dm::NT>(Dm::NT - 1, out, sZ, sZ, false, sR[a], lane);
+            __syncthreads();
+            continue;
+        }
         if (wave < ne && !(dbg & 1)) bcr_invert<B>(sD[T.i[r][wave]], lane);
         __syncthreads();
         bcr_stamp(stamps, 2 + 2 * r);
@@ -922,6 +1066,14 @@
             const bool hasP = a >= 0, hasQ = c >= 0;
             BcrElim<B, NR, 2> E;
             v4d out[Dm::MT][2];
+            double *op = UF == 1 ? tst + (size_t)5 * (4 * r + (active ? e : 0)) * BB : nullptr;
+            if constexpr (UF == 1)
+                if (active && part == 0)
+                    for (int o = lane; o < BB; o += 64) {
+                        op[o] = sD[i][o];
+                        op[BB + o] = hasP ? sG[a][o] : 0.0;
+                        op[2 * BB + o] = hasQ ? sG[i][o] : 0.0;
+                    }
             if (active && !(dbg & 2))
                 E.template phase1<WPE>(part, sD[i], hasP ? sG[a] : sZ, hasP, hasQ ? sG[i] : sZ, sR[i], hasQ ? sD[c] : sD[i],
                                        hasQ ? sR[c] : sR[i], (double *)nullptr, sZ, lane, hasQ);
@@ -931,6 +1083,12 @@
             __syncthreads();
             if (active && hasP && !(dbg & 4)) E.template phase2_put<WPE>(part, out, sG[a], sD[a], false, sR[a], lane);
             __syncthreads();
+            if constexpr (UF == 1)
+                if (active && part == 0)
+                    for (int o = lane; o < BB; o += 64) {
+                        op[3 * BB + o] = sD[i][o];
+                        op[4 * BB + o] = hasQ ? sG[i][o] : 0.0;
+                    }
         };
         if (ne > 2) products(std::integral_constant<int, 2>());
         else products(std::integral_constant<int, 4>());
@@ -938,15 +1096,18 @@
     }
     const int last = T.last;
     if (wave == 0) {
-        bcr_invert<B>(sD[last], lane);
+        if constexpr (UF != 2) bcr_invert<B>(sD[last], lane);
+        const double *Dl = UF == 2 ? tst + (size_t)kTopUnitLast * BB : sD[last];
         for (int o = lane; o < XB; o += 64) {
             const int k = o / NR, q = o - NR * k;
             double acc = 0.0;
-            for (int cidx = 0; cidx < B; cidx++) acc += sD[last][k * B + cidx] * sR[last][cidx * NR + q];
+            for (int cidx = 0; cidx < B; cidx++) acc += Dl[k * B + cidx] * sR[last][cidx * NR + q];
             sX[last][o] = acc;
         }
     }
     __syncthreads();
+    if constexpr (UF == 1)
+        for (int o = tid; o < BB; o += NT_) tst[(size_t)kTopUnitLast * BB + o] = sD[last][o];
     bcr_stamp(stamps, 14);
     {
         constexpr int UPB = B / 4, NCT = (2 * B + 15) / 16;
@@ -957,6 +1118,8 @@
                 const int e = u / UPB, it = u - e * UPB;
                 const int i = T.i[r][e], a = T.a[r][e], c = T.c[r][e];
                 const double *xa = sX[a >= 0 ? a : 0], *xc = sX[c >= 0 ? c : 0];
+                const double *wP = UF == 2 ? tst + ((size_t)5 * (4 * r + e) + 3) * BB : sD[i];
+                const double *wQ = UF == 2 ? tst + ((size_t)5 * (4 * r + e) + 4) * BB : sG[i];
                 const int k = 4 * it + lk;
                 double s0 = 0.0, s1 = 0.0, s2 = 0.0;
 #pragma unroll
@@ -964,14 +1127,14 @@
                     const int cidx = lp + 16 * t;
                     if (cidx < B) {
                         if (a >= 0) {
-                            const double wv = sD[i][k * B + cidx];
+                            const double wv = wP[k * B + cidx];
                             s0 += wv * xa[cidx * 3 + 0];
                             s1 += wv * xa[cidx * 3 + 1];
                             s2 += wv * xa[cidx * 3 + 2];
                         }
                     } else if (cidx < 2 * B) {
                         if (c >= 0) {
-                            const double wv = sG[i][k * B + cidx - B];
+                            const double wv = wQ[k * B + cidx - B];
                             s0 += wv * xc[(cidx - B) * 3 + 0];
                             s1 += wv * xc[(cidx - B) * 3 + 1];
                             s2 += wv * xc[(cidx - B) * 3 + 2];
@@ -1005,29 +1168,30 @@
 
 extern __shared__ __attribute__((aligned(16))) double up_smem[];
 typedef IRH_GPTR(const BcrUpArgs) gp_args;
-template <int B, bool TOP>
+template <int B, bool TOP, int UF = 0>
 __device__ __noinline__ void bcr_up_chunk(gp_args A, int i, int dbg, long long *stl) {
     constexpr int NR = 3;
     IRH_GPTR(const BcrUpLevel) L = &A->lev[i];
     double(*sDG)[B * B] = reinterpret_cast<double(*)[B * B]>(up_smem);
     double(*sR)[B * NR] = reinterpret_cast<double(*)[B * NR]>(up_smem + 16 * B * B);
     double *sZ = up_smem + 16 * B * B + 9 * B * NR;
-    bcr_reduce_body<B, NR, false, TOP, 8, true>(
+    bcr_reduce_body<B, NR, false, TOP, 8, true, UF>(
         blockIdx.x, sDG, sR, sZ, L->nb, L->nred, A->n, (const int *)A->sl_off, (const int *)A->col, (const double *)A->val,
         (const double *)A->diag, (const double4 *)A->rhs, (const double *)L->inD, (const double *)L->inR, (const double *)L->inXD,
         (const double *)L->inXR, (const double *)L->inXG, (double *)L->W, (double *)L->sepD, (double *)L->sepR, (double *)L->extD,
         (double *)L->extR, (double *)L->extG, (double *)A->xtop, dbg, 0, (const int *)nullptr, (const int *)nullptr, 0, (const int *)nullptr, (const int *)nullptr,
-        (const double *)nullptr, (const int *)nullptr, 0, stl ? stl - (size_t)blockIdx.x * 16 : nullptr, (double *)nullptr,
-        (double *)nullptr, (int *)nullptr, 0);
-}
-template <int B>
+        (const double *)nullptr, (const int *)nullptr, 0, stl ? stl - (size_t)blockIdx.x * 16 : nullptr,
+        UF ? (double *)L->stD : (double *)nullptr, (double *)nullptr, (int *)nullptr, 0, UF ? (double *)L->stP : (double *)nullptr,
+        UF ? (double *)L->stQ : (double *)nullptr);
+}
+template <int B, int UF = 0>
 __device__ __noinline__ void bcr_up_top(gp_args A, int i, int dbg, long long *stl) {
     IRH_GPTR(const BcrUpLevel) L = &A->lev[i];
-    bcr_top_body<B, 8, true>(up_smem, (const BcrTopSched *)&A->top, (const double *)L->inD, (const double *)L->inR,
-                             (const double *)L->inXD, (const double *)L->inXR, (const double *)L->inXG, (double *)A->xtop_all, dbg,
-                             stl ? stl - (size_t)blockIdx.x * 16 : nullptr);
-}
-template <int B>
+    bcr_top_body<B, 8, true, UF>(up_smem, (const BcrTopSched *)&A->top, (const double *)L->inD, (const double *)L->inR,
+                                 (const double *)L->inXD, (const double *)L->inXR, (const double *)L->inXG, (double *)A->xtop_all, dbg,
+                                 stl ? stl - (size_t)blockIdx.x * 16 : nullptr, UF ? (double *)A->tst : (double *)nullptr);
+}
+template <int B, int UF = 0>
 __global__ __launch_bounds__(512, 1) void k_bcr_reduce_up(const BcrUpArgs *__restrict__ Ap, unsigned gen, int dbg,
                                                           long long *__restrict__ stamps) {
     constexpr int NR = 3;
@@ -1063,16 +1227,18 @@
         if (i == nl - 1) {
             const bool bad = !fine || __hip_atomic_load((const int *)A.fail, __ATOMIC_RELAXED, __HIP_MEMORY_SCOPE_AGENT) != 0;
             if (A.top16) {
-                if (!bad) bcr_up_top<B>(Ag, i, dbg, stl);
+                if (!bad) bcr_up_top<B, UF>(Ag, i, dbg, stl);
                 else
                     for (int e = threadIdx.x; e < A.top.n * B * NR; e += 512) A.xtop_all[e] = __builtin_nan("");
             } else {
-                if (!bad) bcr_up_chunk<B, true>(Ag, i, dbg, stl);
-                else
+                if constexpr (UF == 0) {
+                    if (!bad) bcr_up_chunk<B, true>(Ag, i, dbg, stl);
+                }
+                if (bad)
                     for (int e = threadIdx.x; e < B * NR; e += 512) A.xtop[e] = __builtin_nan("");
             }
         } else {
-            if (fine) bcr_up_chunk<B, false>(Ag, i, dbg, stl);
+            if (fine) bcr_up_chunk<B, false, UF>(Ag, i, dbg, stl);
             if (stl && threadIdx.x == 0) stl[18] = (long long)__builtin_readcyclecounter();
             __builtin_amdgcn_s_waitcnt(0);
             __syncthreads();
@@ -1088,6 +1254,7 @@
     return ntop > 0 ? std::max(chunk, bcr_top_lds(B, ntop)) : chunk;
 }
 namespace {
+std::atomic<unsigned> g_unit_epoch{0};
 std::atomic<int> g_up_used[16];
 template <int B>
 int bcr_up_capacity(int dev) {
@@ -2287,8 +2454,39 @@
         if (fused_up) fused_up = bcr_up_reserve<B>(g, S.lev[1].nch);
     }
     if (only < 0 && phase != 2) S.up_used = false;
+    int uf = 0;
+    BcrUnit &U = S.unit;
+    if (only < 0 && phase != 2) U.last = 0;
+    if constexpr (NR == 3 && (B == 8 || B == 16 || B == 24)) {
+        const int req = g.bcr_unit_req;
+        if (req && fused_up && S.top16 && dbg == 0 && !g.bcr_guard && !g.bcr_out && !g.sw.bcr_no_unit_factor &&
+            (g.bcr_asm_fused || req == 3)) {
+            if (!U.lev.empty() && U.epoch != g_unit_epoch.load(std::memory_order_acquire)) U.release();
+            uf = U.valid ? 2 : (req == 1 ? 1 : 0);
+            if (uf == 1 && U.lev.empty()) {
+                constexpr int NC = 2 * B + 3;
+                U.epoch = g_unit_epoch.load(std::memory_order_acquire);
+                U.lev.resize((size_t)nl - 1);
+                size_t words = 0;
+                for (int l = 0; l + 1 < nl; l++) {
+                    const size_t ne = (size_t)S.lev[l].nch * 7;
+                    U.lev[(size_t)l].Wu.alloc(ne * B * NC);
+                    U.lev[(size_t)l].Di.alloc(ne * B * B);
+                    U.lev[(size_t)l].P.alloc(ne * B * B);
+                    U.lev[(size_t)l].Q.alloc(ne * B * B);
+                    words += ne * B * (NC + 3 * B);
+                }
+                U.top.alloc((size_t)(kTopUnitLast + 1) * B * B);
+                words += (size_t)(kTopUnitLast + 1) * B * B;
+                U.bytes = (int64_t)(words * sizeof(double));
+            }
+        }
+        U.last = uf;
+    }
+    const bool uf_up_only = uf == 2 && g.bcr_unit_req == 3;
     for (int l = 0; l < nl && phase != 2; l++) {
         if (only >= 0 && only != l) continue;
+        if (l == 0 && uf_up_only) continue;
         if constexpr (NR == 3 && B <= 24) {
             if (S.top16 && l == nl - 1 && !fused_up) {
                 const BcrLevel &F = S.lev[l - 1];
@@ -2339,14 +2537,40 @@
                 if (g.sw.bcr_fake_up_fail && g.stats.direct_up_fallbacks == 0)
                     IRH_CHECK(hipMemsetAsync(S.up_cnt.p + kUpLevels, 1, sizeof(int), st));
                 const size_t lds = bcr_up_lds<B>(S.top16 ? S.lev[nl - 1].nb : 0);
-                static std::atomic<size_t> lds_set[16];
-                if (lds_set[g.device & 15].load() < lds) {
-                    IRH_CHECK(hipFuncSetAttribute(reinterpret_cast<const void *>(&k_bcr_reduce_up<B>),
-                                                  hipFuncAttributeMaxDynamicSharedMemorySize, (int)lds));
-                    lds_set[g.device & 15].store(lds);
-                }
-                hipLaunchKernelGGL((k_bcr_reduce_up<B>), dim3(S.lev[1].nch), dim3(512), lds, st, S.up_args.p, ++S.up_gen, dbg,
-                                   (dbg & 128) ? S.stamps.p : (long long *)nullptr);
+                static std::atomic<size_t> lds_set[3][16];
+                auto launch_up = [&](auto uf_tag, const BcrUpArgs *args) {
+                    constexpr int UF = decltype(uf_tag)::value;
+                    if (lds_set[UF][g.device & 15].load() < lds) {
+                        IRH_CHECK(hipFuncSetAttribute(reinterpret_cast<const void *>(&k_bcr_reduce_up<B, UF>),
+                                                      hipFuncAttributeMaxDynamicSharedMemorySize, (int)lds));
+                        lds_set[UF][g.device & 15].store(lds);
+                    }
+                    hipLaunchKernelGGL((k_bcr_reduce_up<B, UF>), dim3(S.lev[1].nch), dim3(512), lds, st, args, ++S.up_gen, dbg,
+                                       (dbg & 128) ? S.stamps.p : (long long *)nullptr);
+                };
+                if constexpr (B == 8 || B == 16 || B == 24) {
+                    if (uf && !U.up_args.p) {
+                        BcrUpArgs A;
+                        IRH_CHECK(hipMemcpyAsync(&A, S.up_args.p, sizeof(A), hipMemcpyDeviceToHost, st));
+                        IRH_CHECK(hipStreamSynchronize(st));
+                        for (int i = 0; i + 1 < A.nl; i++) {
+                            BcrUnitLevel &Ui = U.lev[(size_t)i + 1];
+                            A.lev[i].W = (gp_d)Ui.Wu.p;
+                            A.lev[i].stD = (gp_d)Ui.Di.p;
+                            A.lev[i].stP = (gp_d)Ui.P.p;
+                            A.lev[i].stQ = (gp_d)Ui.Q.p;
+                        }
+                        A.tst = (gp_d)U.top.p;
+                        U.up_args.alloc(1);
+                        IRH_CHECK(hipMemcpyAsync(U.up_args.p, &A, sizeof(A), hipMemcpyHostToDevice, st));
+                        IRH_CHECK(hipStreamSynchronize(st));
+                    }
+                    if (uf == 2) launch_up(std::integral_constant<int, 2>(), U.up_args.p);
+                    else if (uf == 1) launch_up(std::integral_constant<int, 1>(), U.up_args.p);
+                    else launch_up(std::integral_constant<int, 0>(), S.up_args.p);
+                } else {
+                    launch_up(std::integral_constant<int, 0>(), S.up_args.p);
+                }
                 S.up_used = true;
                 continue;
             }
@@ -2356,10 +2580,15 @@
         const bool top = l == nl - 1 && !open_top;
 #define IRH_BCR_ARGS                                                                                             \
     L.nb, L.nred, L0.n, L0.sl_off.p, L0.col.p, L0.val.p, L0.diag.p, L0.b.p, F ? F->sepD.p : nullptr,             \
-        F ? F->sepR.p : nullptr, F ? F->extD.p : nullptr, F ? F->extR.p : nullptr, F ? F->extG.p : nullptr, L.W.p, \
+        F ? F->sepR.p : nullptr, F ? F->extD.p : nullptr, F ? F->extR.p : nullptr, F ? F->extG.p : nullptr, Wl, \
         L.sepD.p, L.sepR.p, L.extD.p, L.extR.p, L.extG.p, S.xtop.p, dbg, nfar, fi, fj, S.ext0, g.bptr.p, g.bghost.p,  \
-        g.bval.p, S.ghost_extcol.p, (int)g.bcr_shard, stamps, S.nfar > 0 ? S.Dinv[(size_t)l].p : (double *)nullptr,         \
+        g.bval.p, S.ghost_extcol.p, (int)g.bcr_shard, stamps, Dl,                                                          \
         S.nfar > 0 ? S.topDinv.p : (double *)nullptr, S.nfar > 0 ? S.dead.p : (int *)nullptr, (int)g.bcr_guard, asmA
+        double *Wl = L.W.p, *Dl = S.nfar > 0 ? S.Dinv[(size_t)l].p : (double *)nullptr;
+        if (uf && l == 0) {
+            Wl = U.lev[0].Wu.p;
+            Dl = U.lev[0].Di.p;
+        }
         const bool wide = L.nch <= 256;
         BcrAsmArgs asmA{};
         bool asm0 = false;
@@ -2369,13 +2598,35 @@
                 asmA = BcrAsmArgs{L.nch,   L0.nsl,    (long long)g.m, (long long)g.mpad, g.slot_eid.p, g.tile_e0.p, g.beid.p,
                                   g.bflag.p, g.bcr_wsrc, g.er.p,         L0.excess.p,       L0.idg.p,     g.bval.p};
                 const int extra = std::max(0, L0.nsl - L.nch * (8 * B / 64));
+                bool launched = false;
+                if constexpr (B == 8 || B == 16 || B == 24) {
+                    if (uf) {
+                        asmA.stP = U.lev[0].P.p;
+                        asmA.stQ = U.lev[0].Q.p;
+#define IRH_BCR_LAUNCH_UNIT(UF_)                                                                                          \
+    if (wide)                                                                                                             \
+        hipLaunchKernelGGL((k_bcr_reduce<B, NR, true, false, 8, true, UF_>), dim3(L.nch + extra), dim3(512), 0, st,       \
+                           IRH_BCR_ARGS);                                                                                 \
+    else                                                                                                                  \
+        hipLaunchKernelGGL((k_bcr_reduce<B, NR, true, false, 4, true, UF_>), dim3(L.nch + extra), dim3(256), 0, st,       \
+                           IRH_BCR_ARGS);
+                        if (uf == 2) {
+                            IRH_BCR_LAUNCH_UNIT(2)
+                        } else {
+                            IRH_BCR_LAUNCH_UNIT(1)
+                        }
+#undef IRH_BCR_LAUNCH_UNIT
+                        launched = true;
+                    }
+                }
 #define IRH_BCR_LAUNCH_ASM(TOP_)                                                                                          \
     if (B <= 24 && wide)                                                                                                  \
         hipLaunchKernelGGL((k_bcr_reduce<B, NR, true, TOP_, (B <= 24 ? 8 : 4), true>), dim3(L.nch + extra),               \
                            dim3(B <= 24 ? 512 : 256), 0, st, IRH_BCR_ARGS);                                               \
     else                                                                                                                  \
         hipLaunchKernelGGL((k_bcr_reduce<B, NR, true, TOP_, 4, true>), dim3(L.nch + extra), dim3(256), 0, st, IRH_BCR_ARGS);
-                if (top) {
+                if (launched) {
+                } else if (top) {
                     IRH_BCR_LAUNCH_ASM(true)
                 } else {
                     IRH_BCR_LAUNCH_ASM(false)
@@ -2412,7 +2663,7 @@
     const bool apply = NR == 3 && g.bcr_apply && only < 0 && phase == 0 && (fused_back || (S.top16 && nl == 2)) && !g.bcr_out &&
                        g.ng == 0;
     g.bcr_applied = apply;
-    for (int l = ltop; l >= 0 && phase != 1; l--) {
+    for (int l = ltop; l >= 0 && phase != 1 && !uf_up_only; l--) {
         if (only >= 0 && only != 100 + l) continue;
         BcrLevel &L = S.lev[l];
         if constexpr (NR == 3) {
@@ -2420,7 +2671,7 @@
                 if (l > 1) continue;
                 BcrBackPlan P;
                 for (int k = 0; k < nl; k++) {
-                    P.W[k] = S.lev[k].W.p;
+                    P.W[k] = uf && k + 1 < nl ? U.lev[(size_t)k].Wu.p : S.lev[k].W.p;
                     P.nb[k] = S.lev[k].nb;
                 }
                 P.top = ltop;
@@ -2433,7 +2684,8 @@
         }
         const double *xc = l == nl - 1 ? (open_top ? xc_top : S.xtop.p) : S.lev[l + 1].x.p;
         if (l == 0)
-            hipLaunchKernelGGL((k_bcr_back<B, NR, true>), dim3(L.nch), dim3(256), 0, st, L.nb, L.nred, L0.n, L.W.p, xc,
+            hipLaunchKernelGGL((k_bcr_back<B, NR, true>), dim3(L.nch), dim3(256), 0, st, L.nb, L.nred, L0.n,
+                               uf ? U.lev[0].Wu.p : L.W.p, xc,
                                (double *)nullptr, Xout, (double *)nullptr, 0, 0, nfar, xext, (int)g.bcr_shard,
                                apply ? g.Q.p : (double4 *)nullptr, g.f, g.part_score.p, 0);
         else
@@ -2955,6 +3207,10 @@
     }
     put(g.bcr->nfar);
     put(g.bcr_asm_fused_last ? 1 : 0);
+    const bool stored = bcr_unit_valid(g);
+    put(stored ? 1 : 0);
+    put(g.bcr->unit.solves);
+    put(stored ? g.bcr->unit.bytes : 0);
     return k;
 }
 
@@ -3121,6 +3377,23 @@
     bcr_up_release(g);
     return true;
 }
+
+void bcr_unit_commit(Graph &g, bool finite) {
+    if (!g.bcr) return;
+    BcrUnit &U = g.bcr->unit;
+    if (U.last == 1) {
+        if (finite) U.valid = true;
+        else U.release();
+    } else if (U.last == 2 && finite) {
+        U.solves += 1;
+    }
+    U.last = 0;
+}
+int bcr_unit_last(Graph &g) { return g.bcr ? g.bcr->unit.last : 0; }
+bool bcr_unit_valid(Graph &g) {
+    return g.bcr && g.bcr->unit.valid && g.bcr->unit.epoch == g_unit_epoch.load(std::memory_order_acquire);
+}
+void bcr_unit_trim() noexcept { g_unit_epoch.fetch_add(1, std::memory_order_acq_rel); }
 
 int bcr_levels(Graph &g) {
     if (!g.bcr_B) return 0;
diff --git a/irotavg_amd/csrc/capi.cpp b/irotavg_amd/csrc/capi.cpp
--- a/irotavg_amd/csrc/capi.cpp
+++ b/irotavg_amd/csrc/capi.cpp
@@ -240,6 +240,7 @@
 int64_t irotavg_trim_memory(void) {
     try {
         StreamPool::get().trim();
+        bcr_unit_trim();
         return (int64_t)DevPool::get().trim();
     } catch (...) {
         return 0;
diff --git a/irotavg_amd/csrc/graph.hpp b/irotavg_amd/csrc/graph.hpp
--- a/irotavg_amd/csrc/graph.hpp
+++ b/irotavg_amd/csrc/graph.hpp
@@ -115,6 +115,7 @@
     bool pool_headroom = false;
     bool bcr_no_fused_up = false;
     bool bcr_asm_fused = false, bcr_asm_fused_last = false;
+    int bcr_unit_req = 0;
     std::unique_ptr<BcrState, BcrDeleter> bcr;
     std::vector<int> bcr_far_i, bcr_far_j, bcr_far_e;
     const double *bcr_wsrc = nullptr;
@@ -330,6 +331,10 @@
 int bcr_stamps(Graph &g, int level, int chunk, double *out);
 int bcr_stamps_up(Graph &g, double *out);
 bool bcr_up_failed(Graph &g);
+void bcr_unit_commit(Graph &g, bool finite);
+int bcr_unit_last(Graph &g);
+bool bcr_unit_valid(Graph &g);
+void bcr_unit_trim() noexcept;
 const int *bcr_fail_word(Graph &g);
 struct BcrTop {
     int B = 0, world = 0;
diff --git a/irotavg_amd/csrc/solver.hip b/irotavg_amd/csrc/solver.hip
--- a/irotavg_amd/csrc/solver.hip
+++ b/irotavg_amd/csrc/solver.hip
@@ -1965,7 +1965,13 @@
             g.bcr_apply = ap_slots > 0;
             g.bcr_applied = false;
             with_res = !(it + 1 >= max_iters || (it > 0 && score <= 50.0 * change_th));
+            g.bcr_unit_req = it == 0 && fuse_wr ? 1 : 0;
+            struct UnitReq {
+                Graph &g;
+                ~UnitReq() { g.bcr_unit_req = 0; }
+            } unit_req{g};
             rc = ls_solve(g);
+            g.bcr_unit_req = 0;
             g.bcr_apply = false;
             if (rc != IROTAVG_OK) break;
             if (bcr_closures(g) > 0) {
@@ -2037,6 +2043,7 @@
                 launch_update_weights(g, cost, sigma);
                 score = apply_step(g);
             }
+            bcr_unit_commit(g, std::isfinite(score));
             if (!std::isfinite(score)) {
                 if (bcr_up_failed(g)) {
                     er_fresh = true;
@@ -2163,6 +2170,7 @@
     hipEvent_t e0, e1;
     IRH_CHECK(hipEventCreate(&e0));
     IRH_CHECK(hipEventCreate(&e1));
+    bool unit_served = true;
     auto once = [&]() {
         switch (which) {
         case 1: launch_edge_residual(g); break;
@@ -2191,12 +2199,25 @@
             break;
         default:
             if (which == 19) (void)bcr_solve(g);
+            else if (which == 17 || which == 18) {
+                g.bcr_unit_req = which == 17 ? 2 : 3;
+                g.bcr_asm_fused = which == 17;
+                g.bcr_wsrc = g.dw.p;
+                g.bcr_wsquare = 1;
+                (void)bcr_solve(g);
+                g.bcr_unit_req = 0;
+                g.bcr_asm_fused = false;
+                unit_served = unit_served && bcr_unit_last(g) == 2;
+                bcr_unit_commit(g, false);
+            }
             else if (which >= 20 && which < 40) (void)bcr_solve(g, which - 20);
             else if (which >= 40 && which < 60) (void)bcr_solve(g, 100 + which - 40);
             break;
         }
     };
-    if (which >= 19 && which < 60) {
+    if (which == 17 || which == 18) {
+        if (!g.bcr_B || !bcr_unit_valid(g)) return IROTAVG_ERR_BAD_ARG;
+    } else if (which >= 19 && which < 60) {
         if (!g.bcr_B) return IROTAVG_ERR_BAD_ARG;
         const int nl = bcr_levels(g);
         if ((which >= 20 && which < 40 && which - 20 >= nl) || (which >= 40 && which - 40 >= nl)) return IROTAVG_ERR_BAD_ARG;
@@ -2229,6 +2250,7 @@
     *ms = (double)t / std::max(reps, 1);
     (void)hipEventDestroy(e0);
     (void)hipEventDestroy(e1);
+    if ((which == 17 || which == 18) && !unit_served) return IROTAVG_ERR_BAD_ARG;
     return IROTAVG_OK;
 }
 
diff --git a/irotavg_amd/csrc/switches.hpp b/irotavg_amd/csrc/switches.hpp
--- a/irotavg_amd/csrc/switches.hpp
+++ b/irotavg_amd/csrc/switches.hpp
@@ -16,7 +16,7 @@
     bool no_settle = false, no_fused_cl = false;
     int inexact = -1;
     bool bcr_no_mixed = false, bcr_no_top16 = false, bcr_fake_up_fail = false, bcr_fake_give_up = false;
-    bool bcr_no_closures = false, bcr_s_tiles = false, bcr_no_fused_asm = false;
+    bool bcr_no_closures = false, bcr_s_tiles = false, bcr_no_fused_asm = false, bcr_no_unit_factor = false;
     int bcr_up_cap = 1024;
     int bcr_dbg = 0, bcr_stamp_chunk = 0;
     bool dist_no_closures = false, dist_halo_p2p = false;
@@ -52,6 +52,7 @@
     s.bcr_no_closures = set("IROTAVG_BCR_NO_CLOSURES");
     s.bcr_s_tiles = set("IROTAVG_BCR_S_TILES");
     s.bcr_no_fused_asm = set("IROTAVG_BCR_NO_FUSED_ASM");
+    s.bcr_no_unit_factor = set("IROTAVG_BCR_NO_UNIT_FACTOR");
     s.bcr_up_cap = num("IROTAVG_BCR_UP_CAP", 1024);
     s.bcr_dbg = num("IROTAVG_BCR_DBG", 0);
     s.bcr_stamp_chunk = num("IROTAVG_BCR_STAMP_CHUNK", 0);
@@ -71,7 +72,7 @@
             s.has_band_direct, s.band_direct, s.host_build, s.upload_threads, s.asm_classic, s.no_small_tuning,
             s.no_dense_refine, s.no_band_inverse, s.pcg_trace, s.cg2_giveup, s.no_settle, s.no_fused_cl, s.inexact,
             s.bcr_no_mixed, s.bcr_no_top16, s.bcr_fake_up_fail, s.bcr_fake_give_up, s.bcr_no_closures, s.bcr_s_tiles,
-            s.bcr_no_fused_asm,             s.bcr_up_cap, s.bcr_dbg, s.bcr_stamp_chunk, s.dist_no_closures, s.dist_halo_p2p, s.no_resident, s.window_stamps,
+            s.bcr_no_fused_asm, s.bcr_no_unit_factor, s.bcr_up_cap, s.bcr_dbg, s.bcr_stamp_chunk, s.dist_no_closures, s.dist_halo_p2p, s.no_resident, s.window_stamps,
             s.resident_min_edges, s.build_timing, s.rotavg_timing);
     };
     return t(a) == t(b);
```

After: 8.078 billion, median of 6. 1.06x the previous value.
